# zero-savvy/vimz

Measured on AMD Instinct MI355X. Metric: nova_folding_steps_per_sec, higher is better.
Workload: dtype u32 limbs (256-bit Montgomery integers over BN254 Fr/Fq)

## Files before the change

### include/vimz_hip.h

```cpp
#ifndef VIMZ_HIP_H
#define VIMZ_HIP_H

#include <stddef.h>
#include <stdint.h>

#ifdef __cplusplus
extern "C" {
#endif

#define VIMZ_OK 0
#define VIMZ_ERR_INVALID (-1)
#define VIMZ_ERR_HIP (-2)
#define VIMZ_ERR_NO_DEVICE (-3)
#define VIMZ_ERR_UNSAT (-4)

#define VIMZ_FORM_CANONICAL 0
#define VIMZ_FORM_MONTGOMERY 1

#define VIMZ_CURVE_BN254_G1 0
#define VIMZ_CURVE_GRUMPKIN 1
#define VIMZ_CURVE_PALLAS 2
#define VIMZ_CURVE_VESTA 3

#define VIMZ_FIELD_BN254_FR 0
#define VIMZ_FIELD_BN254_FQ 1
#define VIMZ_FIELD_PALLAS_FP 2
#define VIMZ_FIELD_VESTA_FQ 3

typedef struct vimz_ctx vimz_ctx;
typedef struct vimz_bases vimz_bases;
typedef struct vimz_vec vimz_vec;

int vimz_ctx_create(int device, vimz_ctx** out);
void vimz_ctx_destroy(vimz_ctx* ctx);
const char* vimz_last_error(const vimz_ctx* ctx);
const char* vimz_version(void);
int vimz_device_info(vimz_ctx* ctx, char* name, size_t name_len, int* cus, uint64_t* hbm_bytes);
int vimz_sync(vimz_ctx* ctx);

int vimz_trace_marker(vimz_ctx* ctx, int id);
long vimz_set_head_rows(long rows);
long vimz_set_rows_group(long rows);
int vimz_host_fingerprint(vimz_ctx* ctx, double out[4]);
int vimz_timer_start(vimz_ctx* ctx);
int vimz_timer_stop(vimz_ctx* ctx, float* ms_out);
int vimz_set_profiling(vimz_ctx* ctx, int enabled);
int vimz_msm_last_profile(vimz_ctx* ctx, float ms[6], uint32_t info[4]);
int vimz_msm_profile_totals(vimz_ctx* ctx, double ms[6], uint64_t counts[3], int reset);

int vimz_bases_upload(vimz_ctx* ctx, int curve, const uint64_t* xy, size_t n, int form, vimz_bases** out);
int vimz_bases_generate(vimz_ctx* ctx, int curve, const char* label, size_t label_len, size_t n, vimz_bases** out);
int vimz_bases_download(vimz_ctx* ctx, const vimz_bases* b, size_t offset, uint64_t* xy, size_t n, int form);
int vimz_bases_precompute(vimz_ctx* ctx, vimz_bases* b, int window_bits);
size_t vimz_bases_len(const vimz_bases* b);
void vimz_bases_free(vimz_ctx* ctx, vimz_bases* b);

size_t vimz_pack_count(size_t height, size_t width, int block);
int vimz_pack_pixels(vimz_ctx* ctx, const uint8_t* pixels, size_t height, size_t width, int channels, int block, uint64_t* out);

typedef struct {
  const uint8_t* pixels;
  size_t height, width;
  int channels;
  const uint64_t* units;
  size_t n_units, unit_len;
  int block;
  size_t max_units;
  const uint8_t* drop;
} vimz_image_desc;
int vimz_image_hash(vimz_ctx* ctx, const vimz_image_desc* imgs, size_t n, uint64_t* out);
int vimz_image_hash_last_profile(vimz_ctx* ctx, double ms[2]);

#define VIMZ_EDIT_HASH 0
#define VIMZ_EDIT_GRAYSCALE 1
#define VIMZ_EDIT_BRIGHTNESS 2
#define VIMZ_EDIT_CONTRAST 3
#define VIMZ_EDIT_BLUR 4
#define VIMZ_EDIT_SHARPNESS 5
#define VIMZ_EDIT_RESIZE 6
#define VIMZ_EDIT_CROP 7
#define VIMZ_EDIT_REDACT 8
typedef struct {
  int op;
  const uint8_t* pixels;
  size_t height, width;
  int channels;
  int64_t source;
  double factor;
  size_t x, y;
  size_t new_width, new_height;
  const uint8_t* redact;
  size_t n_redact;
  uint8_t* out_pixels;
  uint64_t* out_source;
  uint64_t* out_target;
} vimz_edit_desc;
typedef struct {
  size_t height, width;
  int channels;
  size_t source_units, source_unit_len;
  size_t target_units, target_unit_len;
} vimz_edit_shape;
#define VIMZ_EDIT_MAX_DESCS 4096
int vimz_image_edit_shapes(vimz_ctx* ctx, const vimz_edit_desc* descs, size_t n, vimz_edit_shape* out);
int vimz_image_edit(vimz_ctx* ctx, const vimz_edit_desc* descs, size_t n);
int vimz_image_edit_last_profile(vimz_ctx* ctx, double ms[3]);

int vimz_vec_alloc(vimz_ctx* ctx, int field, size_t n, vimz_vec** out);
int vimz_vec_upload(vimz_ctx* ctx, vimz_vec* v, size_t offset, const uint64_t* host, size_t n, int form);
int vimz_vec_download(vimz_ctx* ctx, const vimz_vec* v, size_t offset, uint64_t* host, size_t n, int form);
size_t vimz_vec_len(const vimz_vec* v);
void vimz_vec_free(vimz_ctx* ctx, vimz_vec* v);

int vimz_msm(vimz_ctx* ctx, const vimz_bases* bases, const uint64_t* scalars, size_t n, int form,
             int window_bits, uint64_t out_xy[8], int out_form);
int vimz_msm_vec(vimz_ctx* ctx, const vimz_bases* bases, size_t base_offset, const vimz_vec* v, size_t offset,
                 size_t n, int window_bits, uint64_t out_xy[8], int out_form);

#define VIMZ_MSM_SPLIT_ONES 1
int vimz_msm_vec_ex(vimz_ctx* ctx, const vimz_bases* bases, size_t base_offset, const vimz_vec* v, size_t offset,
                    size_t n, int window_bits, int flags, uint64_t out_xy[8], int out_form);

typedef struct vimz_r1cs vimz_r1cs;
typedef struct { const uint32_t* row; const uint32_t* col; const uint64_t* val ; size_t nnz; } vimz_coo;
int vimz_r1cs_upload(vimz_ctx* ctx, int field, size_t nrows, size_t ncols, const vimz_coo* A, const vimz_coo* B, const vimz_coo* C, int form,
// ... 201 lines not shown
```

### include/vimz_hip_testing.h

```cpp
#ifndef VIMZ_HIP_TESTING_H
#define VIMZ_HIP_TESTING_H
#include "vimz_hip.h"

#ifdef __cplusplus
extern "C" {
#endif

int vimz_cf_poke(vimz_cf* v, int which, size_t index, const uint64_t value[4]);
int vimz_cf_selfcheck(int steps, uint32_t* result, uint64_t counts[8]);
int64_t vimz_cf_selfcheck_last_step(int steps, void* buf, size_t cap);
int64_t vimz_cf_selfcheck_merge(int segs_run0, int segs_run1, void* buf, size_t cap);
int64_t vimz_worker_selftest(int jobs);
int vimz_strict_bits_selfcheck(int field, int values, uint64_t out[8]);
void vimz_test_forge_public_slot(int on);
int vimz_decider_selfcheck(int steps, int full, uint32_t* result, uint64_t counts[4]);
int vimz_testing_kzg_setup_seeded(vimz_ctx* ctx, const uint8_t* seed, size_t seed_len, size_t n, vimz_bases** srs_out, uint64_t vk_g2_out[16]);
int vimz_testing_decider_setup_seeded(vimz_cf* prover, const uint64_t kzg_vk_g2[16], int light, const uint8_t* seed, size_t seed_len, vimz_decider** out, double seconds[4]);

int vimz_test_fp29_probe(vimz_ctx* ctx, int field, int op, const uint32_t* a, const uint32_t* b, const uint32_t* c, const uint32_t* d, uint32_t* out, size_t n);
int vimz_test_spmv_cross16(vimz_ctx* ctx, const vimz_r1cs* S, size_t row0, size_t nrows, const vimz_vec* z, vimz_vec* az, vimz_vec* bz, vimz_vec* cz,
                           const vimz_vec* az1, const vimz_vec* bz1, const vimz_vec* cz1, const uint64_t u1[4], const uint64_t u2[4], int form, vimz_vec* T);
int vimz_test_cross_term_masked(vimz_ctx* ctx, size_t n, const vimz_vec* az1, const vimz_vec* bz1, const vimz_vec* cz1, const uint64_t u1[4], const vimz_vec* az2,
                                const vimz_vec* bz2, const vimz_vec* cz2, const uint64_t u2[4], int form, vimz_vec* T, vimz_vec* Tm, size_t nb);
int vimz_test_msm_rows(vimz_ctx* ctx, const vimz_bases* bases, const uint64_t* scalars, size_t n, size_t row_stride, size_t G, int form, int use_tables,
                       size_t n_ones, int calls, uint64_t* out_xy, uint64_t* s1_xy, uint64_t* s1_ref_xy);

#ifdef __cplusplus
}
#endif
#endif
```

### vimz_amd/csrc/ivc.hip

```cpp
#include "ivc_internal.hpp"

namespace {

int scalar_bits(const uint32_t* k) {
  for (int i = 7; i >= 0; i--) if (k[i]) return 32 * i + 32 - __builtin_clz(k[i]);
  return 0;
}

int finish_secondary(vimz_ivc* v) {
  if (!v->pending_sec) return VIMZ_OK;
  vimz_ctx* ctx = v->ctx;
  double t0 = now_s();
  P_TRY(vz_wait_stream(v->s2));
  v->u2.W = msm_finish<Grumpkin>(v->plan_W2, v->pin + 2 * v->pin_res);
  P_TRY(vz_wait_stream(ctx->stream));
  v->ph_s[IP_WAIT_SEC] += now_s() - t0; v->ph_n[IP_WAIT_SEC]++;
  if (ctx->profiling) { float ms = 0; if (hipEventElapsedTime(&ms, v->ev_b0, v->ev_b1) == hipSuccess) { v->ph_s[IP_RESERVED] += ms * 1e-3; v->ph_n[IP_RESERVED]++; } }
  if (v->sec_T_valid) v->T2 = msm_finish<Grumpkin>(v->plan_T2, v->pin + 3 * v->pin_res);
  else { v->T2.x = Fe::zero(); v->T2.y = Fe::zero(); }
  static const bool dbg = getenv("VIMZ_DEBUG_CHECK_MSM") != nullptr;
  if (dbg) {
    G2Aff r; MsmStats st;
    P_TRY(msm_run<Grumpkin>(ctx->stream, ctx->msm_ws, v->ck2->d, v->sec.z2 + 8, v->sec.n_w - 3, 1, 0, &r, &st, nullptr, 0, nullptr));
    if (!r.x.eq(v->u2.W.x) || !r.y.eq(v->u2.W.y)) fprintf(stderr, "[dbg] step %llu: MSM(W2) on stream 2 differs from the recomputation\n", (unsigned long long)v->i);
    if (v->sec_T_valid) {
      P_TRY(msm_run<Grumpkin>(ctx->stream, ctx->msm_ws, v->ck2->d, v->sec.T, v->sec.n_c, 1, 0, &r, &st, nullptr, 0, nullptr));
      if (!r.x.eq(v->T2.x) || !r.y.eq(v->T2.y)) fprintf(stderr, "[dbg] step %llu: MSM(T2) differs from the recomputation\n", (unsigned long long)v->i);
    }
  }
  v->pending_sec = false;
  return VIMZ_OK;
}

int ivc_fold_core(vimz_ivc* v, const uint64_t* step_inputs, const uint64_t* witnesses, size_t nsteps) {
  if (!nsteps) return VIMZ_OK;
  vimz_ctx* ctx = v->ctx;
  if (v->broken) return vz_fail(ctx, VIMZ_ERR_INVALID, "this IVC failed in the middle of a step and cannot be folded any further");
  vimz_prover* p = v->pri;
  std::lock_guard<std::mutex> g(ctx->mu);
  P_TRY(hipSetDevice(ctx->device));
  hipStream_t s = ctx->stream;
  const size_t nw = p->n_wires, nc = p->n_c, sw = p->step_wires, sc = p->step_c;
  const size_t aw1 = v->c1->aug_wires();
  SecDev& S = v->sec;
  int rc;
  const double t_all = now_s();
  FoldJob job; job.step_inputs = step_inputs; job.witnesses = witnesses; job.nsteps = nsteps;
  dbg_stamp(p, "ivc fold: lock taken");
  if ((rc = fold_prepare(p, job, true))) return rc;
  struct BrokenGuard { vimz_ivc* v; bool armed = true; ~BrokenGuard() { if (armed) v->broken = true; } } guard{v};
  auto settle = [&](size_t rows_done) {
    hipStreamSynchronize(p->sB);
    if (p->sD) hipStreamSynchronize(p->sD);
    hipStreamSynchronize(v->s3); v->t1[0].step = v->t1[1].step = -1;
    const int rc2 = finish_secondary(v);
    for (uint32_t q = 0; q < p->len_z; q++) p->z_cur[q] = job.zs[rows_done * p->len_z + q];
    if (!rc2) guard.armed = false;
  };
  static const bool dbg_timing = getenv("VIMZ_DEBUG_TIMING") != nullptr;
  const double t_prep = now_s() - t_all;
  double t_first = 0, t_wait0 = 0, t_hook = 0, t_hk[5] = {0, 0, 0, 0, 0}, t_wp[5] = {0, 0, 0, 0, 0};
  const std::vector<Fe>& zs = job.zs;
  const size_t pin_stride = FoldJob::pin_stride;
  char* pin_aug1 = v->pin + 5 * v->pin_res;
  char* pin_w2 = pin_aug1 + 32 * aw1;
  const Fq zero_q = Fq::zero();

  typedef vimz_prover::BatchBuf BufRef;
  const bool trick = v->bool_rows && v->helpers.empty() && !witnesses;
  if (trick && v->i > 0 && !v->ca_valid) {
    G1Aff r; MsmStats st;
    P_TRY(hipStreamSynchronize(v->s3));
    P_TRY(msm_run<BnG1>(s, ctx->msm_ws, p->ck->d, p->AZ, p->n_bool, 1, 0, &r, &st, nullptr, 0, p->ck->tables ? &job.tbl : nullptr));
    v->CA = from_affine(r);
  }
  v->ca_valid = false;
  G1Aff S1_row; S1_row.x = S1_row.y = Fq::zero();
  bool pend_ca = false; uint32_t pend_rho[4] = {0, 0, 0, 0}; G1Aff pend_S1 = S1_row; int pend_slot[2] = {-1, -1};
  auto apply_pending_ca = [&]() {
    if (!pend_ca) return;
    if (!aff_is_identity(pend_S1)) { const uint32_t k[5] = {pend_rho[0], pend_rho[1], pend_rho[2], pend_rho[3], 1u}; G1 t = scalar_mul(pend_S1, k, 129); add_full(v->CA, t); }
    for (int q : pend_slot) if (q >= 0) v->t1[q].ca_at = v->CA;
    pend_ca = false;
  };
  auto queue_msm = [&](int par) -> int {
    auto& S = v->t1[par];
    const size_t parts = v->helpers.size() + 1, share = (sc + parts - 1) / parts;
    v->t1_main_n = std::min(share, sc);
    if (!v->helpers.empty()) {
      P_TRY(hipEventRecord(v->ev_T, v->s3));
      size_t off = v->t1_main_n;
      for (auto& h : v->helpers) {
        h.off = off; h.n = off < sc ? std::min(share, sc - off) : 0; off += h.n;
        if (!h.n) continue;
        P_TRY(hipSetDevice(h.ctx->device));
        P_TRY(hipStreamWaitEvent(h.s, v->ev_T, 0));
        P_TRY(hipMemcpyAsync(h.T, S.buf + 8 * h.off, 32 * h.n, hipMemcpyDefault, h.s));
        P_TRY(msm_launch<BnG1>(h.s, h.ws, h.ck->d + (size_t)AFFINE_WORDS * h.off, h.T, h.n, 1, 0, h.pin, &h.plan, nullptr, 0, nullptr));
      }
      P_TRY(hipSetDevice(ctx->device));
    }
    double tq = now_s();
    P_TRY(msm_launch<BnG1>(v->s3, v->ws3, p->ck->d, S.tricked ? S.bufm : S.buf, v->t1_main_n, 1, 0, S.pin, &S.plan, ctx->profiling ? S.ev : nullptr, 0,
                           p->ck->tables && v->helpers.empty() ? &job.tbl : nullptr));
    t_hk[2] += now_s() - tq; tq = now_s();
    if (ctx->profiling) P_TRY(hipMemcpyAsync(S.pin + v->pin_res, v->ws3.totals, 8, hipMemcpyDeviceToHost, v->s3));
    P_TRY(hipEventRecord(S.done, v->s3));
    t_hk[1] += now_s() - tq;
    return VIMZ_OK;
  };
  auto launch_direct = [&](BufRef& b2, size_t row, uint64_t step) -> int {
    auto& S = v->t1[step & 1];
    P_TRY(hipEventRecord(v->ev_fold, s));
    P_TRY(hipStreamWaitEvent(v->s3, v->ev_fold, 0));
    P_TRY(wait_row_flag(b2, row, b2.ev[row]));
    hipLaunchKernelGGL(k_cross_term<Fr>, dim3(stream_grid(sc)), dim3(256), 0, v->s3, sc, p->AZ, p->BZ, p->CZ, v->u1_run,
                       b2.az + 8 * row * nc, b2.bz + 8 * row * nc, b2.cz + 8 * row * nc, Fe::one(), S.buf, trick ? S.bufm : (uint32_t*)nullptr, p->n_bool);
    P_TRY(hipGetLastError());
    S.step = (int64_t)step; S.hasB = false;
    S.tricked = trick; S.u_at = v->u1_run; S.ca_at = v->CA;
    return queue_msm((int)(step & 1));
  };
  struct RowAt { BufRef* b; size_t row; };
  struct FoldArgs { uint64_t i; BufRef* cur; size_t r; Fe rho; bool need1; RowAt next1; bool look; RowAt next2; };
  auto launch_fold_and_cross = [&](const FoldArgs& a) -> int {
    const int par = (int)(a.i & 1);
    auto& Scur = v->t1[par]; auto& Soth = v->t1[par ^ 1];
    const bool fold_E = a.i > 0, hasB = fold_E && Scur.hasB;
    const uint32_t *az = a.cur->az + 8 * a.r * nc, *bz = a.cur->bz + 8 * a.r * nc, *cz = a.cur->cz + 8 * a.r * nc;
    if (hasB) P_TRY(wait_row_flag(*a.cur, a.cur->flag_rows + a.r, a.cur->ev_d[a.r]));
    const RowAt* t = a.need1 ? &a.next1 : a.look ? &a.next2 : nullptr;
    uint32_t* out = a.need1 ? Soth.buf : a.look ? Scur.buf : nullptr;
    uint32_t* outm = !trick ? nullptr : a.need1 ? Soth.bufm : a.look ? Scur.bufm : nullptr;
    double tq = now_s();
    if (t) P_TRY(wait_row_flag(*t->b, t->row, t->b->ev[t->row]));
    t_hk[4] += now_s() - tq; tq = now_s();
    hipLaunchKernelGGL(k_fold_cross<Fr>, dim3(stream_grid(sc)), dim3(256), 0, v->s3, sc, p->AZ, p->BZ, p->CZ, p->E, (const uint32_t*)Scur.buf, fold_E ? 1 : 0, a.rho,
                       hasB ? 1 : 0, v->rho_prev, hasB ? (const uint32_t*)(a.cur->d + 8 * a.r * sc) : (const uint32_t*)nullptr, v->u1_run, az, bz, cz,
                       out, t ? t->b->az + 8 * t->row * nc : nullptr, t ? t->b->bz + 8 * t->row * nc : nullptr, t ? t->b->cz + 8 * t->row * nc : nullptr, Fe::one(),
                       outm, p->n_bool);
    P_TRY(hipGetLastError());
    if (a.need1 && a.look) {
      P_TRY(wait_row_flag(*a.next2.b, a.next2.row, a.next2.b->ev[a.next2.row]));
      hipLaunchKernelGGL(k_cross_term<Fr>, dim3(stream_grid(sc)), dim3(256), 0, v->s3, sc, p->AZ, p->BZ, p->CZ, v->u1_run,
                         a.next2.b->az + 8 * a.next2.row * nc, a.next2.b->bz + 8 * a.next2.row * nc, a.next2.b->cz + 8 * a.next2.row * nc, Fe::one(), Scur.buf,
                         trick ? Scur.bufm : (uint32_t*)nullptr, p->n_bool);
      P_TRY(hipGetLastError());
    }
    t_hk[0] += now_s() - tq; tq = now_s();
    P_TRY(hipEventRecord(v->ev_fused, v->s3)); v->fused_recorded = true;
    t_hk[1] += now_s() - tq;
    if (a.need1) { Soth.step = (int64_t)a.i + 1; Soth.hasB = false; Soth.tricked = trick; Soth.u_at = v->u1_run; int rc2 = queue_msm(par ^ 1); if (rc2) return rc2; }
    if (a.look) { Scur.step = (int64_t)a.i + 2; Scur.hasB = true; Scur.tricked = trick; Scur.u_at = v->u1_run; int rc2 = queue_msm(par); if (rc2) return rc2; }
    return VIMZ_OK;
  };
  std::atomic<size_t> allowed{0}, issued{job.next_issue};
  std::atomic<int> issuer_rc{VIMZ_OK};
  std::atomic<bool> issuer_stop{false};
  std::thread issuer([&, b0 = job.next_issue] {
    if (hipSetDevice(ctx->device) != hipSuccess) { issuer_rc = VIMZ_ERR_HIP; return; }
    for (size_t b = b0; b < job.nbatches; b++) {
      const size_t need = job.first(b) + job.rows(b);
      while (allowed.load(std::memory_order_acquire) <= b || job.states_upto.load(std::memory_order_acquire) < need) {
        if (issuer_stop.load()) return;
        if (job.helper_done.load() && job.states_upto.load() < need) { issuer_rc = job.helper_rc ? job.helper_rc : VIMZ_ERR_HIP; return; }
        std::this_thread::sleep_for(std::chrono::microseconds(100));
      }
      const double _ti = now_s();
      const int rc2 = fold_issue(p, job, b);
      if (dbg_timing) fprintf(stderr, "[timing] producer: batch %zu (%zu rows): ready at %.1f ms, issue took %.1f ms\n", b, job.rows(b), 1e3 * (_ti - t_all), 1e3 * (now_s() - _ti));
      if (rc2) { issuer_rc = rc2; return; }
      issued.store(b + 1, std::memory_order_release);
    }
  });
  struct IssuerJoin { std::thread& t; std::atomic<bool>& stop; ~IssuerJoin() { stop = true; if (t.joinable()) t.join(); } } issuer_join{issuer, issuer_stop};
  auto wait_issued = [&](size_t b) -> int {
    const double t_wait = now_s(); uint64_t spins = 0;
    while (issued.load(std::memory_order_acquire) <= b) {
      const int irc = issuer_rc.load();
      if (irc) { if (ctx->err.empty()) ctx->err = job.helper_err.empty() ? std::string("fold: the batch producer stopped early") : job.helper_err; return irc; }
      std::this_thread::yield();
      if ((++spins & 0xfffff) == 0 && now_s() - t_wait > 120.0) return vz_fail(ctx, VIMZ_ERR_HIP, "fold: batch not issued within 120 s");
    }
    return VIMZ_OK;
  };
  for (size_t k = 0; k < job.nbatches; k++) {
    auto& bb = p->buf[k & 1];
    const size_t first = job.first(k), rows = job.rows(k);
    double t0 = now_s();
    allowed.store(k + 2, std::memory_order_release);
    if ((rc = wait_issued(k))) return rc;
    if (k == 0) dbg_stamp(p, "ivc fold: first batch issued");
    P_TRY(vz_wait_event(bb.wit_done));
    v->ph_s[IP_PRODUCER] += now_s() - t0;
    if (k == 0) { t_wait0 = now_s() - t0; t_first = now_s() - t_all; dbg_stamp(p, "ivc fold: first batch's witnesses ready"); }
    for (size_t r = 0; r < rows; r++) if (bb.status_host[r]) {
      char msg[128]; snprintf(msg, sizeof(msg), "step %llu: the step relation is not satisfiable for these rows", (unsigned long long)(v->i + r));
      settle(first);
      return vz_fail(ctx, VIMZ_ERR_UNSAT, msg);
    }
    for (size_t r = 0; r < rows; r++) {
      const uint64_t i = v->i;
      uint32_t* Zi = bb.Z + 8 * r * nw;
      uint32_t *az = bb.az + 8 * r * nc, *bz = bb.bz + 8 * r * nc, *cz = bb.cz + 8 * r * nc;
      v->c1->precompute_statement(i + 1, v->z0, zs.data() + (first + r + 1) * p->len_z);
      G1 boolCorr = G1::identity();
      if (trick) {
        apply_pending_ca();
        P_TRY(wait_row_flag(bb, r, bb.ev[r]));
        S1_row = to_affine(ones_finish<BnG1>((const char*)bb.pin + r * pin_stride + vimz_prover::S1_SLOT));
        auto& sl = v->t1[i & 1];
        if (i > 0 && sl.step == (int64_t)i && sl.tricked) {
          if (!aff_is_identity(S1_row)) { const Fe uc = Fe::from_mont(sl.u_at); boolCorr = scalar_mul(S1_row, uc.v, scalar_bits(uc.v)); }
          G1 nca = sl.ca_at; if (!nca.is_identity()) nca.Y = Fq::neg(nca.Y);
          add_full(boolCorr, nca);
        }
      }
      if ((rc = finish_secondary(v))) return rc;
      t0 = now_s();
      AugIn<BnFr> in1; in1.digest = v->c1->digest; in1.z0 = v->z0; in1.i = i; in1.U = v->U2; in1.u = v->u2; in1.T = v->T2;
      std::vector<Fe> aug1; bool bad = false;
      AugOut<BnFr> o1 = v->c1->witness(in1, zs.data() + (first + r) * p->len_z, zs.data() + (first + r + 1) * p->len_z, aug1, &bad);
      if (bad) { settle(first + r); return vz_fail(ctx, VIMZ_ERR_UNSAT, "primary verifier circuit: inconsistent incoming instance"); }
      v->ph_s[IP_SYNTH1] += now_s() - t0; v->ph_n[IP_SYNTH1]++;
      t0 = now_s();
      v->U2 = o1.U_new;
      memcpy(pin_aug1, aug1.data(), 32 * aw1);
      P_TRY(wait_row_flag(bb, r, bb.ev[r]));
      P_TRY(upload_pinned(s, Zi + 8 * sw, pin_aug1, 32 * aw1));
      P_TRY(hipEventRecord(v->ev_fork, s));
      P_TRY(hipStreamWaitEvent(v->s2, v->ev_fork, 0));
      P_TRY(msm_launch<BnG1>(v->s2, v->ws2, p->ck->d + (size_t)AFFINE_WORDS * (sw - 1), Zi + 8 * sw, aw1 - 2, 1, 0, v->pin, &v->plan_aug, nullptr, 0, v->tb_aug.d ? &v->tb_aug : nullptr));
      P_TRY(hipStreamWaitEvent(s, v->ev_fold, 0));
      hipLaunchKernelGGL(k_spmv_cross16<Fr>, dim3((unsigned)((16 * (nc - sc) + 255) / 256)), dim3(256), 0, s, p->A, p->B, p->C, p->dict, (uint32_t)sc, (uint32_t)(nc - sc),
                         Zi, az, bz, cz, i > 0 ? p->AZ : nullptr, p->BZ, p->CZ, v->u1_run, Fe::one(), p->T);
// ... 764 lines not shown
```

### vimz_amd/csrc/msm.hpp

```cpp
#pragma once
#include <cstdlib>
#include <cstring>
#include <mutex>
#include "msm_api.hpp"
#include "ec_mem.hpp"

namespace vz {

struct MsmTuning { int sort_blocks = 0, combine_lane_bits = -1, small_lean = 0, witness_sub = 0, ones_dense = 1, reduce_planes = 0, accum_lds_kb = 0, dense_sub = 0, signed_scalars = 1; };
inline const MsmTuning& msm_tuning() {
  static const MsmTuning t = [] {
    MsmTuning r;
    if (const char* e = getenv("VIMZ_TUNE")) {
      if (const char* q = strstr(e, "sort_blocks=")) r.sort_blocks = atoi(q + 12);
      if (const char* q = strstr(e, "combine_lane_bits=")) r.combine_lane_bits = atoi(q + 18);
      if (const char* q = strstr(e, "small_lean=")) r.small_lean = atoi(q + 11);
      if (const char* q = strstr(e, "witness_sub=")) { const int v = atoi(q + 12); if (v >= 2 && v <= MSM_SUB) r.witness_sub = v; }
      if (const char* q = strstr(e, "dense_sub=")) { const int v = atoi(q + 10); if (v >= 2 && v <= MSM_SUB) r.dense_sub = v; }
      if (const char* q = strstr(e, "ones_dense=")) r.ones_dense = atoi(q + 11);
      if (const char* q = strstr(e, "reduce_planes=")) r.reduce_planes = atoi(q + 14);
      if (const char* q = strstr(e, "signed_scalars=")) r.signed_scalars = atoi(q + 15) != 0;
      if (const char* q = strstr(e, "accum_lds_kb=")) { const int v = atoi(q + 13); if (v >= 0 && v <= 160) r.accum_lds_kb = v; }
    }
    return r;
  }();
  return t;
}


__device__ __forceinline__ uint32_t window_bits(const uint32_t* s, int lo, int c) {
  int limb = lo >> 5, off = lo & 31;
  if (limb >= 8) return 0;
  uint64_t v = s[limb];
  if (limb + 1 < 8) v |= (uint64_t)s[limb + 1] << 32;
  return (uint32_t)(v >> off) & ((1u << c) - 1);
}

template <class S>
__device__ __forceinline__ bool load_scalar(const uint32_t* __restrict__ scalars, size_t i, int mont, int skip_ones, int sgn, uint32_t* s, uint32_t& flip) {
  const uint4* p = reinterpret_cast<const uint4*>(scalars + 8 * i);
  uint4 a = p[0], b = p[1];
  S x;
  x.v[0] = a.x; x.v[1] = a.y; x.v[2] = a.z; x.v[3] = a.w; x.v[4] = b.x; x.v[5] = b.y; x.v[6] = b.z; x.v[7] = b.w;
  if (x.is_zero()) return false;
  if (skip_ones) {
    bool one;
    if (mont) one = x.eq(S::one());
    else { uint32_t o = x.v[0] ^ 1u; for (int k = 1; k < 8; k++) o |= x.v[k]; one = o == 0; }
    if (one) return false;
  }
  if (mont) x = S::from_mont(x);
  flip = 0;
  if (sgn) {
    uint32_t t[8]; uint64_t br = 0, lt = 0;
#pragma unroll
    for (int k = 0; k < 8; k++) { const uint64_t d = (uint64_t)S::Params::MOD.w[k] - x.v[k] - br; t[k] = (uint32_t)d; br = (d >> 32) & 1; }
#pragma unroll
    for (int k = 0; k < 8; k++) { const uint64_t d = (uint64_t)t[k] - x.v[k] - lt; lt = (d >> 32) & 1; }
    if (!br && lt) {
      flip = 1;
#pragma unroll
      for (int k = 0; k < 8; k++) x.v[k] = t[k];
    }
  }
#pragma unroll
  for (int k = 0; k < 8; k++) s[k] = x.v[k];
  return true;
}

template <class Fn>
__device__ __forceinline__ void for_each_digit(const uint32_t* s, int c, int K, uint32_t flip, Fn f) {
  uint32_t carry = 0;
  const uint32_t half = 1u << (c - 1);
  for (int w = 0; w < K; w++) {
    uint32_t d = window_bits(s, w * c, c) + carry;
    uint32_t neg = d > half;
    uint32_t mag = neg ? (1u << c) - d : d;
    carry = neg;
    if (mag) f(w, mag - 1, neg ^ flip);
  }
}

__device__ __forceinline__ uint32_t agg_atomic_inc(uint32_t* __restrict__ ctr, uint32_t g) {
  const uint32_t lane = __lane_id();
  bool done = false;
  uint32_t pos = 0;
  for (int round = 0; round < 4; round++) {
    const uint64_t pending = __ballot(!done);
    if (pending == 0) break;
    const int leader = __ffsll((unsigned long long)pending) - 1;
    const uint32_t lg = __shfl(g, leader);
    const bool mine = !done && g == lg;
    const uint64_t same = __ballot(mine);
    uint32_t base = 0;
    if (mine && lane == (uint32_t)leader) base = atomicAdd(&ctr[g], (uint32_t)__popcll(same));
    base = __shfl(base, leader);
    if (mine) { pos = base + (uint32_t)__popcll(same & ((1ull << lane) - 1ull)); done = true; }
    if (__popcll(same) < 4) break;
  }
  if (!done) pos = atomicAdd(&ctr[g], 1u);
  return pos;
}

template <class S>
__global__ void k_hist(const uint32_t* __restrict__ scalars, size_t n, int mont, int skip_ones, int sgn, int c, int K, uint32_t nbw ,
                       uint32_t* __restrict__ counts) {
  for (size_t i = blockIdx.x * (size_t)blockDim.x + threadIdx.x; i < n; i += (size_t)gridDim.x * blockDim.x) {
    uint32_t s[8], flip;
    if (!load_scalar<S>(scalars, i, mont, skip_ones, sgn, s, flip)) continue;
    for_each_digit(s, c, K, flip, [&](int w, uint32_t b, uint32_t) { agg_atomic_inc(counts, (uint32_t)w * nbw + b); });
  }
}

__device__ __forceinline__ void scan_body(const uint32_t* __restrict__ counts, uint32_t nb,
                                               uint32_t* __restrict__ bucket_off, uint32_t* __restrict__ sub_off,
                                               uint32_t* __restrict__ totals, uint32_t sub,
                                               uint32_t* __restrict__ heavy ,
                                               uint32_t heavy_min, uint32_t heavy_cap) {
  __shared__ uint32_t wv_e[2][16], wv_s[2][16];
  const uint32_t t = threadIdx.x, lane = t & 63u, wv = t >> 6;
  uint32_t carry_e = 0, carry_s = 0;
  for (uint32_t base = 0, it = 0; base < nb; base += 1024, it++) {
    const uint32_t b = base + t;
    const uint32_t cnt = b < nb ? counts[b] : 0u, m = (cnt + sub - 1) / sub;
    uint32_t ie = cnt, is = m;
#pragma unroll
    for (uint32_t d = 1; d < 64; d <<= 1) {
      const uint32_t ve = __shfl_up(ie, d), vs = __shfl_up(is, d);
      if (lane >= d) { ie += ve; is += vs; }
    }
    if (lane == 63) { wv_e[it & 1][wv] = ie; wv_s[it & 1][wv] = is; }
    __syncthreads();
    uint32_t oe = 0, os = 0, te = 0, ts = 0;
    for (uint32_t q = 0; q < 16; q++) { const uint32_t xe = wv_e[it & 1][q], xs = wv_s[it & 1][q]; if (q < wv) { oe += xe; os += xs; } te += xe; ts += xs; }
    if (b < nb) {
      bucket_off[b] = carry_e + oe + ie - cnt; sub_off[b] = carry_s + os + is - m;
      if (m > heavy_min) { const uint32_t slot = atomicAdd(&heavy[0], 1u); if (slot < heavy_cap) heavy[1 + slot] = b; }
    }
    carry_e += te; carry_s += ts;
  }
  if (t == 0) { bucket_off[nb] = carry_e; sub_off[nb] = carry_s; totals[0] = carry_s; totals[1] = carry_e; }
}
template <int SUB>
__global__ void __launch_bounds__(1024) k_scan(const uint32_t* __restrict__ counts, uint32_t nb, uint32_t* __restrict__ bucket_off, uint32_t* __restrict__ sub_off,
                                               uint32_t* __restrict__ totals, uint32_t sub, uint32_t* __restrict__ heavy, uint32_t heavy_min, uint32_t heavy_cap) {
  scan_body(counts, nb, bucket_off, sub_off, totals, sub, heavy, heavy_min, heavy_cap);
}

template <class S>
__global__ void k_scatter(const uint32_t* __restrict__ scalars, size_t n, int mont, int skip_ones, int sgn, int c, int K, uint32_t nbw,
                          uint32_t pt_stride ,
                          const uint32_t* __restrict__ bucket_off, uint32_t* __restrict__ cursor,
                          uint32_t* __restrict__ sorted) {
  for (size_t i = blockIdx.x * (size_t)blockDim.x + threadIdx.x; i < n; i += (size_t)gridDim.x * blockDim.x) {
    uint32_t s[8], flip;
    if (!load_scalar<S>(scalars, i, mont, skip_ones, sgn, s, flip)) continue;
    for_each_digit(s, c, K, flip, [&](int w, uint32_t b, uint32_t neg) {
      uint32_t g = (uint32_t)w * nbw + b;
      uint32_t pos = bucket_off[g] + agg_atomic_inc(cursor, g);
      sorted[pos] = ((uint32_t)i + (uint32_t)w * pt_stride) | (neg << 31);
    });
  }
}

constexpr uint32_t SORT_BLOCKS = 256;
constexpr uint32_t SORT_THREADS = 1024;

template <class S>
__global__ void __launch_bounds__(SORT_THREADS) k_hist_lds(const uint32_t* __restrict__ scalars, size_t n, int mont, int skip_ones, int sgn, int c, int K,
                                                           uint32_t nbw, uint32_t nb, uint32_t* __restrict__ block_hist , MsmRowStrides rs) {
  extern __shared__ uint32_t lds_cnt[];
  scalars += blockIdx.y * rs.scalars; block_hist += blockIdx.y * rs.block_hist;
  for (uint32_t g = threadIdx.x; g < nb; g += SORT_THREADS) lds_cnt[g] = 0;
  __syncthreads();
  const size_t chunk = (n + gridDim.x - 1) / gridDim.x;
  const size_t lo = blockIdx.x * chunk, hi = lo + chunk < n ? lo + chunk : n;
  for (size_t i = lo + threadIdx.x; i < hi; i += SORT_THREADS) {
    uint32_t s[8], flip;
    if (!load_scalar<S>(scalars, i, mont, skip_ones, sgn, s, flip)) continue;
    for_each_digit(s, c, K, flip, [&](int w, uint32_t b, uint32_t) { atomicAdd(&lds_cnt[(uint32_t)w * nbw + b], 1u); });
  }
  __syncthreads();
  uint32_t* out = block_hist + (size_t)blockIdx.x * nb;
  for (uint32_t g = threadIdx.x; g < nb; g += SORT_THREADS) out[g] = lds_cnt[g];
}

template <int DUMMY>
__global__ void __launch_bounds__(1024) k_prefix_scan(uint32_t* __restrict__ block_hist, uint32_t nb, uint32_t* __restrict__ counts, uint32_t nblocks,
                                                      uint32_t* __restrict__ heavy, uint32_t* __restrict__ bucket_off, uint32_t* __restrict__ sub_off,
                                                      uint32_t* __restrict__ totals, uint32_t sub, uint32_t heavy_min, uint32_t heavy_cap, MsmRowStrides rs) {
  __shared__ uint32_t s_last;
  {
    const size_t row = blockIdx.y;
    block_hist += row * rs.block_hist; counts += row * rs.counts; heavy += row * rs.heavy; bucket_off += row * rs.offs; sub_off += row * rs.offs; totals += row * rs.totals;
  }
  const uint32_t g = blockIdx.x * blockDim.x + threadIdx.x;
  if (g < nb) {
    uint32_t run = 0;
    for (uint32_t blk = 0; blk < nblocks; blk++) {
      const size_t idx = (size_t)blk * nb + g;
      const uint32_t v = block_hist[idx];
      block_hist[idx] = run;
      run += v;
    }
    counts[g] = run;
  }
  __threadfence();
  __syncthreads();
  if (threadIdx.x == 0) s_last = atomicAdd(&totals[2], 1u) == gridDim.x - 1 ? 1u : 0u;
  __syncthreads();
  if (!s_last) return;
  __threadfence();
  if (threadIdx.x == 0) { __hip_atomic_store(&totals[2], 0u, __ATOMIC_RELAXED, __HIP_MEMORY_SCOPE_AGENT); heavy[0] = 0; }
  __syncthreads();
  scan_body(counts, nb, bucket_off, sub_off, totals, sub, heavy, heavy_min, heavy_cap);
}

template <class S>
__global__ void __launch_bounds__(SORT_THREADS) k_scatter_lds(const uint32_t* __restrict__ scalars, size_t n, int mont, int skip_ones, int sgn, int c, int K,
                                                              uint32_t nbw, uint32_t nb, uint32_t pt_stride, const uint32_t* __restrict__ bucket_off,
                                                              const uint32_t* __restrict__ block_hist, uint32_t* __restrict__ sorted, MsmRowStrides rs) {
  extern __shared__ uint32_t lds_pos[];
  { const size_t row = blockIdx.y; scalars += row * rs.scalars; bucket_off += row * rs.offs; block_hist += row * rs.block_hist; sorted += row * rs.sorted; }
  const uint32_t* mine = block_hist + (size_t)blockIdx.x * nb;
  for (uint32_t g = threadIdx.x; g < nb; g += SORT_THREADS) lds_pos[g] = bucket_off[g] + mine[g];
  __syncthreads();
  const size_t chunk = (n + gridDim.x - 1) / gridDim.x;
  const size_t lo = blockIdx.x * chunk, hi = lo + chunk < n ? lo + chunk : n;
  for (size_t i = lo + threadIdx.x; i < hi; i += SORT_THREADS) {
    uint32_t s[8], flip;
    if (!load_scalar<S>(scalars, i, mont, skip_ones, sgn, s, flip)) continue;
    for_each_digit(s, c, K, flip, [&](int w, uint32_t b, uint32_t neg) {
      const uint32_t pos = atomicAdd(&lds_pos[(uint32_t)w * nbw + b], 1u);
      sorted[pos] = ((uint32_t)i + (uint32_t)w * pt_stride) | (neg << 31);
    });
  }
}

template <class F>
__global__ void __launch_bounds__(256, 3) k_accum(const uint32_t* __restrict__ bases, const uint32_t* __restrict__ sorted,
                                               const uint32_t* __restrict__ bucket_off, const uint32_t* __restrict__ sub_off,
                                               uint32_t nb, const uint32_t* __restrict__ totals,
                                               uint32_t* __restrict__ partial, uint32_t sub, MsmRowStrides rs) {
  { const size_t row = blockIdx.y; sorted += row * rs.sorted; bucket_off += row * rs.offs; sub_off += row * rs.offs; totals += row * rs.totals; partial += row * rs.partial; }
  const uint32_t total = totals[0];
  uint32_t s = blockIdx.x * blockDim.x + threadIdx.x;
  if (s >= total) return;
  uint32_t lo = 0, hi = nb;
  while (hi - lo > 1) {
    uint32_t mid = (lo + hi) >> 1;
    if (sub_off[mid] <= s) lo = mid; else hi = mid;
  }
  const uint32_t b = lo, k = s - sub_off[b];
  const uint32_t beg = bucket_off[b] + k * sub;
  const uint32_t end = min(bucket_off[b + 1], beg + sub);
  XYZZ<F> acc = XYZZ<F>::identity();
  uint32_t ent = beg < end ? sorted[beg] : 0u;
  RawAffine raw = load_affine_raw(bases, ent & 0x7fffffffu);
  for (uint32_t e = beg; e < end; e++) {
    const uint32_t ent_n = e + 1 < end ? sorted[e + 1] : ent;
    const RawAffine raw_n = load_affine_raw(bases, ent_n & 0x7fffffffu);
    Affine<F> q = affine_of_raw<F>(raw);
    if ((ent >> 31) && !aff_is_identity(q)) q.y = F::neg(q.y);
    add_mixed(acc, q);
    ent = ent_n; raw = raw_n;
  }
  store_xyzz(partial, s, acc);
}

constexpr uint32_t ONES_THREADS = 16384;
template <class S>
__device__ __forceinline__ bool scalar_is_one(const uint32_t* __restrict__ scalars, size_t i, int mont) {
  const uint4* p = reinterpret_cast<const uint4*>(scalars + 8 * i);
  const uint4 a = p[0], b = p[1];
  if (mont) return a.x == S::Params::R1.w[0] && a.y == S::Params::R1.w[1] && a.z == S::Params::R1.w[2] && a.w == S::Params::R1.w[3] &&
                   b.x == S::Params::R1.w[4] && b.y == S::Params::R1.w[5] && b.z == S::Params::R1.w[6] && b.w == S::Params::R1.w[7];
  return a.x == 1u && (a.y | a.z | a.w | b.x | b.y | b.z | b.w) == 0u;
}
template <class S, class F>
__global__ void __launch_bounds__(256) k_ones_partial(const uint32_t* __restrict__ scalars, const uint32_t* __restrict__ bases, size_t n, int mont,
                                                      uint32_t* __restrict__ out ) {
  const uint32_t t = blockIdx.x * blockDim.x + threadIdx.x;
  XYZZ<F> acc = XYZZ<F>::identity();
  for (size_t i = t; i < n; i += ONES_THREADS)
    if (scalar_is_one<S>(scalars, i, mont)) { Affine<F> q = load_affine<F>(bases, (uint32_t)i); add_mixed(acc, q); }
  store_xyzz(out, t, acc);
}
template <class S, class F>
__device__ __forceinline__ XYZZ<F> ones_dense_sum(const uint32_t* __restrict__ scalars, const uint32_t* __restrict__ bases, size_t n, int mont, uint32_t (*queue)[128]) {
  const uint32_t t = blockIdx.x * blockDim.x + threadIdx.x, lane = threadIdx.x & 63u, wv = threadIdx.x >> 6;
  const size_t wave = t >> 6, nwaves = ONES_THREADS / 64;
  volatile uint32_t* q = queue[wv];
  XYZZ<F> acc = XYZZ<F>::identity();
  uint32_t cnt = 0;
  for (size_t base = wave * 64; base < n; base += nwaves * 64) {
    const size_t i = base + lane;
    const bool one = i < n && scalar_is_one<S>(scalars, i, mont);
    const uint64_t m = __ballot(one);
    if (one) q[cnt + (uint32_t)__popcll(m & ((1ull << lane) - 1ull))] = (uint32_t)i;
    cnt += (uint32_t)__popcll(m);
    __builtin_amdgcn_wave_barrier();
    if (cnt >= 64) {
      cnt -= 64;
      const uint32_t idx = q[cnt + lane];
      __builtin_amdgcn_wave_barrier();
      Affine<F> pt = load_affine<F>(bases, idx);
      add_mixed(acc, pt);
    }
  }
  if (lane < cnt) { Affine<F> pt = load_affine<F>(bases, q[lane]); add_mixed(acc, pt); }
  return acc;
}
// ... 428 lines not shown
    have[k] = false; neg[k] = false;
    if (i < n) {
      uint32_t sc[8], flip;
      if (load_scalar<S>(scalars, i, mont, 0, sgn, sc, flip)) {
        const int d = flip ? -signed_digit<SMALL_C>(sc, (int)w) : signed_digit<SMALL_C>(sc, (int)w);
        if (d) {
          have[k] = true; neg[k] = d < 0;
          const uint32_t m = (uint32_t)(d < 0 ? -d : d) - 1u;
          const uint32_t* src = mult + (size_t)AFFINE_WORDS * (((size_t)w * tstride + i) * NM + m);
          pt[k] = load_affine_at<F>(src);
        }
      }
    }
  }
  XYZZ<F> acc = XYZZ<F>::identity();
#pragma unroll
  for (int k = 0; k < (int)FIXED_PER_THREAD; k++) {
    if (have[k]) {
      if (neg[k] && !aff_is_identity(pt[k])) pt[k].y = F::neg(pt[k].y);
      add_mixed(acc, pt[k]);
    }
  }
  sh[t] = acc;
  __syncthreads();
  quad_level<F>(sh, 64, [](uint32_t e) { return e; }, [](uint32_t e) { return e + 128; });
  quad_level<F>(sh, 64, [](uint32_t e) { return e + 64; }, [](uint32_t e) { return e + 192; });
  for (uint32_t d = 64; d > 0; d >>= 1) quad_level<F>(sh, d, [](uint32_t e) { return e; }, [d](uint32_t e) { return e + d; });
  if (Q == 1) { if (t == 0) store_xyzz(window_sums, w, sh[0]); return; }
  if (t < 64) {
    if (t == 0) store_xyzz(partial, (size_t)w * Q + q, sh[0]);
    __threadfence();
    if (t == 0) s_ticket = atomicAdd(&done[w], 1u);
  }
  __syncthreads();
  if (s_ticket != Q - 1) return;
  __threadfence();
  if (t < FIXED_MAXQ) {
    XYZZ<F> v = XYZZ<F>::identity();
    if (t < Q) {
      v = load_xyzz<F>(partial, (size_t)w * Q + t);
    }
    sh[t] = v;
  }
  __syncthreads();
  uint32_t top = 1; while (top < Q) top <<= 1;
  for (uint32_t d = top >> 1; d > 0; d >>= 1) quad_level<F>(sh, d, [](uint32_t e) { return e; }, [d](uint32_t e) { return e + d; });
  if (t == 0) { store_xyzz(window_sums, w, sh[0]); __hip_atomic_store(&done[w], 0u, __ATOMIC_RELAXED, __HIP_MEMORY_SCOPE_AGENT); }
}



template <class F>
__device__ __forceinline__ XYZZ<F> small_mul(const XYZZ<F>& p, uint32_t k) {
  XYZZ<F> acc = XYZZ<F>::identity();
  if (!k) return acc;
  for (int bit = 31 - __clz(k); bit >= 0; bit--) { acc = dbl(acc); if ((k >> bit) & 1) add_full(acc, p); }
  return acc;
}
template <class F>
__global__ void __launch_bounds__(256) k_build_tables(const uint32_t* __restrict__ bases, size_t n, int c, int K, uint32_t* __restrict__ tables) {
  const size_t i = blockIdx.x * (size_t)blockDim.x + threadIdx.x;
  if (i >= n) return;
  Affine<F> p = load_affine<F>(bases, (uint32_t)i);
  store_affine<F>(tables, i, p);
  for (int j = 1; j < K; j++) {
    XYZZ<F> acc = from_affine(p);
    for (int k = 0; k < c; k++) acc = dbl(acc);
    p = to_affine(acc);
    store_affine<F>(tables, (size_t)j * n + i, p);
  }
}
template <class C>
hipError_t build_tables(hipStream_t stream, const uint32_t* d_bases, size_t n, int c, int K, uint32_t* d_tables) {
  typedef typename C::Coord F;
  if (!n) return hipSuccess;
  hipLaunchKernelGGL(k_build_tables<F>, dim3((unsigned)((n + 255) / 256)), dim3(256), 0, stream, d_bases, n, c, K, d_tables);
  return hipGetLastError();
}

struct MsmRowGroup { uint32_t G; size_t scalar_row_stride , pinned_row_stride ; const OnesDesc* extra; uint32_t n_extra; uint32_t max_rows; size_t* row_bytes_out ; };
template <class C>
static hipError_t msm_launch_impl(hipStream_t stream, MsmWorkspace& ws, const uint32_t* d_bases, const uint32_t* d_scalars, size_t n,
                                  int scalars_mont, int c_override, void* pinned_dst, MsmPlan* plan_out, hipEvent_t* ev, int split_ones,
                                  const BaseTables* tb, const MsmRowGroup* rg) {
  typedef typename C::Coord F;
  typedef typename C::Scalar S;
  if (n == 0 || n >= (1u << 31)) return hipErrorInvalidValue;
  const uint32_t G = rg ? rg->G : 1u;
  if (rg && !rg->row_bytes_out && (G == 0 || G > MSM_ROWS_MAX || rg->n_extra > MSM_ROWS_MAX || (split_ones == 0 && rg->n_extra))) return hipErrorInvalidValue;
  const int sgn = msm_tuning().signed_scalars;
  constexpr bool direct = true;
  static const bool no_small = getenv("VIMZ_DEBUG_NO_SMALL_MSM") != nullptr;
  const bool small_fmt = tb && tb->d && tb->c == SMALL_C;
  const bool small_tb = small_fmt && !no_small && c_override <= 0;
  bool tabled = tb && tb->d && !small_fmt && c_override <= 0;
  if (tabled && tb->own && tb->c != msm_plan(n, S::Params::BITS, 0).c) tabled = false;
  const bool own = tabled && tb->own;
  if (small_tb && (n > MSM_SMALL_MAX || tb->K != (S::Params::BITS + SMALL_C) / SMALL_C)) return hipErrorInvalidValue;
  if (!no_small && !tabled && c_override <= 0 && n <= MSM_SMALL_MAX) {
    if (rg) return hipErrorNotSupported;
    MsmPlan ps; ps.c = SMALL_C; ps.K = (S::Params::BITS + SMALL_C) / SMALL_C; ps.nbw = SMALL_NBW; ps.nb = SMALL_NBW * (uint32_t)ps.K; ps.split_ones = 0; ps.tabled = small_tb ? 2 : 0;
    *plan_out = ps;
    VZ_HIP_CHECK(ws.reserve_small());
    const uint32_t Q = (uint32_t)((n + SMALL_CHUNK - 1) / SMALL_CHUNK), chunk = (uint32_t)((n + Q - 1) / Q);
    uint32_t* done = reinterpret_cast<uint32_t*>(ws.small_buf);
    uint32_t* chunk_out = done + 128;
    if (small_tb && tb->mult) {
      const uint32_t Qf = (uint32_t)((n + FIXED_CHUNK - 1) / FIXED_CHUNK);
      if (ev) for (int i = 0; i < 4; i++) VZ_HIP_CHECK(hipEventRecord(ev[i], stream));
      hipLaunchKernelGGL((k_msm_fixed<S, F>), dim3(Qf, ps.K), dim3(256), 0, stream, tb->mult + (size_t)AFFINE_WORDS * SMALL_NBW * tb->offset, (uint32_t)tb->n_total, d_scalars, (uint32_t)n,
                         scalars_mont, sgn, Qf, chunk_out, done, direct ? reinterpret_cast<uint32_t*>(pinned_dst) : reinterpret_cast<uint32_t*>(ws.window_sums));
      if (ev) for (int i = 4; i < 7; i++) VZ_HIP_CHECK(hipEventRecord(ev[i], stream));
      VZ_HIP_CHECK(hipGetLastError());
      if (!direct) VZ_HIP_CHECK(hipMemcpyAsync(pinned_dst, ws.window_sums, 4 * (size_t)XYZZ_WORDS * ps.K, hipMemcpyDeviceToHost, stream));
      return hipSuccess;
    }
    if (ev) for (int i = 0; i < 4; i++) VZ_HIP_CHECK(hipEventRecord(ev[i], stream));
    static const bool sum_kernel = getenv("VIMZ_DEBUG_SMALL_SUM_KERNEL") != nullptr;
#define VZ_SMALL(LEAN) hipLaunchKernelGGL((k_msm_small<S, F, LEAN>), dim3(ps.K, Q), dim3(SMALL_THREADS), 0, stream, d_bases, d_scalars, (uint32_t)n, scalars_mont, sgn, Q, chunk, chunk_out, \
                       sum_kernel ? (uint32_t*)nullptr : done, direct ? reinterpret_cast<uint32_t*>(pinned_dst) : reinterpret_cast<uint32_t*>(ws.window_sums), \
                       small_tb ? tb->d + (size_t)AFFINE_WORDS * tb->offset : (const uint32_t*)nullptr, small_tb ? (uint32_t)tb->n_total : 0u)
    switch (msm_tuning().small_lean) { case 0: VZ_SMALL(0); break; case 1: VZ_SMALL(1); break; default: VZ_SMALL(2); break; }
#undef VZ_SMALL
    if (Q > 1 && sum_kernel) hipLaunchKernelGGL(k_msm_small_sum<F>, dim3(ps.K), dim3(64), 0, stream, chunk_out, Q, direct ? reinterpret_cast<uint32_t*>(pinned_dst) : reinterpret_cast<uint32_t*>(ws.window_sums));
    if (ev) for (int i = 4; i < 7; i++) VZ_HIP_CHECK(hipEventRecord(ev[i], stream));
    VZ_HIP_CHECK(hipGetLastError());
    if (!direct) VZ_HIP_CHECK(hipMemcpyAsync(pinned_dst, ws.window_sums, 4 * (size_t)XYZZ_WORDS * ps.K, hipMemcpyDeviceToHost, stream));
    return hipSuccess;
  }
  MsmPlan pl = msm_plan(n, S::Params::BITS, tabled ? tb->c : c_override);
  if (tabled) {
    if (tb->K != pl.K || pl.nbw < 256 || (size_t)tb->K * tb->n_total >= (1u << 31)) return hipErrorInvalidValue;
    if (!own && 2 * (pl.nbw / std::min<uint32_t>(pl.nbw, MSM_VWIN)) + 1 > (uint32_t)MSM_MAX_WINDOWS) return hipErrorInvalidValue;
    if (own) pl.tabled = 3; else { pl.nb = pl.nbw; pl.tabled = 1; }
    d_bases = tb->d + (size_t)AFFINE_WORDS * tb->offset;
  }
  if (pl.K + 1 > MSM_MAX_WINDOWS || pl.c > 16 || pl.c < 2) return hipErrorInvalidValue;
  pl.split_ones = split_ones;
  const bool no_planes = !msm_tuning().reduce_planes;
  uint32_t Pl = 0; while ((1u << Pl) < pl.nbw) Pl++;
  uint32_t Gp = std::min<uint32_t>(16u, pl.nbw / 1024u);
  while (Gp > 1 && (Pl + 2) * Gp > 256) Gp >>= 1;
  const bool planes = tabled && !own && !no_planes && pl.nbw >= 1024 && (1u << Pl) == pl.nbw && (Pl + 2) * Gp <= 256 && (int)Pl + 2 + 1 <= MSM_MAX_WINDOWS;
  if (planes) pl.tabled = 4;
  const bool lds_sort = (size_t)pl.nb * 4 <= 144 * 1024;
  if (rg && (planes || own || !lds_sort)) return hipErrorNotSupported;
  *plan_out = pl;
  const size_t entries = (size_t)pl.K * n;
  const int wsub = msm_tuning().witness_sub;
  const int dsub = tb && tb->sub_hint > 0 ? tb->sub_hint : msm_tuning().dense_sub;
  const uint32_t sub = n < (1u << 15) ? 8u : split_ones ? (uint32_t)(wsub > 0 ? wsub : n < (1u << 19) ? 8 : MSM_SUB) : (uint32_t)(dsub >= 2 && dsub <= (int)MSM_SUB ? dsub : MSM_SUB);
  const size_t max_subs = entries / sub + pl.nb + 1;
  if (rg && rg->row_bytes_out) { *rg->row_bytes_out = MsmWorkspace::row_bytes(pl.nb, entries, max_subs, (size_t)SORT_BLOCKS * pl.nb); return hipSuccess; }
  VZ_HIP_CHECK(ws.reserve(pl.nb, entries, max_subs, rg ? std::max<size_t>(G, rg->max_rows) : 1));
  MsmRowStrides rs;
  if (G > 1) {
    rs.scalars = 8 * rg->scalar_row_stride; rs.block_hist = (size_t)SORT_BLOCKS * pl.nb; rs.sorted = entries; rs.partial = (size_t)XYZZ_WORDS * max_subs;
    rs.heavy_scratch = MsmWorkspace::HEAVY_SCRATCH_WORDS; rs.out = rg->pinned_row_stride / 4;
    rs.counts = pl.nb; rs.offs = pl.nb + 1; rs.totals = MsmWorkspace::TOTALS_WORDS; rs.heavy = MsmWorkspace::HEAVY_CAP + 1; rs.heavy_done = MsmWorkspace::HEAVY_DONE_WORDS;
  }
  const int TB = 256;
#define VZ_EV(i) do { if (ev) VZ_HIP_CHECK(hipEventRecord(ev[i], stream)); } while (0)
  VZ_EV(0);
  const unsigned gs = (unsigned)std::min<size_t>((n + TB - 1) / TB, 256 * 16);
  if (!lds_sort) {
    VZ_HIP_CHECK(hipMemsetAsync(ws.counts, 0, 4 * (size_t)pl.nb, stream));
    VZ_HIP_CHECK(hipMemsetAsync(ws.cursor, 0, 4 * (size_t)pl.nb, stream));
    VZ_HIP_CHECK(hipMemsetAsync(ws.heavy, 0, 4, stream));
  }
  const int sort_blocks_env = msm_tuning().sort_blocks;
  const uint32_t sort_blocks = sort_blocks_env > 0 && sort_blocks_env <= (int)SORT_BLOCKS ? (uint32_t)sort_blocks_env
                                                                                           : (uint32_t)std::min<size_t>(SORT_BLOCKS, std::max<size_t>(32, n / 4096));
  const uint32_t bstride = tabled && !own ? 0u : pl.nbw, pstride = tabled ? (uint32_t)tb->n_total : 0u;
  if (lds_sort) {
    VZ_HIP_CHECK(ws.reserve_block_hist((size_t)SORT_BLOCKS * pl.nb));
    {
      static std::mutex attr_mu;
      static uint64_t attr_devices = 0;
      int dev = 0;
      VZ_HIP_CHECK(hipGetDevice(&dev));
      std::lock_guard<std::mutex> g(attr_mu);
      if (!((attr_devices >> (dev & 63)) & 1ull)) {
        VZ_HIP_CHECK(hipFuncSetAttribute(reinterpret_cast<const void*>(&k_hist_lds<S>), hipFuncAttributeMaxDynamicSharedMemorySize, 160 * 1024));
        VZ_HIP_CHECK(hipFuncSetAttribute(reinterpret_cast<const void*>(&k_scatter_lds<S>), hipFuncAttributeMaxDynamicSharedMemorySize, 160 * 1024));
        attr_devices |= 1ull << (dev & 63);
      }
    }
    hipLaunchKernelGGL(k_hist_lds<S>, dim3(sort_blocks, G), dim3(SORT_THREADS), pl.nb * 4, stream, d_scalars, n, scalars_mont, split_ones, sgn, pl.c, pl.K, bstride, pl.nb, ws.block_hist, rs);
  } else {
    hipLaunchKernelGGL(k_hist<S>, dim3(gs), dim3(TB), 0, stream, d_scalars, n, scalars_mont, split_ones, sgn, pl.c, pl.K, bstride, ws.counts);
  }
  VZ_EV(1);
  const size_t mean_parts = (split_ones ? entries / 8 : entries) / sub / pl.nb + 1;
  const int lane_bits_env = msm_tuning().combine_lane_bits;
  const uint32_t lane_bits = lane_bits_env >= 0 ? (uint32_t)lane_bits_env : mean_parts > 96 ? 4u : mean_parts > 48 ? 3u : mean_parts > 24 ? 2u : 1u;
  const uint32_t heavy_min = 16u << lane_bits;
  if (lds_sort)
    hipLaunchKernelGGL(k_prefix_scan<0>, dim3((pl.nb + 1023) / 1024, G), dim3(1024), 0, stream, ws.block_hist, pl.nb, ws.counts, sort_blocks, ws.heavy, ws.bucket_off, ws.sub_off,
                       ws.totals, sub, heavy_min, MsmWorkspace::HEAVY_CAP, rs);
  else
    hipLaunchKernelGGL(k_scan<MSM_SUB>, dim3(1), dim3(1024), 0, stream, ws.counts, pl.nb, ws.bucket_off, ws.sub_off, ws.totals, sub, ws.heavy, heavy_min, MsmWorkspace::HEAVY_CAP);
  VZ_EV(2);
  if (lds_sort)
    hipLaunchKernelGGL(k_scatter_lds<S>, dim3(sort_blocks, G), dim3(SORT_THREADS), pl.nb * 4, stream, d_scalars, n, scalars_mont, split_ones, sgn, pl.c, pl.K, bstride, pl.nb,
                       pstride, ws.bucket_off, ws.block_hist, ws.sorted, rs);
  else
    hipLaunchKernelGGL(k_scatter<S>, dim3(gs), dim3(TB), 0, stream, d_scalars, n, scalars_mont, split_ones, sgn, pl.c, pl.K, bstride, pstride,
                       ws.bucket_off, ws.cursor, ws.sorted);
  VZ_EV(3);
  uint32_t* partial = reinterpret_cast<uint32_t*>(ws.partial);
  const unsigned ga = (unsigned)((max_subs + TB - 1) / TB);
  const size_t accum_lds = (size_t)msm_tuning().accum_lds_kb * 1024;
  if (accum_lds > 65536) { static const hipError_t once = hipFuncSetAttribute((const void*)k_accum<F>, hipFuncAttributeMaxDynamicSharedMemorySize, 160 * 1024); (void)once; }
  hipLaunchKernelGGL(k_accum<F>, dim3(ga, G), dim3(TB), accum_lds, stream, d_bases, ws.sorted, ws.bucket_off, ws.sub_off, pl.nb,
                     ws.totals, partial, sub, rs);
  VZ_EV(4);
  const unsigned per_wg = 256u >> lane_bits, nbn = (pl.nb + per_wg - 1) / per_wg;
  hipLaunchKernelGGL(k_combine<F>, dim3(nbn + COMBINE_HEAVY_BLOCKS + COMBINE_SPLIT_BLOCKS, G), dim3(256), 0, stream, partial, ws.sub_off, pl.nb, nbn,
                     (const uint32_t*)ws.heavy, MsmWorkspace::HEAVY_CAP, ws.heavy_scratch, lane_bits, heavy_min, ws.heavy_done, rs);
  VZ_EV(5);
  const unsigned T = pl.nbw < 256 ? pl.nbw : 256;
  uint32_t* wsum = direct ? reinterpret_cast<uint32_t*>(pinned_dst) : reinterpret_cast<uint32_t*>(ws.window_sums);
  const uint32_t vw = std::min<uint32_t>(pl.nbw, MSM_VWIN);
  const int V = (int)(pl.nbw / vw);
  const int kout = planes ? (int)Pl + 2 : tabled && !own ? 2 * V : pl.K;
  if (planes) {
    hipLaunchKernelGGL(k_reduce_planes<F>, dim3((Pl + 2) * Gp), dim3(256), 0, stream, (const uint32_t*)partial, (const uint32_t*)ws.counts, (const uint32_t*)ws.sub_off, pl.nbw, Pl, Gp,
                       pl.nbw / (512u * Gp), ws.plane_scratch, ws.totals + 3, wsum);
  } else if (tabled && !own) {
    hipLaunchKernelGGL(k_reduce<F>, dim3(V, G), dim3(vw < 256 ? vw : 256), 0, stream, (const uint32_t*)partial, (const uint32_t*)ws.counts, (const uint32_t*)ws.sub_off, vw, wsum, wsum + (size_t)XYZZ_WORDS * V, rs);
  } else
    hipLaunchKernelGGL(k_reduce<F>, dim3(pl.K, G), dim3(T), 0, stream, (const uint32_t*)partial, (const uint32_t*)ws.counts, (const uint32_t*)ws.sub_off, pl.nbw, wsum, (uint32_t*)nullptr, rs);
  VZ_EV(6);
#undef VZ_EV
  if (split_ones && rg) {
    OnesDesc ds[2 * MSM_ROWS_MAX];
    for (uint32_t r = 0; r < G; r++) ds[r] = OnesDesc{d_scalars + 8 * r * rg->scalar_row_stride, d_bases, wsum + r * (rg->pinned_row_stride / 4) + (size_t)XYZZ_WORDS * kout, n};
    for (uint32_t e = 0; e < rg->n_extra; e++) ds[G + e] = rg->extra[e];
    VZ_HIP_CHECK(ones_launch_rows<C>(stream, ws, ds, G + rg->n_extra, scalars_mont));
  } else if (split_ones) {
    uint32_t* lvl0 = reinterpret_cast<uint32_t*>(ws.ones_partial);
    if (msm_tuning().ones_dense) hipLaunchKernelGGL((k_ones_dense<S, F>), dim3(ONES_THREADS / 256), dim3(256), 0, stream, d_scalars, d_bases, n, scalars_mont, lvl0);
    else hipLaunchKernelGGL((k_ones_partial<S, F>), dim3(ONES_THREADS / 256), dim3(256), 0, stream, d_scalars, d_bases, n, scalars_mont, lvl0);
    uint32_t* lvl1 = lvl0 + (size_t)XYZZ_WORDS * ONES_THREADS;
    hipLaunchKernelGGL(k_tree256<F>, dim3(ONES_THREADS / 256), dim3(256), 0, stream, lvl0, ONES_THREADS, lvl1);
    hipLaunchKernelGGL(k_tree256<F>, dim3(1), dim3(256), 0, stream, lvl1, ONES_THREADS / 256, wsum + (size_t)XYZZ_WORDS * kout);
  }
  VZ_HIP_CHECK(hipGetLastError());
  if (!direct) VZ_HIP_CHECK(hipMemcpyAsync(pinned_dst, wsum, 4 * (size_t)XYZZ_WORDS * (kout + (split_ones ? 1 : 0)), hipMemcpyDeviceToHost, stream));
  return hipSuccess;
}

template <class C>
hipError_t msm_launch(hipStream_t stream, MsmWorkspace& ws, const uint32_t* d_bases, const uint32_t* d_scalars, size_t n,
                      int scalars_mont, int c_override, void* pinned_dst, MsmPlan* plan_out, hipEvent_t* ev, int split_ones,
                      const BaseTables* tb) {
  return msm_launch_impl<C>(stream, ws, d_bases, d_scalars, n, scalars_mont, c_override, pinned_dst, plan_out, ev, split_ones, tb, nullptr);
}
template <class C>
hipError_t msm_launch_rows(hipStream_t stream, MsmWorkspace& ws, const uint32_t* d_bases, const uint32_t* d_scalars, size_t n, size_t scalar_row_stride, uint32_t G,
                           int scalars_mont, void* pinned_dst, size_t pinned_row_stride, MsmPlan* plan_out, int split_ones, const BaseTables* tb,
                           const OnesDesc* extra, uint32_t n_extra, uint32_t max_rows) {
  if (G > 1 && (scalar_row_stride < n || (pinned_row_stride & 15))) return hipErrorInvalidValue;
  const MsmRowGroup rg{G, scalar_row_stride, pinned_row_stride, extra, n_extra, max_rows, nullptr};
  const hipError_t e = msm_launch_impl<C>(stream, ws, d_bases, d_scalars, n, scalars_mont, 0, pinned_dst, plan_out, nullptr, split_ones, tb, &rg);
  if (e != hipErrorNotSupported) return e;
  for (uint32_t r = 0; r < G; r++)
    VZ_HIP_CHECK(msm_launch<C>(stream, ws, d_bases, d_scalars + 8 * r * scalar_row_stride, n, scalars_mont, 0, (char*)pinned_dst + r * pinned_row_stride, plan_out, nullptr, split_ones, tb));
  if (n_extra) VZ_HIP_CHECK(ones_launch_rows<C>(stream, ws, extra, n_extra, scalars_mont));
  return hipSuccess;
}
template <class C>
size_t msm_rows_row_bytes(size_t n, int split_ones, const BaseTables* tb) {
  size_t bytes = 0;
  MsmWorkspace none; MsmPlan pl;
  const MsmRowGroup rg{1, n, 0, nullptr, 0, 0, &bytes};
  return msm_launch_impl<C>(nullptr, none, tb ? tb->d : nullptr, nullptr, n, 1, 0, nullptr, &pl, nullptr, split_ones, tb, &rg) == hipSuccess ? bytes : 0;
}

template <class C>
Affine<typename C::Base> msm_finish(const MsmPlan& pl, const void* pinned) {
  typedef typename C::Coord F;
  typedef typename C::Base FS;
  const uint32_t* hw = reinterpret_cast<const uint32_t*>(pinned);
  auto host_point = [&](int w) {
    XYZZ<FS> p; const uint32_t* d = hw + (size_t)XYZZ_WORDS * w;
    FS* f[4] = {&p.X, &p.Y, &p.ZZ, &p.ZZZ};
    for (int k = 0; k < 4; k++) { F t; for (int i = 0; i < 9; i++) t.v[i] = d[COORD_WORDS * k + i]; *f[k] = t.to_std(); }
    return p;
  };
  XYZZ<FS> acc = XYZZ<FS>::identity();
  if (pl.tabled == 4) {
    int P = 0; while ((1u << P) < pl.nbw) P++;
    for (int q = P - 1; q >= 0; q--) { acc = dbl(acc); add_full(acc, host_point(q)); }
    add_full(acc, host_point(P)); add_full(acc, host_point(P + 1));
    if (pl.split_ones) add_full(acc, host_point(P + 2));
    return to_affine(acc);
  }
  if (pl.tabled == 1) {
    const uint32_t vw = pl.nbw < MSM_VWIN ? pl.nbw : MSM_VWIN;
    const int V = (int)(pl.nbw / vw);
    XYZZ<FS> run = XYZZ<FS>::identity();
    for (int v = V - 1; v >= 1; v--) { add_full(run, host_point(V + v)); add_full(acc, run); }
    for (uint32_t k = 1; k < vw; k <<= 1) acc = dbl(acc);
    for (int v = 0; v < V; v++) add_full(acc, host_point(v));
    if (pl.split_ones) add_full(acc, host_point(2 * V));
    return to_affine(acc);
  }
  const int kout = pl.K;
  for (int w = kout - 1; w >= 0; w--) {
    if (!pl.tabled) for (int k = 0; k < pl.c; k++) acc = dbl(acc);
    add_full(acc, host_point(w));
  }
  if (pl.split_ones) add_full(acc, host_point(kout));
  return to_affine(acc);
}

template <class C>
hipError_t ones_launch(hipStream_t stream, MsmWorkspace& ws, const uint32_t* d_bases, const uint32_t* d_scalars, size_t n, int scalars_mont, void* pinned_dst) {
  typedef typename C::Coord F;
  typedef typename C::Scalar S;
  if (!ws.ones_partial) VZ_HIP_CHECK(hipMalloc(&ws.ones_partial, 4 * (size_t)XYZZ_WORDS * (16384 + 64 + 512)));
  uint32_t* lvl0 = reinterpret_cast<uint32_t*>(ws.ones_partial);
  uint32_t* lvl1 = lvl0 + (size_t)XYZZ_WORDS * ONES_THREADS;
  uint32_t* top = lvl1 + (size_t)XYZZ_WORDS * (ONES_THREADS / 256);
  hipLaunchKernelGGL((k_ones_dense<S, F>), dim3(ONES_THREADS / 256), dim3(256), 0, stream, d_scalars, d_bases, n, scalars_mont, lvl0);
  hipLaunchKernelGGL(k_tree256<F>, dim3(ONES_THREADS / 256), dim3(256), 0, stream, lvl0, ONES_THREADS, lvl1);
  hipLaunchKernelGGL(k_tree256<F>, dim3(1), dim3(256), 0, stream, lvl1, ONES_THREADS / 256, top);
  VZ_HIP_CHECK(hipGetLastError());
  return hipMemcpyAsync(pinned_dst, top, 4 * (size_t)XYZZ_WORDS, hipMemcpyDeviceToHost, stream);
}
template <class C>
hipError_t ones_launch_rows(hipStream_t stream, MsmWorkspace& ws, const OnesDesc* descs, uint32_t count, int scalars_mont) {
  typedef typename C::Coord F;
  typedef typename C::Scalar S;
  if (!count) return hipSuccess;
  if (count > 2 * MSM_ROWS_MAX) return hipErrorInvalidValue;
  if (!ws.ones_partial) VZ_HIP_CHECK(hipMalloc(&ws.ones_partial, 4 * (size_t)XYZZ_WORDS * (16384 + 64 + 512)));
  static_assert(2 * MSM_ROWS_MAX * (ONES_THREADS / 256) <= 16384, "the groups' partial sums fit ones_partial");
  OnesDescs ds;
  for (uint32_t i = 0; i < count; i++) ds.d[i] = descs[i];
  for (uint32_t i = count; i < 2 * MSM_ROWS_MAX; i++) ds.d[i] = OnesDesc{nullptr, nullptr, nullptr, 0};
  uint32_t* lvl = reinterpret_cast<uint32_t*>(ws.ones_partial);
  hipLaunchKernelGGL((k_ones_dense_rows<S, F>), dim3(ONES_THREADS / 256, count), dim3(256), 0, stream, ds, scalars_mont, lvl);
  hipLaunchKernelGGL(k_tree_rows<F>, dim3(count), dim3(256), 0, stream, (const uint32_t*)lvl, ONES_THREADS / 256, ds);
  return hipGetLastError();
}
template <class C>
XYZZ<typename C::Base> ones_finish(const void* pinned) {
  typedef typename C::Coord F;
  typedef typename C::Base FS;
  const uint32_t* d = reinterpret_cast<const uint32_t*>(pinned);
  XYZZ<FS> p; FS* f[4] = {&p.X, &p.Y, &p.ZZ, &p.ZZZ};
// ... 24 lines not shown
```

### vimz_amd/csrc/msm_api.hpp

```cpp
#pragma once
#include <hip/hip_runtime.h>
#include <vector>
#include <algorithm>
#include "ec.hpp"

namespace vz {

#define VZ_HIP_CHECK(x) do { hipError_t _e = (x); if (_e != hipSuccess) return _e; } while (0)

constexpr int MSM_SUB = 16;
constexpr int MSM_MAX_WINDOWS = 96;
constexpr uint32_t MSM_VWIN = 1024;

struct MsmPlan {
  int c;
  int K;
  uint32_t nbw;
  uint32_t nb;
  int split_ones;
  int tabled;
};

constexpr int SMALL_C = 7;
constexpr uint32_t SMALL_CHUNK = 1536, SMALL_MAXQ = 32;
constexpr size_t MSM_SMALL_MAX = (size_t)SMALL_CHUNK * 20;
static_assert(MSM_SMALL_MAX <= (size_t)SMALL_CHUNK * SMALL_MAXQ, "chunk results of a window fit the workspace");

struct BaseTables {
  const uint32_t* d; size_t n_total; size_t offset; int c, K; int own = 0;
  const uint32_t* mult = nullptr;
  int sub_hint = 0;
};

static inline MsmPlan msm_plan(size_t n, int scalar_bits, int c_override) {
  MsmPlan p;
  p.split_ones = 0; p.tabled = 0;
  int c = c_override;
  if (c <= 0) {
    c = n >= (1u << 15) ? 11 : n >= (1u << 12) ? 9 : n >= 256 ? 7 : 5;
  }
  p.c = c;
  p.K = (scalar_bits + 1 + c - 1) / c;
  p.nbw = 1u << (c - 1);
  p.nb = p.nbw * (uint32_t)p.K;
  return p;
}

struct MsmRowStrides {
  size_t scalars = 0, block_hist = 0, sorted = 0, partial = 0, heavy_scratch = 0, out = 0;
  uint32_t counts = 0, offs = 0 , totals = 0, heavy = 0, heavy_done = 0;
};
constexpr uint32_t MSM_ROWS_MAX = 16;
struct OnesDesc { const uint32_t* scalars; const uint32_t* bases; uint32_t* out; size_t n; };
struct OnesDescs { OnesDesc d[2 * MSM_ROWS_MAX]; };

struct MsmWorkspace {
  uint32_t* counts = nullptr;
  uint32_t* cursor = nullptr;
  uint32_t* bucket_off = nullptr;
  uint32_t* sub_off = nullptr;
  uint32_t* sorted = nullptr;
  void* partial = nullptr;
  void* window_sums = nullptr;
  uint32_t* totals = nullptr;
  uint32_t* block_hist = nullptr;
  size_t cap_block_hist = 0;
  void* ones_partial = nullptr;
  uint32_t* heavy = nullptr;
  uint32_t* heavy_scratch = nullptr;
  uint32_t* heavy_done = nullptr;
  uint32_t* plane_scratch = nullptr;
  static constexpr uint32_t HEAVY_CAP = 65536;
  size_t cap_nb = 0, cap_entries = 0, cap_subs = 0;
  size_t cap_rows = 1;
  void* host_pinned = nullptr;
  static constexpr uint32_t TOTALS_WORDS = 16, HEAVY_DONE_WORDS = 1024;
  static constexpr size_t HEAVY_SCRATCH_WORDS = (size_t)XYZZ_WORDS * 1024 * 32;

  static size_t row_bytes(uint32_t nb, size_t entries, size_t subs, size_t block_hist_words) {
    return 4 * (4 * (size_t)nb + 2 + entries + (size_t)XYZZ_WORDS * subs + block_hist_words + TOTALS_WORDS + HEAVY_CAP + 1 + HEAVY_SCRATCH_WORDS + HEAVY_DONE_WORDS);
  }
  hipError_t reserve(uint32_t nb, size_t entries, size_t subs, size_t rows = 1) {
    if (rows > cap_rows) {
      hipFree(counts); hipFree(cursor); hipFree(bucket_off); hipFree(sub_off); hipFree(sorted); hipFree(partial); hipFree(totals); hipFree(heavy); hipFree(heavy_scratch);
      hipFree(heavy_done); hipFree(block_hist);
      counts = cursor = bucket_off = sub_off = sorted = totals = heavy = heavy_scratch = heavy_done = block_hist = nullptr; partial = nullptr;
      cap_nb = cap_entries = cap_subs = cap_block_hist = 0;
      cap_rows = rows;
    }
    const size_t R = cap_rows;
    if (nb > cap_nb) {
      hipFree(counts); hipFree(cursor); hipFree(bucket_off); hipFree(sub_off);
      VZ_HIP_CHECK(hipMalloc(&counts, 4 * R * (size_t)nb)); VZ_HIP_CHECK(hipMalloc(&cursor, 4 * R * (size_t)nb));
      VZ_HIP_CHECK(hipMalloc(&bucket_off, 4 * R * ((size_t)nb + 1))); VZ_HIP_CHECK(hipMalloc(&sub_off, 4 * R * ((size_t)nb + 1)));
      cap_nb = nb;
    }
    if (entries > cap_entries) {
      hipFree(sorted); VZ_HIP_CHECK(hipMalloc(&sorted, 4 * R * entries)); cap_entries = entries;
    }
    if (subs > cap_subs) {
      hipFree(partial);
      VZ_HIP_CHECK(hipMalloc(&partial, 4 * XYZZ_WORDS * R * subs)); cap_subs = subs;
    }
    if (!window_sums) VZ_HIP_CHECK(hipMalloc(&window_sums, 4 * XYZZ_WORDS * MSM_MAX_WINDOWS));
    if (!totals) { VZ_HIP_CHECK(hipMalloc(&totals, 4 * R * TOTALS_WORDS)); VZ_HIP_CHECK(hipMemset(totals, 0, 4 * R * TOTALS_WORDS)); VZ_HIP_CHECK(hipStreamSynchronize(nullptr)); }
    if (!heavy) VZ_HIP_CHECK(hipMalloc(&heavy, 4 * R * (HEAVY_CAP + 1)));
    if (!heavy_scratch) VZ_HIP_CHECK(hipMalloc(&heavy_scratch, 4 * R * HEAVY_SCRATCH_WORDS));
    if (!heavy_done) { VZ_HIP_CHECK(hipMalloc(&heavy_done, 4 * R * HEAVY_DONE_WORDS)); VZ_HIP_CHECK(hipMemset(heavy_done, 0, 4 * R * HEAVY_DONE_WORDS)); VZ_HIP_CHECK(hipStreamSynchronize(nullptr)); }
    if (!plane_scratch) VZ_HIP_CHECK(hipMalloc(&plane_scratch, 4 * (size_t)XYZZ_WORDS * 256));
    if (!ones_partial) VZ_HIP_CHECK(hipMalloc(&ones_partial, 4 * (size_t)XYZZ_WORDS * (16384 + 64 + 512)));
    if (!host_pinned) VZ_HIP_CHECK(hipHostMalloc(&host_pinned, 4 * XYZZ_WORDS * MSM_MAX_WINDOWS));
    return hipSuccess;
  }
  void* small_buf = nullptr;
  hipError_t reserve_small() {
    if (!window_sums) VZ_HIP_CHECK(hipMalloc(&window_sums, 4 * XYZZ_WORDS * MSM_MAX_WINDOWS));
    if (!host_pinned) VZ_HIP_CHECK(hipHostMalloc(&host_pinned, 4 * XYZZ_WORDS * MSM_MAX_WINDOWS));
    if (!totals) { VZ_HIP_CHECK(hipMalloc(&totals, 4 * cap_rows * TOTALS_WORDS)); VZ_HIP_CHECK(hipMemset(totals, 0, 4 * cap_rows * TOTALS_WORDS)); VZ_HIP_CHECK(hipStreamSynchronize(nullptr)); }
    if (small_buf) return hipSuccess;
    const size_t bytes = 512 + 4 * (size_t)XYZZ_WORDS * MSM_MAX_WINDOWS * SMALL_MAXQ * (1u << (SMALL_C - 1));
    VZ_HIP_CHECK(hipMalloc(&small_buf, bytes));
    VZ_HIP_CHECK(hipMemset(small_buf, 0, 512));
    return hipStreamSynchronize(nullptr);
  }
  hipError_t reserve_block_hist(size_t words ) {
    if (words <= cap_block_hist) return hipSuccess;
    hipFree(block_hist); block_hist = nullptr; cap_block_hist = 0;
    VZ_HIP_CHECK(hipMalloc(&block_hist, 4 * cap_rows * words));
    cap_block_hist = words;
    return hipSuccess;
  }
  void release() {
    hipFree(counts); hipFree(cursor); hipFree(bucket_off); hipFree(sub_off); hipFree(sorted);
    hipFree(partial); hipFree(window_sums); hipFree(totals); hipFree(heavy); hipFree(heavy_scratch); hipFree(heavy_done); hipFree(plane_scratch); hipFree(small_buf); hipFree(ones_partial); hipFree(block_hist);
    if (host_pinned) hipHostFree(host_pinned);
    *this = MsmWorkspace();
  }
};

struct MsmStats { int c, K; uint32_t subs, entries; float ms[6]; };

template <class C>
hipError_t msm_launch(hipStream_t stream, MsmWorkspace& ws, const uint32_t* d_bases, const uint32_t* d_scalars, size_t n,
                      int scalars_mont, int c_override, void* pinned_dst, MsmPlan* plan_out, hipEvent_t* ev, int split_ones,
                      const BaseTables* tb = nullptr);
template <class C>
hipError_t msm_launch_rows(hipStream_t stream, MsmWorkspace& ws, const uint32_t* d_bases, const uint32_t* d_scalars, size_t n, size_t scalar_row_stride, uint32_t G,
                           int scalars_mont, void* pinned_dst, size_t pinned_row_stride, MsmPlan* plan_out, int split_ones, const BaseTables* tb,
                           const OnesDesc* extra = nullptr, uint32_t n_extra = 0, uint32_t max_rows = 0);
template <class C>
size_t msm_rows_row_bytes(size_t n, int split_ones, const BaseTables* tb);
template <class C>
hipError_t ones_launch_rows(hipStream_t stream, MsmWorkspace& ws, const OnesDesc* descs, uint32_t count, int scalars_mont);
template <class C>
hipError_t build_tables(hipStream_t stream, const uint32_t* d_bases, size_t n, int c, int K, uint32_t* d_tables);
template <class C>
hipError_t build_multiples(hipStream_t stream, const uint32_t* d_tables, size_t n, int c, int K, uint32_t* d_mult);
template <class C>
Affine<typename C::Base> msm_finish(const MsmPlan& pl, const void* pinned);
template <class C>
hipError_t msm_run(hipStream_t stream, MsmWorkspace& ws, const uint32_t* d_bases, const uint32_t* d_scalars, size_t n,
                   int scalars_mont, int c_override, Affine<typename C::Base>* out_affine_mont, MsmStats* stats,
                   hipEvent_t* ev , int split_ones, const BaseTables* tb = nullptr);
template <class C>
hipError_t ones_launch(hipStream_t stream, MsmWorkspace& ws, const uint32_t* d_bases, const uint32_t* d_scalars, size_t n, int scalars_mont, void* pinned_dst);
template <class C>
XYZZ<typename C::Base> ones_finish(const void* pinned);

}
```

### vimz_amd/csrc/msm_inst_bn254_g1.hip

```cpp
#include "msm.hpp"
namespace vz {
template hipError_t msm_run<BnG1>(hipStream_t, MsmWorkspace&, const uint32_t*, const uint32_t*, size_t, int, int,
                                  Affine<BnG1::Base>*, MsmStats*, hipEvent_t*, int, const BaseTables*);
template hipError_t msm_launch<BnG1>(hipStream_t, MsmWorkspace&, const uint32_t*, const uint32_t*, size_t, int, int, void*, MsmPlan*, hipEvent_t*, int, const BaseTables*);
template hipError_t build_tables<BnG1>(hipStream_t, const uint32_t*, size_t, int, int, uint32_t*);
template hipError_t build_multiples<BnG1>(hipStream_t, const uint32_t*, size_t, int, int, uint32_t*);
template Affine<BnG1::Base> msm_finish<BnG1>(const MsmPlan&, const void*);
template hipError_t ones_launch<BnG1>(hipStream_t, MsmWorkspace&, const uint32_t*, const uint32_t*, size_t, int, void*);
template XYZZ<BnG1::Base> ones_finish<BnG1>(const void*);
template hipError_t msm_launch_rows<BnG1>(hipStream_t, MsmWorkspace&, const uint32_t*, const uint32_t*, size_t, size_t, uint32_t, int, void*, size_t, MsmPlan*, int, const BaseTables*,
                                          const OnesDesc*, uint32_t, uint32_t);
template size_t msm_rows_row_bytes<BnG1>(size_t, int, const BaseTables*);
template hipError_t ones_launch_rows<BnG1>(hipStream_t, MsmWorkspace&, const OnesDesc*, uint32_t, int);
}
```

### vimz_amd/csrc/prover.hip

```cpp
#include "prover_internal.hpp"

HostPool& vz_shared_pool() {
  static HostPool* pool = [] { const unsigned hw = usable_cpus(); return new HostPool(hw > 2 ? std::min(15u, hw - 2) : 0u); }();
  return *pool;
}

std::atomic<long>& vz_head_rows_override() { static std::atomic<long> v{-1}; return v; }
std::atomic<long>& vz_rows_group_override() { static std::atomic<long> v{-1}; return v; }

extern "C" {

void vimz_prover_free(vimz_prover* p) {
  if (!p) return;
  if (p->ctx) {
    std::lock_guard<std::mutex> g(p->ctx->mu);
    hipSetDevice(p->ctx->device);
    hipStreamSynchronize(p->ctx->stream);
    { int lo = 0, hi = 0; hipDeviceGetStreamPriorityRange(&lo, &hi); vz_stream_release(p->ctx, lo, p->sB); vz_stream_release(p->ctx, lo, p->sH); }
    if (p->ev_head) hipEventDestroy(p->ev_head);
    if (p->ev_hash) hipEventDestroy(p->ev_hash);
    p->wsH.release();
    if (p->stage_host) hipHostFree(p->stage_host);
    if (p->jobvals_host) hipHostFree(p->jobvals_host);
    if (p->zs_host) hipHostFree(p->zs_host);
    hipFree(p->stage_d); hipFree(p->jobvals_d);
    for (auto& bb : p->buf) {
      for (auto e : bb.ev) hipEventDestroy(e);
      if (bb.wit_done) hipEventDestroy(bb.wit_done);
      for (auto e : bb.ev_p) hipEventDestroy(e);
      for (auto e : bb.ev_d) hipEventDestroy(e);
      if (bb.pin_d) hipHostFree(bb.pin_d);
      if (bb.pin) hipHostFree(bb.pin);
      if (bb.status_host) hipHostFree(bb.status_host);
      if (bb.row_flag) hipHostFree(bb.row_flag);
    }
    p->wsB.release();
    hipFree(p->priv_all_d); hipFree(p->zs_all_d); hipFree(p->job_all_d);
    for (void* d : p->retired) hipFree(d);
    for (void* d : p->owned) hipFree(d);
  }
  delete p;
}

int vimz_prover_create(vimz_ctx* ctx, const vimz_circuit* circuit, const vimz_bases* ck, size_t max_batch, vimz_prover** out) {
  return vz_prover_create_layout(ctx, circuit, ck, max_batch, 0, 0, 0, out);
}
}

int vz_prover_create_layout(vimz_ctx* ctx, const vimz_circuit* circuit, const vimz_bases* ck, size_t max_batch, int ivc, uint32_t step_wires, uint32_t step_c, vimz_prover** out) {
  if (!ctx || !circuit || !ck || !out || max_batch == 0) return vz_fail(ctx, VIMZ_ERR_INVALID, "vimz_prover_create: bad argument");
  if (ck->curve != VIMZ_CURVE_BN254_G1) return vz_fail(ctx, VIMZ_ERR_INVALID, "vimz_prover_create: the step circuits are over BN254 Fr; the key must be on BN254 G1");
  const cb::Builder& b = circuit->build->b;
  const uint32_t c0 = ivc ? 1u : 1 + 2 * b.len_z;
  const uint32_t n_aux = ivc ? b.n_wires - 3 : b.n_wires - 1 - 2 * b.len_z;
  if (ck->n < n_aux || ck->n < b.n_constraints()) return vz_fail(ctx, VIMZ_ERR_INVALID, "vimz_prover_create: commitment key shorter than max(witness, constraints)");
  for (auto& J : b.jobs) if (J.t != 3 && J.t != 9) return vz_fail(ctx, VIMZ_ERR_INVALID, "vimz_prover_create: the GPU Poseidon kernel supports widths 3 and 9 only (row widths must be multiples of 8... of the window fold)");
  std::lock_guard<std::mutex> g(ctx->mu);
  P_TRY(hipSetDevice(ctx->device));
  auto* p = new vimz_prover();
  p->ctx = ctx; p->circuit = circuit; p->ck = ck; p->max_batch = max_batch;
  static const bool dbg_create = getenv("VIMZ_DEBUG_TIMING") != nullptr;
  double t_c = now_s();
  auto lap = [&](const char* what) { if (dbg_create) { const double t = now_s(); fprintf(stderr, "[timing] prover_create(%p): %s %.1f ms\n", (void*)ctx, what, 1e3 * (t - t_c)); t_c = t; } };
  p->n_wires = b.n_wires; p->n_c = b.n_constraints(); p->len_z = b.len_z; p->n_priv = b.n_priv; p->n_aux = n_aux;
  p->n_jobs = (uint32_t)b.jobs.size(); p->n_fops = (uint32_t)b.fops.size();
  p->ivc = ivc != 0; p->c0 = c0; p->step_wires = ivc ? step_wires : b.n_wires; p->step_c = ivc ? step_c : b.n_constraints();
  p->n_bool = std::min<uint32_t>(b.n_bool, p->step_c);
  auto fail_free = [&](const char* what, hipError_t e) { for (void* d : p->owned) hipFree(d); delete p; return vz_fail(ctx, VIMZ_ERR_HIP, what, e); };
  hipError_t e;
#define UP(vec, dst) do { e = upload(vec, &dst); if (dst) p->owned.push_back((void*)dst); if (e != hipSuccess) return fail_free("upload " #vec, e); } while (0)
  UP(b.A.row_ptr, p->A.row_ptr); UP(b.A.col, p->A.col); UP(b.A.coef, p->A.coef);
  UP(b.B.row_ptr, p->B.row_ptr); UP(b.B.col, p->B.col); UP(b.B.coef, p->B.coef);
  UP(b.C.row_ptr, p->C.row_ptr); UP(b.C.col, p->C.col); UP(b.C.coef, p->C.coef);
  { const Fe* d = nullptr; const std::vector<Fe> dd = dict_for_device(b.dict); UP(dd, d); p->dict = (const uint32_t*)d; }
  {
    std::vector<uint32_t> items, items_aug;
    const cb::Csr* Ms[3] = {&b.A, &b.B, &b.C};
    for (uint32_t m = 0; m < 3; m++)
      for (uint32_t r = 0; r + 1 < Ms[m]->row_ptr.size(); r++)
        if (Ms[m]->row_ptr[r + 1] - Ms[m]->row_ptr[r] > SPMV_LONG) (r < p->step_c ? items : items_aug).push_back((m << 30) | r);
    auto terms = [&](uint32_t it) { const cb::Csr* M = Ms[it >> 30]; const uint32_t r = it & 0x3fffffffu; return M->row_ptr[r + 1] - M->row_ptr[r]; };
    p->n_med = spmv_sort_items(items, terms); p->n_med_aug = spmv_sort_items(items_aug, terms);
    p->n_long = (uint32_t)items.size(); p->n_long_aug = (uint32_t)items_aug.size();
    UP(items, p->long_items); UP(items_aug, p->long_items_aug);
  }
  lap("CSR + dictionary uploads");
  WitnessDev& W = p->wd;
  UP(b.decomp, W.decomp); UP(b.lane_groups, W.groups); UP(b.lane_instr, W.instr); UP(b.lane_rows, W.rows);
  UP(b.jobs, W.jobs); UP(b.chains, W.chains); UP(b.fops, W.fops); UP(b.lc_terms, W.lc_terms);
  W.dict = p->dict;
  W.n_decomp = (uint32_t)b.decomp.size(); W.n_groups = (uint32_t)b.lane_groups.size(); W.n_jobs = p->n_jobs;
// ... 23 lines not shown
      const uint32_t* w;
      const std::vector<uint32_t> c29 = to29(t == 3 ? t3.C : t9.C), m29 = to29(t == 3 ? t3.M : t9.M), s29 = to29(packed), f29 = to29(S.Pfin);
      UP(c29, w); (t == 3 ? W.pc3_29 : W.pc9_29) = w;
      UP(m29, w); (t == 3 ? W.pm3_29 : W.pm9_29) = w;
      UP(s29, w); (t == 3 ? W.ps3_29 : W.ps9_29) = w;
      UP(f29, w); (t == 3 ? W.pf3_29 : W.pf9_29) = w;
    }
    W.poseidon29 = getenv("VIMZ_DEBUG_POSEIDON_STD") ? 0u : 1u;
  }
#undef UP
  lap("witness program + Poseidon tables");
  auto dalloc = [&](uint32_t** dst, size_t bytes) { e = hipMalloc((void**)dst, bytes ? bytes : 32); if (e == hipSuccess) { p->owned.push_back(*dst); e = hipMemset(*dst, 0, bytes ? bytes : 32); } return e; };
  const size_t B = max_batch;
  if (dalloc(&p->priv_d, 32 * B * p->n_priv) != hipSuccess || dalloc(&p->zs_d, 32 * (B + 1) * p->len_z) != hipSuccess ||
      dalloc(&p->Z_d, 32 * B * (size_t)p->n_wires) != hipSuccess || dalloc(&p->job_out_d, 32 * B * (size_t)(p->n_jobs + p->n_fops)) != hipSuccess ||
      dalloc(&p->status_d, 4 * B) != hipSuccess || dalloc(&p->Zrun, 32 * (size_t)p->n_wires) != hipSuccess ||
      dalloc(&p->E, 32 * (size_t)p->n_c) != hipSuccess || dalloc(&p->AZ, 32 * (size_t)p->n_c) != hipSuccess ||
      dalloc(&p->BZ, 32 * (size_t)p->n_c) != hipSuccess || dalloc(&p->CZ, 32 * (size_t)p->n_c) != hipSuccess ||
      dalloc(&p->T, 32 * (size_t)p->n_c) != hipSuccess || dalloc(&p->az2, 32 * (size_t)p->n_c) != hipSuccess ||
      dalloc(&p->bz2, 32 * (size_t)p->n_c) != hipSuccess || dalloc(&p->cz2, 32 * (size_t)p->n_c) != hipSuccess ||
      dalloc(&p->bad_d, 64) != hipSuccess)
    return fail_free("device allocation", e);
  lap("device buffers (running instance, batch 0)");
  { int lo = 0, hi = 0; hipDeviceGetStreamPriorityRange(&lo, &hi);
    if ((e = vz_stream_acquire(ctx, lo, &p->sB)) != hipSuccess) return fail_free("stream", e); }
  for (int k = 0; k < 2; k++) {
    auto& bb = p->buf[k];
    if (k == 0) { bb.Z = p->Z_d; bb.job_out = p->job_out_d; bb.status = p->status_d; }
    else if (dalloc(&bb.Z, 32 * B * (size_t)p->n_wires) != hipSuccess || dalloc(&bb.job_out, 32 * B * (size_t)(p->n_jobs + p->n_fops)) != hipSuccess ||
             dalloc(&bb.status, 4 * B) != hipSuccess) return fail_free("device allocation", e);
    if (dalloc(&bb.az, 32 * B * (size_t)p->n_c) != hipSuccess || dalloc(&bb.bz, 32 * B * (size_t)p->n_c) != hipSuccess ||
        dalloc(&bb.cz, 32 * B * (size_t)p->n_c) != hipSuccess) return fail_free("device allocation", e);
    bb.ev.resize(B);
    for (size_t i = 0; i < B; i++) if ((e = hipEventCreateWithFlags(&bb.ev[i], hipEventDisableTiming)) != hipSuccess) return fail_free("event", e);
    if ((e = hipEventCreateWithFlags(&bb.wit_done, hipEventDisableTiming)) != hipSuccess) return fail_free("event", e);
    if ((e = hipHostMalloc(&bb.pin, 4 * (size_t)XYZZ_WORDS * MSM_MAX_WINDOWS * B)) != hipSuccess) return fail_free("pinned", e);
    if ((e = hipHostMalloc((void**)&bb.status_host, 4 * B)) != hipSuccess) return fail_free("pinned", e);
    if ((e = hipHostMalloc((void**)&bb.row_flag, 8 * B)) != hipSuccess) return fail_free("pinned", e);
    memset(bb.row_flag, 0, 8 * B); bb.flag_rows = B;
    bb.has_d.assign(B, 0);
    if (p->ivc) {
      bb.ev_p.resize(B);
      for (size_t i = 0; i < B; i++) if ((e = hipEventCreateWithFlags(&bb.ev_p[i], hipEventDisableTiming)) != hipSuccess) return fail_free("event", e);
    }
    if (p->ivc && ivc_lookahead_enabled()) {
      if (dalloc(&bb.d, 32 * B * (size_t)p->step_c) != hipSuccess) return fail_free("device allocation", e);
      if ((e = hipHostMalloc(&bb.pin_d, 4 * (size_t)XYZZ_WORDS * MSM_MAX_WINDOWS * B)) != hipSuccess) return fail_free("pinned", e);
      bb.ev_d.resize(B);
      for (size_t i = 0; i < B; i++) if ((e = hipEventCreateWithFlags(&bb.ev_d[i], hipEventDisableTiming)) != hipSuccess) return fail_free("event", e);
    }
  }
  lap("batch buffers, events, pinned");
  {
    int lo = 0, hi = 0; hipDeviceGetStreamPriorityRange(&lo, &hi);
    if ((e = vz_stream_acquire(ctx, lo, &p->sH)) != hipSuccess) return fail_free("stream", e);
    p->sD = p->sH;
    if ((e = hipEventCreateWithFlags(&p->ev_head, hipEventDisableTiming)) != hipSuccess || (e = hipEventCreateWithFlags(&p->ev_hash, hipEventDisableTiming)) != hipSuccess)
      return fail_free("event", e);
    const cb::PoseidonTable& t3 = cb::poseidon_table(3); const cb::PoseidonTable& t9 = cb::poseidon_table(9);
    p->job_stage_off.assign(1, 0); p->job_fold_mask.clear();
    for (auto& J : b.jobs) {
      uint32_t mask = 0, nonconst = 0;
      for (uint32_t i = 0; i + 1 < J.t; i++) { if (J.in[i].kind == REF_CONST_ZERO) mask |= 1u << (i + 1); else nonconst++; }
      p->job_fold_mask.push_back(mask);
      p->job_stage_off.push_back(p->job_stage_off.back() + cb::poseidon_job_wire_count((int)J.t, J.t == 3 ? t3.rp : t9.rp, nonconst, J.out_wire != 0));
    }
    e = upload(p->job_stage_off, &p->job_stage_off_d); if (p->job_stage_off_d) p->owned.push_back((void*)p->job_stage_off_d);
    if (e != hipSuccess) return fail_free("upload job layout", e);
    bool ok = !b.jobs.empty() && b.gpu_witness && !b.zout.empty();
    for (auto& c : b.chains) ok = ok && c.phase <= 1;
    for (auto& f : b.fops) ok = ok && !f.early && f.op != FOP_LC;
    p->head_eligible = ok;
  }
  if ((e = hipStreamSynchronize(nullptr)) != hipSuccess) return fail_free("sync", e);
  lap("head-batch layout + sync of the fills");
  p->z_cur.assign(p->len_z, Fe::zero()); p->z0 = p->z_cur;
  *out = p;
  return VIMZ_OK;
}

extern "C" {
long vimz_set_head_rows(long rows) { return vz_head_rows_override().exchange(rows < 0 ? -1 : rows); }
long vimz_set_rows_group(long rows) { return vz_rows_group_override().exchange(rows < 0 ? -1 : rows); }

int vimz_prover_reset(vimz_prover* p, const uint64_t* z0) {
  if (!p || !z0) return VIMZ_ERR_INVALID;
  vimz_ctx* ctx = p->ctx;
  std::lock_guard<std::mutex> g(ctx->mu);
  P_TRY(hipSetDevice(ctx->device));
  for (uint32_t i = 0; i < p->len_z; i++) p->z_cur[i] = fe_from_canon(z0 + 4 * i);
  p->steps = 0; p->u = Fe::zero();
  p->comm_W.x = Fq::zero(); p->comm_W.y = Fq::zero(); p->comm_E = p->comm_W;
  Fe seed[6] = {cb::fe_from_u64(0x56494d7a), cb::fe_from_u64(p->n_c), cb::fe_from_u64(p->n_wires), cb::fe_from_u64(p->len_z),
                cb::fe_from_u64((uint64_t)p->circuit->transformation), cb::fe_from_u64((uint64_t)p->circuit->shape.width)};
  p->ro = cb::poseidon_hash(seed, 6);
  prover_start_state_changed(p);
  memset(p->phase_s, 0, sizeof(p->phase_s)); memset(p->phase_n, 0, sizeof(p->phase_n));
  P_TRY(hipMemsetAsync(p->Zrun, 0, 32 * (size_t)p->n_wires, ctx->stream));
  P_TRY(hipMemsetAsync(p->E, 0, 32 * (size_t)p->n_c, ctx->stream));
  P_TRY(hipMemsetAsync(p->AZ, 0, 32 * (size_t)p->n_c, ctx->stream));
  P_TRY(hipMemsetAsync(p->BZ, 0, 32 * (size_t)p->n_c, ctx->stream));
  P_TRY(hipMemsetAsync(p->CZ, 0, 32 * (size_t)p->n_c, ctx->stream));
  P_TRY(hipStreamSynchronize(ctx->stream));
  return VIMZ_OK;
}

static int witness_batch_locked(vimz_prover* p, const uint64_t* inputs, size_t rows, std::vector<Fe>& zs) {
  vimz_ctx* ctx = p->ctx;
  hipStream_t s = ctx->stream;
  FoldJob job; job.step_inputs = inputs; job.nsteps = rows;
  int rc = fold_prepare(p, job);
  if (rc) return rc;
  zs = job.zs;
  double t0 = now_s();
  P_TRY(hipMemsetAsync(p->status_d, 0, 4 * rows, s));
  if ((rc = launch_witness(p, s, p->Z_d, p->job_out_d, p->status_d, p->priv_all_d, 0, rows, job, false))) return rc;
  p->last_status.assign(rows, 0);
  P_TRY(hipMemcpyAsync(p->last_status.data(), p->status_d, 4 * rows, hipMemcpyDeviceToHost, s));
  P_TRY(hipStreamSynchronize(s));
  p->phase_s[PH_WITNESS] += now_s() - t0;
  return VIMZ_OK;
}

int vimz_prover_witness(vimz_prover* p, const uint64_t* inputs, size_t rows, uint64_t* z_wires_out, uint64_t* zs_out, uint32_t* status_out) {
  if (!p || !inputs || rows == 0 || rows > p->max_batch) return vz_fail(p ? p->ctx : nullptr, VIMZ_ERR_INVALID, "vimz_prover_witness: bad argument");
  if (!p->circuit->build->b.gpu_witness || p->circuit->build->b.zout.empty()) return vz_fail(p->ctx, VIMZ_ERR_INVALID, "vimz_prover_witness: this circuit has no GPU witness program");
  vimz_ctx* ctx = p->ctx;
  std::lock_guard<std::mutex> g(ctx->mu);
  P_TRY(hipSetDevice(ctx->device));
  std::vector<Fe> zs;
  int rc = witness_batch_locked(p, inputs, rows, zs);
  if (rc) return rc;
  if (zs_out) for (size_t i = 0; i < zs.size(); i++) fe_to_canon(zs[i], zs_out + 4 * i);
  if (status_out) memcpy(status_out, p->last_status.data(), 4 * rows);
  if (z_wires_out) {
    const size_t n = rows * (size_t)p->n_wires;
    rc = vz_ensure_scratch(ctx, 32 * n); if (rc) return rc;
    launch_from_mont<Fr>(ctx->stream, p->Z_d, (uint32_t*)ctx->scratch, n);
    P_TRY(hipMemcpyAsync(z_wires_out, ctx->scratch, 32 * n, hipMemcpyDeviceToHost, ctx->stream));
    P_TRY(hipStreamSynchronize(ctx->stream));
  }
  return VIMZ_OK;
}

int vimz_prover_spmv(vimz_prover* p, const uint64_t* z, uint64_t* az, uint64_t* bz, uint64_t* cz) {
  if (!p || !z || !az || !bz || !cz) return VIMZ_ERR_INVALID;
  vimz_ctx* ctx = p->ctx;
  std::lock_guard<std::mutex> g(ctx->mu);
  P_TRY(hipSetDevice(ctx->device));
  hipStream_t s = ctx->stream;
  int rc = vz_ensure_scratch(ctx, 32 * (size_t)p->n_wires); if (rc) return rc;
  uint32_t* zd = (uint32_t*)ctx->scratch;
  P_TRY(hipMemcpyAsync(zd, z, 32 * (size_t)p->n_wires, hipMemcpyHostToDevice, s));
  launch_to_mont<Fr>(s, zd, p->n_wires);
  launch_spmv(p, s, zd, p->az2, p->bz2, p->cz2);
  uint32_t* src[3] = {p->az2, p->bz2, p->cz2}; uint64_t* dst[3] = {az, bz, cz};
  for (int m = 0; m < 3; m++) {
    launch_from_mont<Fr>(s, src[m], p->T, p->n_c);
    P_TRY(hipMemcpyAsync(dst[m], p->T, 32 * (size_t)p->n_c, hipMemcpyDeviceToHost, s));
    P_TRY(hipStreamSynchronize(s));
  }
  return VIMZ_OK;
}

static void ro_absorb_point(const G1Aff& pt, Fe* out2) {
  Fq xc = Fq::from_mont(pt.x), yc = Fq::from_mont(pt.y);
// ... 452 lines not shown
```

### vimz_amd/csrc/prover_internal.hpp

```cpp
#pragma once
#include <hip/hip_runtime.h>
#include <atomic>
#include <chrono>
#include <condition_variable>
#include <cstdio>
#include <cstring>
#include <functional>
#include <memory>
#include <string>
#include <thread>
#include <vector>
#include <algorithm>

#include "internal.hpp"
#include "circuit_handle.hpp"
#include "r1cs_ops.hpp"
#include "witness.hpp"
#include "aug/cs.hpp"

using namespace vz;
typedef cb::Fe Fe;
typedef Fp<BnFq> Fq;
typedef Affine<Fq> G1Aff;
typedef XYZZ<Fq> G1;
// ... 326 lines not shown

struct FoldJob {
  int started_batch = -1;
  const uint64_t* step_inputs = nullptr;
  const uint64_t* witnesses = nullptr;
  size_t nsteps = 0;
  std::vector<Fe> zs;
  size_t nbatches = 0;
  std::vector<size_t> bfirst, brows;
  size_t first(size_t k) const { return bfirst[k]; }
  size_t rows(size_t k) const { return brows[k]; }
  uint32_t nA = 0, nB = 0, nE = 0;
  bool early_fops = false;
  size_t pre_rows = 0;
  BaseTables tbl{};
  bool head = false;
  size_t next_issue = 0;
  std::thread helper; std::atomic<size_t> states_upto{0};
  std::atomic<int> helper_done{1}; int helper_rc = VIMZ_OK; std::string helper_err;
  std::vector<Fe> jobA_rest;
  ~FoldJob() { if (helper.joinable()) helper.join(); }
  static constexpr size_t pin_stride = 4 * (size_t)XYZZ_WORDS * MSM_MAX_WINDOWS;
};

static int launch_witness(vimz_prover* p, hipStream_t st, uint32_t* Z, uint32_t* job_out, uint32_t* status, const uint32_t* priv, size_t first, size_t rows,
                          const FoldJob& J, bool ahead, int part = 0) {
  vimz_ctx* ctx = p->ctx;
  const cb::Builder& b = p->circuit->build->b;
  const WitnessDev& W = p->wd;
  const unsigned R = (unsigned)rows;
  auto chain_wires_std = [&](uint32_t phase) {
    if (W.poseidon29 && p->n_jobs) hipLaunchKernelGGL(k_wit_chain_wires_std, dim3(p->n_jobs, R), dim3(128), 0, st, W, p->job_stage_off_d, phase, Z);
  };
  if (part != 2)
    for (uint32_t gI = 0; gI < W.n_decomp; gI++) {
      const uint32_t total = (b.decomp[gI].nbits - 1) * b.decomp[gI].count;
      hipLaunchKernelGGL(k_wit_decomp, dim3((total + 255) / 256, R), dim3(256), 0, st, W, gI, priv, Z, status);
    }
  hipLaunchKernelGGL(k_wit_inputs, dim3(((1 + 2 * p->len_z + p->n_priv) + 255) / 256, R), dim3(256), 0, st, W, priv, (const uint32_t*)p->zs_all_d, Z, (uint32_t)first);
  if (part == 1) {
    hipLaunchKernelGGL(k_wit_chains, dim3((J.nA + 3) / 4, R), dim3(64), 0, st, W, 0u, Z, job_out, (const uint32_t*)nullptr);
    chain_wires_std(0u);
    P_TRY(hipGetLastError());
    return VIMZ_OK;
  }
  for (uint32_t gI = 0; gI < W.n_groups; gI++)
    hipLaunchKernelGGL(k_wit_lanes, dim3((b.lane_groups[gI].lanes + LANE_TB - 1) / LANE_TB, R), dim3(LANE_TB), 0, st, W, gI, priv, (const uint32_t*)p->zs_all_d, (uint32_t)first, Z, status);
  if (J.nA && !ahead && part != 2) { hipLaunchKernelGGL(k_wit_chains, dim3((J.nA + 3) / 4, R), dim3(64), 0, st, W, 0u, Z, job_out, (const uint32_t*)nullptr); chain_wires_std(0u); }
  if (J.early_fops) {
    hipLaunchKernelGGL(k_wit_fops_lc, dim3(p->n_fops, R), dim3(64), 0, st, W, (const uint32_t*)Z, job_out, 1u);
    hipLaunchKernelGGL(k_wit_fops, dim3((R + 63) / 64), dim3(64), 0, st, W, Z, job_out, (uint32_t)rows, 1u);
  }
  if (J.nE) { hipLaunchKernelGGL(k_wit_chains, dim3((J.nE + 3) / 4, R), dim3(64), 0, st, W, 2u, Z, job_out, (const uint32_t*)nullptr); chain_wires_std(2u); }
  if (!ahead) {
    if (J.nB) { hipLaunchKernelGGL(k_wit_chains, dim3((J.nB + 3) / 4, R), dim3(64), 0, st, W, 1u, Z, job_out, (const uint32_t*)nullptr); chain_wires_std(1u); }
    if (p->n_fops) hipLaunchKernelGGL(k_wit_fops, dim3((R + 63) / 64), dim3(64), 0, st, W, Z, job_out, (uint32_t)rows, 0u);
  }
  P_TRY(hipGetLastError());
  return VIMZ_OK;
}

static void plan_batches(FoldJob& J, size_t first, size_t n, size_t B) {
  if (!n) return;
  const size_t nb = (n + B - 1) / B, per = (n + nb - 1) / nb;
  for (size_t off = 0; off < n; off += per) { J.bfirst.push_back(first + off); J.brows.push_back(std::min(per, n - off)); }
}

template <int DUMMY>
__global__ void k_row_flag(uint32_t* flag, uint32_t v) { __hip_atomic_store(flag, v, __ATOMIC_RELEASE, __HIP_MEMORY_SCOPE_SYSTEM); }
template <int DUMMY>
__global__ void k_row_flags(uint32_t* flag, uint32_t v, uint32_t n) { if (threadIdx.x < n) __hip_atomic_store(flag + threadIdx.x, v, __ATOMIC_RELEASE, __HIP_MEMORY_SCOPE_SYSTEM); }
static inline hipError_t mark_row(hipStream_t st, vimz_prover::BatchBuf& bb, size_t idx) {
  hipLaunchKernelGGL(k_row_flag<0>, dim3(1), dim3(1), 0, st, bb.row_flag + idx, bb.gen);
  return hipGetLastError();
}
std::atomic<long>& vz_rows_group_override();
constexpr size_t ROWS_GROUP_DEFAULT = 4, ROWS_GROUP_BYTES_MAX = (size_t)2 << 30;
static size_t rows_group_wanted() {
  static const long env = [] { const char* e = getenv("VIMZ_TUNE"); const char* q = e ? strstr(e, "rows_group=") : nullptr; return q ? atol(q + 11) : -1L; }();
  const long ov = vz_rows_group_override().load(std::memory_order_relaxed);
  const long v = ov >= 0 ? ov : env >= 0 ? env : (long)ROWS_GROUP_DEFAULT;
  return (size_t)std::min<long>(v, (long)MSM_ROWS_MAX);
}
static inline hipError_t wait_row_flag(const vimz_prover::BatchBuf& bb, size_t idx, hipEvent_t ev) {
  const uint32_t want = bb.gen;
  const uint32_t* f = bb.row_flag + idx;
  double t_start = 0;
  for (uint32_t spins = 1; __atomic_load_n(f, __ATOMIC_ACQUIRE) != want; spins++) {
    if (spins & 31) continue;
    std::this_thread::yield();
    if ((spins & 0x3ffff) == 0) {
      const hipError_t q = hipEventQuery(ev);
      if (q == hipSuccess) break;
      if (q != hipErrorNotReady) return q;
      if (t_start == 0) t_start = now_s(); else if (now_s() - t_start > 120.0) return hipErrorNotReady;
    }
  }
  return hipSuccess;
}
static int fold_issue(vimz_prover* p, const FoldJob& J, size_t k);

static bool getenv_once(const char* name) {
  static std::mutex m; static std::vector<std::pair<std::string, bool>> seen;
  std::lock_guard<std::mutex> g(m);
  for (auto& e : seen) if (e.first == name) return e.second;
  seen.emplace_back(name, getenv(name) != nullptr);
  return seen.back().second;
}
static unsigned usable_cpus() {
  static const unsigned v = [] {
    unsigned n = aug::affinity_cpus();
    if (FILE* f = fopen("/sys/fs/cgroup/cpu.max", "r")) {
      char q[32] = {0}; long per = 0;
      if (fscanf(f, "%31s %ld", q, &per) == 2 && strcmp(q, "max") != 0 && per > 0) { const long k = atol(q) / per; if (k >= 1) n = std::min<unsigned>(n, (unsigned)k); }
      fclose(f);
    } else if (FILE* g = fopen("/sys/fs/cgroup/cpu/cpu.cfs_quota_us", "r")) {
      long quota = -1, per = 100000;
      if (fscanf(g, "%ld", &quota) != 1) quota = -1;
      fclose(g);
      if (FILE* h = fopen("/sys/fs/cgroup/cpu/cpu.cfs_period_us", "r")) { if (fscanf(h, "%ld", &per) != 1) per = 100000; fclose(h); }
      if (quota > 0 && per > 0 && quota / per >= 1) n = std::min<unsigned>(n, (unsigned)(quota / per));
    }
    const bool bound = aug::affinity_cpus() < std::max(1u, std::thread::hardware_concurrency());
    if (const char* lw = getenv("LOCAL_WORLD_SIZE")) { const long k = atol(lw); if (k > 1 && !bound) n = std::max(1u, n / (unsigned)k); }
    return n;
  }();
  return v;
}

static inline hipError_t vz_wait_stream(hipStream_t s) { return hipStreamSynchronize(s); }
static inline hipError_t vz_wait_event(hipEvent_t e) { return hipEventSynchronize(e); }

std::atomic<long>& vz_head_rows_override();
constexpr size_t HEAD_CALL_MAX = 24;
constexpr size_t HEAD_JOB_MAX = 28;
static size_t head_rows_wanted(size_t nsteps = 0) {
  static const long env = getenv("VIMZ_HEAD_ROWS") ? atol(getenv("VIMZ_HEAD_ROWS")) : -1;
  const long ov = vz_head_rows_override().load(std::memory_order_relaxed);
  if (ov >= 0) return (size_t)ov;
  if (env >= 0) return (size_t)env;
  static const bool few_cores = usable_cpus() < 6;
  if (few_cores) return 0;
  return nsteps == 0 || nsteps <= HEAD_CALL_MAX ? 24 : 0;
}

static bool ivc_lookahead_enabled() { static const bool v = getenv("VIMZ_IVC_LOOKAHEAD") && atoi(getenv("VIMZ_IVC_LOOKAHEAD")) != 0; return v; }

static int fold_issue_d(vimz_prover* p, const FoldJob& J, size_t k, size_t r, hipStream_t sp, MsmWorkspace& ws) {
  vimz_ctx* ctx = p->ctx;
  auto& bb = p->buf[k & 1];
  bb.has_d[r] = 0;
  if (!p->want_d) return VIMZ_OK;
  const size_t nc = p->n_c, sc = p->step_c;
  const uint32_t *az0, *bz0, *cz0; hipEvent_t prev;
  if (r > 0) { az0 = bb.az + 8 * (r - 1) * nc; bz0 = bb.bz + 8 * (r - 1) * nc; cz0 = bb.cz + 8 * (r - 1) * nc; prev = bb.ev_p[r - 1]; }
  else if (k > 0) { auto& ob = p->buf[(k - 1) & 1]; const size_t lr = J.rows(k - 1) - 1; az0 = ob.az + 8 * lr * nc; bz0 = ob.bz + 8 * lr * nc; cz0 = ob.cz + 8 * lr * nc; prev = ob.ev_p[lr]; }
  else return VIMZ_OK;
  P_TRY(hipStreamWaitEvent(sp, prev, 0));
  uint32_t* d = bb.d + 8 * r * sc;
  hipLaunchKernelGGL(k_fresh_cross_neg<Fr>, dim3(stream_grid(sc)), dim3(256), 0, sp, sc, az0, bz0, cz0, bb.az + 8 * r * nc, bb.bz + 8 * r * nc, bb.cz + 8 * r * nc, d);
  P_TRY(hipGetLastError());
  P_TRY(msm_launch<BnG1>(sp, ws, p->ck->d, d, sc, 1, 0, (char*)bb.pin_d + r * FoldJob::pin_stride, &p->planD, nullptr, 1, nullptr));
  P_TRY(mark_row(sp, bb, bb.flag_rows + r));
  P_TRY(hipEventRecord(bb.ev_d[r], sp));
  bb.has_d[r] = 1;
  return VIMZ_OK;
// ... 401 lines not shown
```

### vimz_amd/csrc/r1cs_capi.hip

```cpp
#include <hip/hip_runtime.h>
#include <array>
#include <cstring>
#include <memory>
#include <new>
#include <unordered_map>
#include <vector>

#include "internal.hpp"
#include "r1cs_ops.hpp"

using namespace vz;

struct vimz_r1cs {
  int field = 0;
  size_t nrows = 0, ncols = 0, nnz[3] = {0, 0, 0};
  CsrDev M[3] = {};
  uint32_t* dict = nullptr; size_t ndict = 0;
  uint32_t* long_items = nullptr; uint32_t n_long = 0, n_med = 0;
  uint32_t* scratch = nullptr;
  std::vector<void*> owned;
};

#define R_TRY(x) do { hipError_t _e = (x); if (_e != hipSuccess) return vz_fail(ctx, VIMZ_ERR_HIP, #x, _e); } while (0)

namespace {

struct KeyHash {
  size_t operator()(const std::array<uint64_t, 4>& k) const { return (size_t)(k[0] * 0x9e3779b97f4a7c15ull ^ (k[1] + 0x7f4a7c15ull) * 0xff51afd7ed558ccdull ^ k[2] * 0xc4ceb9fe1a85ec53ull ^ k[3]); }
};

template <class F>
int upload_shape(vimz_ctx* ctx, vimz_r1cs* S, const uint32_t* const rows[3], const uint32_t* const cols[3], const uint64_t* const vals[3], const size_t nnz[3], int form) {
  const size_t nr = S->nrows;
  std::unordered_map<std::array<uint64_t, 4>, uint32_t, KeyHash> index;
  std::vector<F> dict;
  std::vector<uint32_t> items;
  for (int m = 0; m < 3; m++) {
    std::vector<uint32_t> row_ptr(nr + 1, 0), col(nnz[m]), coef(nnz[m]);
    for (size_t k = 0; k < nnz[m]; k++) {
      if (rows[m][k] >= nr || cols[m][k] >= S->ncols) return vz_fail(ctx, VIMZ_ERR_INVALID, "vimz_r1cs_upload: triplet outside the shape");
      row_ptr[rows[m][k] + 1]++;
    }
    for (size_t r = 0; r < nr; r++) row_ptr[r + 1] += row_ptr[r];
    std::vector<uint32_t> cur(row_ptr.begin(), row_ptr.end() - 1);
    for (size_t k = 0; k < nnz[m]; k++) {
      std::array<uint64_t, 4> key; memcpy(key.data(), vals[m] + 4 * k, 32);
      auto it = index.find(key);
      uint32_t id;
      if (it == index.end()) {
        F v; memcpy(v.v, key.data(), 32);
        if (!v.is_reduced()) return vz_fail(ctx, VIMZ_ERR_INVALID, "vimz_r1cs_upload: coefficient not below the modulus");
        id = (uint32_t)dict.size();
        dict.push_back(form == VIMZ_FORM_CANONICAL ? F::to_mont(v) : v);
        index.emplace(key, id);
      } else id = it->second;
      const uint32_t pos = cur[rows[m][k]]++;
      col[pos] = cols[m][k]; coef[pos] = id;
    }
    for (size_t r = 0; r < nr; r++) if (row_ptr[r + 1] - row_ptr[r] > SPMV_LONG) items.push_back(((uint32_t)m << 30) | (uint32_t)r);
    auto up = [&](const std::vector<uint32_t>& v, const uint32_t** dst) -> hipError_t {
      uint32_t* d = nullptr;
      hipError_t e = hipMalloc((void**)&d, 4 * std::max<size_t>(v.size(), 1));
      if (e != hipSuccess) return e;
      S->owned.push_back(d);
      *dst = d;
      return v.empty() ? hipSuccess : hipMemcpy(d, v.data(), 4 * v.size(), hipMemcpyHostToDevice);
    };
    R_TRY(up(row_ptr, &S->M[m].row_ptr)); R_TRY(up(col, &S->M[m].col)); R_TRY(up(coef, &S->M[m].coef));
    S->nnz[m] = nnz[m];
  }
  {
    std::vector<std::vector<uint32_t>> cnt(3, std::vector<uint32_t>(nr, 0));
    for (int m = 0; m < 3; m++) for (size_t k = 0; k < nnz[m]; k++) cnt[m][rows[m][k]]++;
    S->n_med = spmv_sort_items(items, [&](uint32_t it) { return cnt[it >> 30][it & 0x3fffffffu]; });
  }
  S->n_long = (uint32_t)items.size();
  if (!items.empty()) {
    R_TRY(hipMalloc((void**)&S->long_items, 4 * items.size())); S->owned.push_back(S->long_items);
    R_TRY(hipMemcpy(S->long_items, items.data(), 4 * items.size(), hipMemcpyHostToDevice));
  }
  S->ndict = dict.size();
  const std::vector<F> dd = dict_for_device(dict);
  R_TRY(hipMalloc((void**)&S->dict, 32 * std::max<size_t>(dd.size(), 1))); S->owned.push_back(S->dict);
  if (!dd.empty()) R_TRY(hipMemcpy(S->dict, dd.data(), 32 * dd.size(), hipMemcpyHostToDevice));
  R_TRY(hipMalloc((void**)&S->scratch, 32 * 6 * std::max<size_t>(nr, 1))); S->owned.push_back(S->scratch);
  return VIMZ_OK;
}

template <class F>
void spmv3(const vimz_r1cs* S, hipStream_t s, const uint32_t* z, uint32_t* az, uint32_t* bz, uint32_t* cz) {
  hipLaunchKernelGGL(k_spmv3<F>, dim3(stream_grid(3 * S->nrows)), dim3(256), 0, s, S->M[0], S->M[1], S->M[2], (const uint32_t*)S->dict, S->nrows, z, az, bz, cz);
  if (S->n_long)
// ... 186 lines not shown

int vimz_test_fp29_probe(vimz_ctx* ctx, int field, int op, const uint32_t* a, const uint32_t* b, const uint32_t* c, const uint32_t* d, uint32_t* out, size_t n) {
  if (!ctx || !a || !b || !c || !d || !out || field < 0 || field > 3) return vz_fail(ctx, VIMZ_ERR_INVALID, "vimz_test_fp29_probe: bad argument");
  {
    uint32_t zero[FP29_PROBE_WORDS] = {}, r[FP29_PROBE_WORDS];
    if (fp29_probe<BnFr>(op, zero, zero, zero, zero, r)) return vz_fail(ctx, VIMZ_ERR_INVALID, "vimz_test_fp29_probe: unknown operation");
  }
  if (!n) return VIMZ_OK;
  std::lock_guard<std::mutex> g(ctx->mu);
  R_TRY(hipSetDevice(ctx->device));
  const size_t bytes = 4 * (size_t)FP29_PROBE_WORDS * n;
  uint32_t* buf = nullptr;
  R_TRY(hipMalloc((void**)&buf, 5 * bytes));
  const uint32_t* src[4] = {a, b, c, d};
  hipError_t e = hipSuccess;
  for (int k = 0; k < 4 && e == hipSuccess; k++) e = hipMemcpyAsync((char*)buf + k * bytes, src[k], bytes, hipMemcpyHostToDevice, ctx->stream);
  if (e == hipSuccess) {
    uint32_t* p = buf; const size_t w = (size_t)FP29_PROBE_WORDS * n;
    fp29_probe_field(field, [&](auto pp) {
      typedef decltype(pp) P;
      hipLaunchKernelGGL(k_fp29_probe<P>, dim3(stream_grid(n)), dim3(256), 0, ctx->stream, op, (const uint32_t*)p, (const uint32_t*)(p + w), (const uint32_t*)(p + 2 * w), (const uint32_t*)(p + 3 * w), p + 4 * w, n);
      return 0;
    });
    e = hipGetLastError();
  }
  if (e == hipSuccess) e = hipMemcpyAsync(out, (char*)buf + 4 * bytes, bytes, hipMemcpyDeviceToHost, ctx->stream);
  const hipError_t e2 = hipStreamSynchronize(ctx->stream);
  hipFree(buf);
  if (e != hipSuccess) return vz_fail(ctx, VIMZ_ERR_HIP, "vimz_test_fp29_probe", e);
  if (e2 != hipSuccess) return vz_fail(ctx, VIMZ_ERR_HIP, "vimz_test_fp29_probe: synchronize", e2);
  return VIMZ_OK;
}

int vimz_test_spmv_cross16(vimz_ctx* ctx, const vimz_r1cs* S, size_t row0, size_t nrows, const vimz_vec* z, vimz_vec* az, vimz_vec* bz, vimz_vec* cz,
                           const vimz_vec* az1, const vimz_vec* bz1, const vimz_vec* cz1, const uint64_t u1[4], const uint64_t u2[4], int form, vimz_vec* T) {
  if (!ctx || !S || !z || !az || !bz || !cz || !u1 || !u2) return vz_fail(ctx, VIMZ_ERR_INVALID, "vimz_test_spmv_cross16: bad argument");
  if (az1 && (!bz1 || !cz1 || !T)) return vz_fail(ctx, VIMZ_ERR_INVALID, "vimz_test_spmv_cross16: a running instance needs all of az1, bz1, cz1 and T");
  if (row0 > S->nrows || nrows > S->nrows - row0) return vz_fail(ctx, VIMZ_ERR_INVALID, "vimz_test_spmv_cross16: rows outside the shape");
  const vimz_vec* vs[7] = {az, bz, cz, az1, bz1, cz1, T};
  for (const vimz_vec* v : vs) if (v && (v->field != S->field || v->n < S->nrows)) return vz_fail(ctx, VIMZ_ERR_INVALID, "vimz_test_spmv_cross16: field or length of a vector does not fit the shape");
  if (z->field != S->field || z->n < S->ncols) return vz_fail(ctx, VIMZ_ERR_INVALID, "vimz_test_spmv_cross16: z does not fit the shape");
  if (!nrows) return VIMZ_OK;
  std::lock_guard<std::mutex> g(ctx->mu);
  R_TRY(hipSetDevice(ctx->device));
  int rc = field_dispatch(S->field, [&](auto f) {
    typedef decltype(f) F;
    F a, b; int r;
    if ((r = scalar_arg(ctx, u1, form, &a, "vimz_test_spmv_cross16: u1 not below the modulus")) || (r = scalar_arg(ctx, u2, form, &b, "vimz_test_spmv_cross16: u2 not below the modulus"))) return r;
    hipLaunchKernelGGL(k_spmv_cross16<F>, dim3((unsigned)((16 * nrows + 255) / 256)), dim3(256), 0, ctx->stream, S->M[0], S->M[1], S->M[2], (const uint32_t*)S->dict, (uint32_t)row0, (uint32_t)nrows,
                       (const uint32_t*)z->d, az->d, bz->d, cz->d, az1 ? (const uint32_t*)az1->d : (const uint32_t*)nullptr, bz1 ? (const uint32_t*)bz1->d : (const uint32_t*)nullptr,
                       cz1 ? (const uint32_t*)cz1->d : (const uint32_t*)nullptr, a, b, T ? T->d : (uint32_t*)nullptr);
    return VIMZ_OK;
  });
  if (rc) return rc;
  R_TRY(hipGetLastError());
  R_TRY(hipStreamSynchronize(ctx->stream));
  return VIMZ_OK;
}

int vimz_test_cross_term_masked(vimz_ctx* ctx, size_t n, const vimz_vec* az1, const vimz_vec* bz1, const vimz_vec* cz1, const uint64_t u1[4], const vimz_vec* az2, const vimz_vec* bz2,
                                const vimz_vec* cz2, const uint64_t u2[4], int form, vimz_vec* T, vimz_vec* Tm, size_t nb) {
  if (!ctx || !az1 || !bz1 || !cz1 || !az2 || !bz2 || !cz2 || !u1 || !u2 || !T) return vz_fail(ctx, VIMZ_ERR_INVALID, "vimz_test_cross_term_masked: bad argument");
  const vimz_vec* vs[8] = {az1, bz1, cz1, az2, bz2, cz2, T, Tm};
  for (const vimz_vec* v : vs) if (v && (v->field != T->field || v->n < n)) return vz_fail(ctx, VIMZ_ERR_INVALID, "vimz_test_cross_term_masked: field or length of a vector");
  if (nb > n || n >= (1ull << 32)) return vz_fail(ctx, VIMZ_ERR_INVALID, "vimz_test_cross_term_masked: nb beyond n");
  if (T == Tm) return vz_fail(ctx, VIMZ_ERR_INVALID, "vimz_test_cross_term_masked: T and Tm must differ");
  if (!n) return VIMZ_OK;
  std::lock_guard<std::mutex> g(ctx->mu);
  R_TRY(hipSetDevice(ctx->device));
  int rc = field_dispatch(T->field, [&](auto f) {
    typedef decltype(f) F;
    F a, b; int r;
    if ((r = scalar_arg(ctx, u1, form, &a, "vimz_test_cross_term_masked: u1 not below the modulus")) || (r = scalar_arg(ctx, u2, form, &b, "vimz_test_cross_term_masked: u2 not below the modulus"))) return r;
    hipLaunchKernelGGL(k_cross_term<F>, dim3(stream_grid(n)), dim3(256), 0, ctx->stream, n, (const uint32_t*)az1->d, (const uint32_t*)bz1->d, (const uint32_t*)cz1->d, a,
                       (const uint32_t*)az2->d, (const uint32_t*)bz2->d, (const uint32_t*)cz2->d, b, T->d, Tm ? Tm->d : (uint32_t*)nullptr, (uint32_t)nb);
    return VIMZ_OK;
  });
  if (rc) return rc;
  R_TRY(hipGetLastError());
  R_TRY(hipStreamSynchronize(ctx->stream));
  return VIMZ_OK;
}

}
#endif
```

### vimz_amd/csrc/r1cs_ops.hpp

```cpp
#pragma once
#include <hip/hip_runtime.h>
#include <algorithm>
#include <vector>
#include "vecops.hpp"
#include "fp29.hpp"

namespace vz {

struct CsrDev { const uint32_t* row_ptr; const uint32_t* col; const uint32_t* coef; };

template <class F>
inline std::vector<F> dict_for_device(const std::vector<F>& dict) {
  std::vector<F> out(2 * dict.size());
  for (size_t i = 0; i < dict.size(); i++) { F t = dict[i]; out[2 * i] = t; for (int k = 0; k < 5; k++) t = F::dbl(t); out[2 * i + 1] = t; }
  return out;
}

constexpr uint32_t SPMV_LONG = 6;

template <class F>
__device__ __forceinline__ void spmv_term(R29<F>& acc, const uint32_t* __restrict__ dict, uint32_t coef, const uint32_t* __restrict__ z, uint32_t col) {
  const F v = load_fe<F>(z, col);
  const bool zr = v.is_zero(), on = v.eq(F::one());
  if (__ballot(!zr) == 0ull) return;
// ... 94 lines not shown
                                                      const uint32_t* __restrict__ az1, const uint32_t* __restrict__ bz1, const uint32_t* __restrict__ cz1, F u1, F u2,
                                                      uint32_t* __restrict__ T) {
  VZ_SET_CRIT_PRIO();
  const uint32_t g = (blockIdx.x * blockDim.x + threadIdx.x) >> 4, l = threadIdx.x & 15u;
  const bool live = g < nrows;
  const uint32_t r = row0 + (live ? g : 0u);
  R29<F> acc[3];
#pragma unroll
  for (int m = 0; m < 3; m++) {
    const CsrDev M = m == 0 ? A : (m == 1 ? B : C);
    acc[m] = R29<F>::zero();
    if (live) {
      const uint32_t lo = M.row_ptr[r], hi = M.row_ptr[r + 1];
      for (uint32_t k0 = lo + l; k0 < hi; k0 += 64) {
        uint32_t col[4], cf[4];
#pragma unroll
        for (int j = 0; j < 4; j++) { const uint32_t kk = k0 + 16u * j; const bool on = kk < hi; col[j] = on ? M.col[kk] : 0xffffffffu; cf[j] = on ? M.coef[kk] : 0u; }
        F v[4], c[4];
#pragma unroll
        for (int j = 0; j < 4; j++) { v[j] = col[j] != 0xffffffffu ? load_fe<F>(z, col[j]) : F::zero(); c[j] = load_fe<F>(dict, 2 * (size_t)cf[j]); }
#pragma unroll
        for (int j = 0; j < 4; j++) {
          const bool zr = v[j].is_zero(), on = v[j].eq(F::one());
          if (__ballot(!zr) == 0ull) continue;
          F t = c[j];
          const bool cp = t.eq(F::one()), cm = t.eq(F::neg(F::one()));
          if (!on && cp) t = v[j];
          if (!on && cm) t = F::neg(v[j]);
          R29<F> term = R29<F>::pack(t.v);
          if (__ballot(!(zr || on || cp || cm)) != 0ull) {
            const R29<F> mm = R29<F>::mul(R29<F>::pack(load_fe<F>(dict, 2 * (size_t)cf[j] + 1).v), R29<F>::pack(v[j].v));
            if (!(on || cp || cm)) term = mm;
          }
          if (!zr) acc[m] = R29<F>::add(acc[m], term);
        }
        acc[m] = acc[m].weak_reduce();
      }
    }
  }
#pragma unroll
  for (int m = 0; m < 3; m++) {
#pragma unroll
    for (int off = 8; off >= 1; off >>= 1) spmv_exchange_add<F>(acc[m], off);
    acc[m] = acc[m].weak_reduce().canon();
  }
  if (!live || l != 0) return;
  F a2, b2, c2;
  acc[0].unpack(a2.v); acc[1].unpack(b2.v); acc[2].unpack(c2.v);
  store_fe(az, r, a2); store_fe(bz, r, b2); store_fe(cz, r, c2);
  if (!az1) return;
  typedef R29<F> G;
  const G t1 = G::mul_add2(r29_of<F>(load_fe<F>(az1, r)), acc[1], acc[0], r29_of<F>(load_fe<F>(bz1, r)));
  const F c1 = load_fe<F>(cz1, r);
  G t2;
  if (u2.eq(F::one())) t2 = G::add(G::mul(r29_of<F>(u1), acc[2]), G::pack(c1.v));
  else t2 = G::mul_add2(r29_of<F>(u1), acc[2], r29_of<F>(u2), G::pack(c1.v));
  store_fe(T, r, fe_of29<F>(G::template sub<3>(t1, t2)));
}

template <class F>
__device__ __forceinline__ F bool_row_masked(const F& t, const F& a, const F& az_fresh) {
  const bool z = az_fresh.is_zero(), o = az_fresh.eq(F::one());
  F r = F::zero();
  if (o) r = F::dbl(t);
  if (!z && !o) r = F::add(t, a);
  return r;
}
template <class F>
__global__ void __launch_bounds__(256) k_cross_term(size_t n, const uint32_t* __restrict__ az1, const uint32_t* __restrict__ bz1, const uint32_t* __restrict__ cz1, F u1,
                                                    const uint32_t* __restrict__ az2, const uint32_t* __restrict__ bz2, const uint32_t* __restrict__ cz2, F u2,
                                                    uint32_t* __restrict__ T, uint32_t* __restrict__ Tm = nullptr, uint32_t nb = 0) {
  VZ_GRID_STRIDE(i, n) {
    const F a1 = load_fe<F>(az1, i), a2 = load_fe<F>(az2, i);
    F t = mul_fresh(a1, load_fe<F>(bz2, i));
    t = F::add(t, mul_fresh(load_fe<F>(bz1, i), a2));
    t = F::sub(t, mul_fresh(u1, load_fe<F>(cz2, i)));
    t = F::sub(t, mul_fresh(load_fe<F>(cz1, i), u2));
    store_fe(T, i, t);
    if (Tm) store_fe(Tm, i, i < nb ? bool_row_masked(t, a1, a2) : t);
  }
}

template <class F>
__global__ void __launch_bounds__(256) k_fold_cross(size_t n, uint32_t* __restrict__ AZ, uint32_t* __restrict__ BZ, uint32_t* __restrict__ CZ, uint32_t* __restrict__ E,
                                                    const uint32_t* Tin, int fold_E, F r, int hasB, F r_prev, const uint32_t* __restrict__ negB, F u1_new,
                                                    const uint32_t* __restrict__ az, const uint32_t* __restrict__ bz, const uint32_t* __restrict__ cz,
                                                    uint32_t* out, const uint32_t* __restrict__ azn, const uint32_t* __restrict__ bzn, const uint32_t* __restrict__ czn, F u2,
                                                    uint32_t* __restrict__ outm = nullptr, uint32_t nb = 0) {
  VZ_GRID_STRIDE(i, n) {
    const F a = F::add(load_fe<F>(AZ, i), mul_fresh(r, load_fe<F>(az, i)));
    const F b = F::add(load_fe<F>(BZ, i), mul_fresh(r, load_fe<F>(bz, i)));
    const F c = F::add(load_fe<F>(CZ, i), mul_fresh(r, load_fe<F>(cz, i)));
    store_fe(AZ, i, a); store_fe(BZ, i, b); store_fe(CZ, i, c);
    if (fold_E) {
      F t = load_fe<F>(Tin, i);
      if (hasB) t = F::sub(t, mul_fresh(r_prev, load_fe<F>(negB, i)));
      if (__ballot(!t.is_zero()) != 0ull) { const F e = F::add(load_fe<F>(E, i), F::mul(r, t)); if (!t.is_zero()) store_fe(E, i, e); }
    }
    if (out) {
      const F an = load_fe<F>(azn, i);
      F t = mul_fresh(a, load_fe<F>(bzn, i));
      t = F::add(t, mul_fresh(b, an));
      t = F::sub(t, mul_fresh(u1_new, load_fe<F>(czn, i)));
      t = F::sub(t, mul_fresh(c, u2));
      store_fe(out, i, t);
      if (outm) store_fe(outm, i, i < nb ? bool_row_masked(t, a, an) : t);
    }
  }
}

template <class F>
__global__ void __launch_bounds__(256) k_fresh_cross_neg(size_t n, const uint32_t* __restrict__ az0, const uint32_t* __restrict__ bz0, const uint32_t* __restrict__ cz0,
                                                         const uint32_t* __restrict__ az1, const uint32_t* __restrict__ bz1, const uint32_t* __restrict__ cz1,
                                                         uint32_t* __restrict__ out) {
  VZ_GRID_STRIDE(i, n) {
    F t = F::add(load_fe<F>(cz0, i), load_fe<F>(cz1, i));
    t = F::sub(t, F::mul(load_fe<F>(az0, i), load_fe<F>(bz1, i)));
    t = F::sub(t, F::mul(load_fe<F>(az1, i), load_fe<F>(bz0, i)));
    store_fe(out, i, t);
  }
}

template <class F>
__global__ void __launch_bounds__(256) k_axpy_inplace(size_t n, uint32_t* __restrict__ x1, F r, const uint32_t* __restrict__ x2) {
  VZ_GRID_STRIDE(i, n) store_fe(x1, i, F::add(load_fe<F>(x1, i), F::mul(r, load_fe<F>(x2, i))));
}

static __global__ void __launch_bounds__(256) k_copy16(uint4* __restrict__ dst, const uint4* __restrict__ src, size_t n16) {
  VZ_GRID_STRIDE(i, n16) dst[i] = src[i];
}
static __global__ void __launch_bounds__(256) k_copy4(uint32_t* __restrict__ dst, const uint32_t* __restrict__ src, size_t n4) {
  VZ_GRID_STRIDE(i, n4) dst[i] = src[i];
}
static inline hipError_t copy_pinned(hipStream_t s, void* dst, const void* src, size_t bytes) {
  if (!bytes) return hipSuccess;
  if ((bytes & 15) || (((uintptr_t)dst | (uintptr_t)src) & 15)) {
    if (bytes & 3) return hipErrorInvalidValue;
    hipLaunchKernelGGL(k_copy4, dim3((unsigned)std::min<size_t>(1024, (bytes / 4 + 255) / 256)), dim3(256), 0, s, (uint32_t*)dst, (const uint32_t*)src, bytes / 4);
    return hipGetLastError();
  }
  const size_t n16 = bytes / 16;
  hipLaunchKernelGGL(k_copy16, dim3((unsigned)std::min<size_t>(1024, (n16 + 255) / 256)), dim3(256), 0, s, (uint4*)dst, (const uint4*)src, n16);
  return hipGetLastError();
}
static inline hipError_t upload_pinned(hipStream_t s, void* dst, const void* src_pinned, size_t bytes) { return copy_pinned(s, dst, src_pinned, bytes); }

struct Fold5 { uint32_t* x1[5]; const uint32_t* x2[5]; size_t n[5]; };
template <class F>
__global__ void __launch_bounds__(256) k_fold5(Fold5 a, F r) {
#pragma unroll 1
  for (int v = 0; v < 5; v++) {
    uint32_t* x1 = a.x1[v]; const uint32_t* x2 = a.x2[v];
    if (!x1) continue;
    VZ_GRID_STRIDE(i, a.n[v]) {
      const F y = load_fe<F>(x2, i);
      if (!y.is_zero()) store_fe(x1, i, F::add(load_fe<F>(x1, i), mul_fresh(r, y)));
    }
  }
}

template <class F>
__global__ void __launch_bounds__(256) k_check_relaxed(size_t n, const uint32_t* __restrict__ az, const uint32_t* __restrict__ bz, const uint32_t* __restrict__ cz,
                                                       F u, const uint32_t* __restrict__ E, uint32_t* __restrict__ bad ) {
  VZ_GRID_STRIDE(i, n) {
    F lhs = F::mul(load_fe<F>(az, i), load_fe<F>(bz, i));
    F rhs = F::mul(u, load_fe<F>(cz, i));
    if (E) rhs = F::add(rhs, load_fe<F>(E, i));
    if (!lhs.eq(rhs)) { atomicAdd(&bad[0], 1u); atomicMin(&bad[1], (uint32_t)i); }
  }
}

static __global__ void __launch_bounds__(256) k_count_diff(size_t n, const uint32_t* __restrict__ a, const uint32_t* __restrict__ b, uint32_t* __restrict__ bad) {
  VZ_GRID_STRIDE(i, n) {
    uint32_t d = 0;
#pragma unroll
    for (int k = 0; k < 8; k++) d |= a[8 * i + k] ^ b[8 * i + k];
    if (d) atomicAdd(&bad[0], 1u);
  }
}

template <class F>
__global__ void __launch_bounds__(256) k_count_unreduced(size_t n, const uint32_t* __restrict__ a, uint32_t* __restrict__ bad) {
  VZ_GRID_STRIDE(i, n) {
    F x = load_fe<F>(a, i);
    if (!x.is_reduced()) atomicAdd(&bad[0], 1u);
  }
}

}
```

### vimz_amd/hip.py

```python
import ctypes as C

import numpy as np

from . import _lib as L


def _ptr(a):
    return a.ctypes.data_as(C.c_void_p) if a is not None else None


def _u64(a):
    return np.ascontiguousarray(a, dtype=np.uint64)


class DeviceVec:
    def __init__(self, ctx, handle, field, n):
        self.ctx, self.h, self.field, self.n = ctx, handle, field, n

    def upload(self, host, offset=0, form=L.FORM_CANONICAL):
        host = _u64(host)
        self.ctx._chk(self.ctx.lib.vimz_vec_upload(self.ctx.h, self.h, offset, _ptr(host), host.size // 4, form))
        return self

    def download(self, offset=0, n=None, form=L.FORM_CANONICAL):
# ... 722 lines not shown
        n = lib.vimz_cf_proof_size(self.h)
        buf = np.zeros(n, dtype=np.uint8)
        self.ctx._chk(lib.vimz_cf_proof_export(self.h, _ptr(buf), n))
        return buf

    def proof_import(self, blob):
        lib = self.ctx.lib
        lib.vimz_cf_proof_import.argtypes = [C.c_void_p, C.c_void_p, C.c_size_t]
        b = np.ascontiguousarray(blob, dtype=np.uint8)
        self.ctx._chk(lib.vimz_cf_proof_import(self.h, _ptr(b), b.size))


def cyclefold_selfcheck_last_step(steps=4):
    from . import _lib
    lib = _lib.testing_lib()
    lib.vimz_cf_selfcheck_last_step.argtypes = [C.c_int, C.c_void_p, C.c_size_t]
    lib.vimz_cf_selfcheck_last_step.restype = C.c_int64
    n = lib.vimz_cf_selfcheck_last_step(int(steps), None, 0)
    if n < 0:
        raise _lib.VimzError(int(n), "vimz_cf_selfcheck_last_step")
    buf = np.zeros(n // 8, dtype=np.uint64)
    assert lib.vimz_cf_selfcheck_last_step(int(steps), _ptr(buf), n) == n
    ints = lambda a: sum(int(a[k]) << (64 * k) for k in range(4))
    return ints(buf[0:4]), ints(buf[4:8]), buf[8:]


def cyclefold_selfcheck_merge(segs_run0=3, segs_run1=2):
    from . import _lib
    lib = _lib.testing_lib()
    lib.vimz_cf_selfcheck_merge.argtypes = [C.c_int, C.c_int, C.c_void_p, C.c_size_t]
    lib.vimz_cf_selfcheck_merge.restype = C.c_int64
    n = lib.vimz_cf_selfcheck_merge(segs_run0, segs_run1, None, 0)
    if n < 0:
        raise _lib.VimzError(int(n), "vimz_cf_selfcheck_merge")
    buf = np.zeros(n // 8, dtype=np.uint64)
    assert lib.vimz_cf_selfcheck_merge(segs_run0, segs_run1, _ptr(buf), n) == n
    w = [int(x) for x in buf]
    el = lambda pos: sum(w[pos + k] << (64 * k) for k in range(4))
    dg, nrec = el(0), w[4]
    rec = buf[5:5 + nrec]
    pos = 5 + nrec
    acc = {"n": w[pos], "zs": [el(pos + 1)], "ze": [el(pos + 5)]}
    pos += 9
    vals = [el(pos + 4 * k) for k in range(7 + 12)]
    acc["P"] = [(vals[0], vals[1]), (vals[2], vals[3]), vals[4], vals[5], vals[6]]
    acc["Q"] = [(vals[7], vals[8]), (vals[9], vals[10]), vals[11], vals[12:19]]
    return dg, rec, acc


def kzg_setup(ctx, n, seed=None):
    vp = C.c_void_p
    h = vp()
    vk = np.zeros((4, 4), dtype=np.uint64)
    if seed is None:
        ctx.lib.vimz_kzg_setup.argtypes = [vp, C.c_size_t, C.POINTER(vp), vp]
        ctx._chk(ctx.lib.vimz_kzg_setup(ctx.h, n, C.byref(h), _ptr(vk)))
    else:
        fn = _seeded(ctx, "vimz_testing_kzg_setup_seeded")
        fn.argtypes = [vp, C.c_char_p, C.c_size_t, C.c_size_t, C.POINTER(vp), vp]
        ctx._chk(fn(ctx.h, bytes(seed), len(seed), n, C.byref(h), _ptr(vk)))
    return Bases(ctx, h, L.CURVE_BN254_G1, n), vk


def _seeded(ctx, name):
    if not hasattr(ctx.lib, name):
        raise RuntimeError(f"{name} exists only in libvimz_hip_testing.so (start the process with VIMZ_HIP_LIBRARY=testing): seeded setups are test hooks")
    return getattr(ctx.lib, name)


def set_head_rows(rows):
    lib = L.lib()
    lib.vimz_set_head_rows.argtypes = [C.c_long]
    lib.vimz_set_head_rows.restype = C.c_long
    return int(lib.vimz_set_head_rows(int(rows)))


def set_rows_group(rows):
    lib = L.lib()
    lib.vimz_set_rows_group.argtypes = [C.c_long]
    lib.vimz_set_rows_group.restype = C.c_long
    return int(lib.vimz_set_rows_group(int(rows)))


class Decider:
    RESULT_BITS = {1: "fewer than two steps", 2: "KZG opening of cmW", 4: "KZG opening of cmE", 8: "Groth16", 16: "a word pair is not a curve point"}

    def __init__(self, prover, kzg_vk=None, seed=None, light=False):
        self.prover, self.ctx = prover, prover.ctx
        self.light = bool(light)
        lib = self.ctx.lib
        vp = C.c_void_p
        lib.vimz_decider_setup.argtypes = [vp, vp, C.c_int, C.POINTER(vp), C.POINTER(C.c_double)]
        lib.vimz_decider_free.argtypes = [vp]
        lib.vimz_decider_free.restype = None
        lib.vimz_decider_info.argtypes = [vp, vp]
        lib.vimz_decider_vk.argtypes = [vp, vp, C.c_size_t]
        lib.vimz_decider_vk.restype = C.c_int64
        lib.vimz_decider_prove.argtypes = [vp, vp, vp, vp, C.POINTER(C.c_double)]
        lib.vimz_decider_verify.argtypes = [vp, C.c_uint64, vp, vp, vp, C.POINTER(C.c_uint32)]
        h = vp()
        sec = (C.c_double * 4)()
        self._kzg_vk = None if kzg_vk is None else np.ascontiguousarray(kzg_vk, dtype=np.uint64)
        kp = None if self._kzg_vk is None else _ptr(self._kzg_vk)
        if seed is None:
            self.ctx._chk(lib.vimz_decider_setup(prover.h, kp, int(self.light), C.byref(h), sec))
        else:
            fn = _seeded(self.ctx, "vimz_testing_decider_setup_seeded")
            fn.argtypes = [vp, vp, C.c_int, C.c_char_p, C.c_size_t, C.POINTER(vp), C.POINTER(C.c_double)]
            self.ctx._chk(fn(prover.h, kp, int(self.light), bytes(seed), len(seed), C.byref(h), sec))
        self.h = h
        self.setup_seconds = {"circuit_synthesis": sec[0], "qap_at_trapdoor_host": sec[1], "key_points_gpu": sec[2], "total": sec[3]}

    def close(self):
        if self.h:
            self.ctx.lib.vimz_decider_free(self.h)
            self.h = None

    def save_key(self):
        lib = self.ctx.lib
        lib.vimz_decider_key_save.argtypes = [C.c_void_p, C.c_void_p, C.c_size_t]
        lib.vimz_decider_key_save.restype = C.c_int64
        n = lib.vimz_decider_key_save(self.h, None, 0)
        if n < 0:
            self.ctx._chk(int(n))
        buf = np.zeros(n, dtype=np.uint8)
        got = lib.vimz_decider_key_save(self.h, _ptr(buf), n)
        if got != n:
            self.ctx._chk(int(got) if got < 0 else L.ERR_INVALID)
        return buf

    @classmethod
    def load_key(cls, prover, blob):
        d = cls.__new__(cls)
        d.prover, d.ctx = prover, prover.ctx
        lib = d.ctx.lib
        vp = C.c_void_p
        lib.vimz_decider_key_load.argtypes = [vp, vp, C.c_size_t, C.POINTER(vp)]
        lib.vimz_decider_free.argtypes = [vp]
        lib.vimz_decider_free.restype = None
        lib.vimz_decider_info.argtypes = [vp, vp]
        lib.vimz_decider_vk.argtypes = [vp, vp, C.c_size_t]
        lib.vimz_decider_vk.restype = C.c_int64
        lib.vimz_decider_prove.argtypes = [vp, vp, vp, vp, C.POINTER(C.c_double)]
        lib.vimz_decider_verify.argtypes = [vp, C.c_uint64, vp, vp, vp, C.POINTER(C.c_uint32)]
        b = np.ascontiguousarray(blob, dtype=np.uint8)
        h = vp()
        d.ctx._chk(lib.vimz_decider_key_load(prover.h, _ptr(b), b.size, C.byref(h)))
        d.h = h
        d._kzg_vk = None
        d.setup_seconds = {"circuit_synthesis": 0.0, "qap_at_trapdoor_host": 0.0, "key_points_gpu": 0.0, "total": 0.0}
        return d

    def info(self):
        a = np.zeros(8, dtype=np.uint64)
        self.ctx._chk(self.ctx.lib.vimz_decider_info(self.h, _ptr(a)))
        return dict(zip(["constraints", "wires", "public_inputs", "domain", "nnz_a", "nnz_b", "nnz_c", "cyclefold_rows"], (int(x) for x in a[:8])))

    def key_words(self):
        return _export(self.ctx.lib.vimz_decider_vk, self.h).view(np.uint64)

    def verifying_key(self):
        return parse_verifying_key(self.key_words())

    def prove(self, ivc=None):
        ivc = self.prover if ivc is None else ivc
        n_pub = self.info()["public_inputs"]
# ... 546 lines not shown
```

Baseline: 1437.

## Fuse MSM digit histogram into the fold/cross-term kernel

Adds a fused kernel that computes the folded R1CS rows and cross term and, in the same pass, builds the MSM bucket histogram (and optionally the scan) in LDS. The following commitment MSM then skips its own histogram pass over the scalars. This saves one full read of the scalar vector and a kernel launch per fold step. In exchange it uses 1024-thread blocks with large dynamic LDS for the fold arithmetic, which may lower occupancy. The path is gated by a fused-sort mode setting and only runs when there are no helper devices.

```diff
diff --git a/include/vimz_hip.h b/include/vimz_hip.h
--- a/include/vimz_hip.h
+++ b/include/vimz_hip.h
@@ -41,6 +41,7 @@
 int vimz_trace_marker(vimz_ctx* ctx, int id);
 long vimz_set_head_rows(long rows);
 long vimz_set_rows_group(long rows);
+long vimz_set_fused_sort(long mode);
 int vimz_host_fingerprint(vimz_ctx* ctx, double out[4]);
 int vimz_timer_start(vimz_ctx* ctx);
 int vimz_timer_stop(vimz_ctx* ctx, float* ms_out);
diff --git a/include/vimz_hip_testing.h b/include/vimz_hip_testing.h
--- a/include/vimz_hip_testing.h
+++ b/include/vimz_hip_testing.h
@@ -24,6 +24,10 @@
                                 const vimz_vec* bz2, const vimz_vec* cz2, const uint64_t u2[4], int form, vimz_vec* T, vimz_vec* Tm, size_t nb);
 int vimz_test_msm_rows(vimz_ctx* ctx, const vimz_bases* bases, const uint64_t* scalars, size_t n, size_t row_stride, size_t G, int form, int use_tables,
                        size_t n_ones, int calls, uint64_t* out_xy, uint64_t* s1_xy, uint64_t* s1_ref_xy);
+int vimz_test_fold_cross_msm(vimz_ctx* ctx, const vimz_bases* bases, int use_tables, size_t n, vimz_vec* AZ, vimz_vec* BZ, vimz_vec* CZ, vimz_vec* E, const vimz_vec* Tin,
+                             const vimz_vec* az, const vimz_vec* bz, const vimz_vec* cz, const vimz_vec* azn, const vimz_vec* bzn, const vimz_vec* czn, const uint64_t r[4],
+                             const uint64_t u[4], int form, size_t nb, int fold_E, int mode, vimz_vec* out, vimz_vec* outm, uint64_t commit_xy[8]);
+int vimz_test_msm_counted_refusal(vimz_ctx* ctx, const vimz_bases* bases, int use_tables, size_t n, size_t G, int* hip_error);
 
 #ifdef __cplusplus
 }
diff --git a/vimz_amd/csrc/fold_hist.hpp b/vimz_amd/csrc/fold_hist.hpp
--- /dev/null
+++ b/vimz_amd/csrc/fold_hist.hpp
@@ -0,0 +1,62 @@
+#pragma once
+#include <mutex>
+#include "msm_api.hpp"
+#include "msm_digits.hpp"
+#include "r1cs_ops.hpp"
+
+namespace vz {
+
+template <class F, class S>
+__global__ void __launch_bounds__(SORT_THREADS) k_fold_cross_hist(size_t n, uint32_t* __restrict__ AZ, uint32_t* __restrict__ BZ, uint32_t* __restrict__ CZ, uint32_t* __restrict__ E,
+                                                                  const uint32_t* Tin, int fold_E, F r, int hasB, F r_prev, const uint32_t* __restrict__ negB, F u1_new,
+                                                                  const uint32_t* __restrict__ az, const uint32_t* __restrict__ bz, const uint32_t* __restrict__ cz,
+                                                                  uint32_t* out, const uint32_t* __restrict__ azn, const uint32_t* __restrict__ bzn, const uint32_t* __restrict__ czn, F u2,
+                                                                  uint32_t* __restrict__ outm, uint32_t nb_bool, MsmPrehist h) {
+  static_assert(sizeof(F) == sizeof(S), "the vector's elements are the MSM's scalars");
+  extern __shared__ uint32_t lds_cnt[];
+  __shared__ uint32_t s_last;
+  for (uint32_t g = threadIdx.x; g < h.nb; g += SORT_THREADS) lds_cnt[g] = 0;
+  __syncthreads();
+  const SortRange rows = sort_range(n, gridDim.x, blockIdx.x);
+  for (size_t i = rows.lo + threadIdx.x; i < rows.hi; i += SORT_THREADS) {
+    const F m = fold_cross_row<F>(i, AZ, BZ, CZ, E, Tin, fold_E, r, hasB, r_prev, negB, u1_new, az, bz, cz, out, azn, bzn, czn, u2, outm, nb_bool);
+    S x;
+#pragma unroll
+    for (int k = 0; k < 8; k++) x.v[k] = m.v[k];
+    uint32_t s[8], flip;
+    if (!scalar_of_word<S>(x, 1, 0, h.sgn, s, flip)) continue;
+    for_each_digit(s, h.c, h.K, flip, [&](int w, uint32_t b, uint32_t) { atomicAdd(&lds_cnt[(uint32_t)w * h.bstride + b], 1u); });
+  }
+  __syncthreads();
+  uint32_t* mine = h.block_hist + (size_t)blockIdx.x * h.nb;
+  for (uint32_t g = threadIdx.x; g < h.nb; g += SORT_THREADS) mine[g] = lds_cnt[g];
+  if (!h.scan) return;
+  __threadfence();
+  __syncthreads();
+  if (threadIdx.x == 0) s_last = atomicAdd(&h.totals[2], 1u) == gridDim.x - 1 ? 1u : 0u;
+  __syncthreads();
+  if (!s_last) return;
+  __threadfence();
+  if (threadIdx.x == 0) { __hip_atomic_store(&h.totals[2], 0u, __ATOMIC_RELAXED, __HIP_MEMORY_SCOPE_AGENT); h.heavy[0] = 0; }
+  for (uint32_t g = threadIdx.x; g < h.nb; g += SORT_THREADS) h.counts[g] = prefix_column<8>(h.block_hist, h.nb, gridDim.x, g);
+  __syncthreads();
+  scan_body(h.counts, h.nb, h.bucket_off, h.sub_off, h.totals, h.sub, h.heavy, h.heavy_min, h.heavy_cap);
+}
+
+template <class F, class S, class... Args>
+hipError_t launch_fold_cross_hist(hipStream_t stream, const MsmPrehist& h, Args... args) {
+  {
+    static uint64_t attr_devices = 0;
+    int dev = 0;
+    VZ_HIP_CHECK(hipGetDevice(&dev));
+    std::lock_guard<std::mutex> g(msm_sort_attr_mutex());
+    if (!((attr_devices >> (dev & 63)) & 1ull)) {
+      VZ_HIP_CHECK(hipFuncSetAttribute(reinterpret_cast<const void*>(&k_fold_cross_hist<F, S>), hipFuncAttributeMaxDynamicSharedMemorySize, 159 * 1024));
+      attr_devices |= 1ull << (dev & 63);
+    }
+  }
+  hipLaunchKernelGGL((k_fold_cross_hist<F, S>), dim3(h.sort_blocks), dim3(SORT_THREADS), (size_t)h.nb * 4, stream, args..., h);
+  return hipGetLastError();
+}
+
+}
diff --git a/vimz_amd/csrc/ivc.hip b/vimz_amd/csrc/ivc.hip
--- a/vimz_amd/csrc/ivc.hip
+++ b/vimz_amd/csrc/ivc.hip
@@ -1,4 +1,5 @@
 #include "ivc_internal.hpp"
+#include "fold_hist.hpp"
 
 namespace {
 
@@ -83,7 +84,7 @@
     for (int q : pend_slot) if (q >= 0) v->t1[q].ca_at = v->CA;
     pend_ca = false;
   };
-  auto queue_msm = [&](int par) -> int {
+  auto queue_msm = [&](int par, const MsmPrehist* counted = nullptr) -> int {
     auto& S = v->t1[par];
     const size_t parts = v->helpers.size() + 1, share = (sc + parts - 1) / parts;
     v->t1_main_n = std::min(share, sc);
@@ -101,8 +102,10 @@
       P_TRY(hipSetDevice(ctx->device));
     }
     double tq = now_s();
-    P_TRY(msm_launch<BnG1>(v->s3, v->ws3, p->ck->d, S.tricked ? S.bufm : S.buf, v->t1_main_n, 1, 0, S.pin, &S.plan, ctx->profiling ? S.ev : nullptr, 0,
-                           p->ck->tables && v->helpers.empty() ? &job.tbl : nullptr));
+    if (counted) P_TRY(msm_launch_counted<BnG1>(v->s3, v->ws3, p->ck->d, S.tricked ? S.bufm : S.buf, v->t1_main_n, S.pin, &S.plan, ctx->profiling ? S.ev : nullptr,
+                                                p->ck->tables ? &job.tbl : nullptr, *counted));
+    else P_TRY(msm_launch<BnG1>(v->s3, v->ws3, p->ck->d, S.tricked ? S.bufm : S.buf, v->t1_main_n, 1, 0, S.pin, &S.plan, ctx->profiling ? S.ev : nullptr, 0,
+                                p->ck->tables && v->helpers.empty() ? &job.tbl : nullptr));
     t_hk[2] += now_s() - tq; tq = now_s();
     if (ctx->profiling) P_TRY(hipMemcpyAsync(S.pin + v->pin_res, v->ws3.totals, 8, hipMemcpyDeviceToHost, v->s3));
     P_TRY(hipEventRecord(S.done, v->s3));
@@ -135,10 +138,22 @@
     double tq = now_s();
     if (t) P_TRY(wait_row_flag(*t->b, t->row, t->b->ev[t->row]));
     t_hk[4] += now_s() - tq; tq = now_s();
-    hipLaunchKernelGGL(k_fold_cross<Fr>, dim3(stream_grid(sc)), dim3(256), 0, v->s3, sc, p->AZ, p->BZ, p->CZ, p->E, (const uint32_t*)Scur.buf, fold_E ? 1 : 0, a.rho,
-                       hasB ? 1 : 0, v->rho_prev, hasB ? (const uint32_t*)(a.cur->d + 8 * a.r * sc) : (const uint32_t*)nullptr, v->u1_run, az, bz, cz,
-                       out, t ? t->b->az + 8 * t->row * nc : nullptr, t ? t->b->bz + 8 * t->row * nc : nullptr, t ? t->b->cz + 8 * t->row * nc : nullptr, Fe::one(),
-                       outm, p->n_bool);
+    const int fs = a.need1 && !a.look && a.i > 0 && v->helpers.empty() ? fused_sort_wanted() : 0;
+    MsmPrehist hist; bool counted = false;
+    if (fs) {
+      const hipError_t e = msm_prehist_plan<BnG1>(v->ws3, sc, p->ck->tables ? &job.tbl : nullptr, fs >= 2, &hist);
+      if (e != hipErrorNotSupported) { P_TRY(e); counted = true; }
+    }
+    const uint32_t* negB = hasB ? (const uint32_t*)(a.cur->d + 8 * a.r * sc) : (const uint32_t*)nullptr;
+    if (counted)
+      P_TRY((launch_fold_cross_hist<Fr, BnG1::Scalar>(v->s3, hist, sc, p->AZ, p->BZ, p->CZ, p->E, (const uint32_t*)Scur.buf, fold_E ? 1 : 0, a.rho, hasB ? 1 : 0, v->rho_prev, negB, v->u1_run,
+                                                      az, bz, cz, out, (const uint32_t*)(t->b->az + 8 * t->row * nc), (const uint32_t*)(t->b->bz + 8 * t->row * nc),
+                                                      (const uint32_t*)(t->b->cz + 8 * t->row * nc), Fe::one(), outm, (uint32_t)p->n_bool)));
+    else
+      hipLaunchKernelGGL(k_fold_cross<Fr>, dim3(stream_grid(sc)), dim3(256), 0, v->s3, sc, p->AZ, p->BZ, p->CZ, p->E, (const uint32_t*)Scur.buf, fold_E ? 1 : 0, a.rho,
+                         hasB ? 1 : 0, v->rho_prev, negB, v->u1_run, az, bz, cz,
+                         out, t ? t->b->az + 8 * t->row * nc : nullptr, t ? t->b->bz + 8 * t->row * nc : nullptr, t ? t->b->cz + 8 * t->row * nc : nullptr, Fe::one(),
+                         outm, p->n_bool);
     P_TRY(hipGetLastError());
     if (a.need1 && a.look) {
       P_TRY(wait_row_flag(*a.next2.b, a.next2.row, a.next2.b->ev[a.next2.row]));
@@ -150,7 +165,7 @@
     t_hk[0] += now_s() - tq; tq = now_s();
     P_TRY(hipEventRecord(v->ev_fused, v->s3)); v->fused_recorded = true;
     t_hk[1] += now_s() - tq;
-    if (a.need1) { Soth.step = (int64_t)a.i + 1; Soth.hasB = false; Soth.tricked = trick; Soth.u_at = v->u1_run; int rc2 = queue_msm(par ^ 1); if (rc2) return rc2; }
+    if (a.need1) { Soth.step = (int64_t)a.i + 1; Soth.hasB = false; Soth.tricked = trick; Soth.u_at = v->u1_run; int rc2 = queue_msm(par ^ 1, counted ? &hist : nullptr); if (rc2) return rc2; }
     if (a.look) { Scur.step = (int64_t)a.i + 2; Scur.hasB = true; Scur.tricked = trick; Scur.u_at = v->u1_run; int rc2 = queue_msm(par); if (rc2) return rc2; }
     return VIMZ_OK;
   };
diff --git a/vimz_amd/csrc/msm.hpp b/vimz_amd/csrc/msm.hpp
--- a/vimz_amd/csrc/msm.hpp
+++ b/vimz_amd/csrc/msm.hpp
@@ -4,15 +4,17 @@
 #include <mutex>
 #include "msm_api.hpp"
 #include "ec_mem.hpp"
+#include "msm_digits.hpp"
 
 namespace vz {
 
-struct MsmTuning { int sort_blocks = 0, combine_lane_bits = -1, small_lean = 0, witness_sub = 0, ones_dense = 1, reduce_planes = 0, accum_lds_kb = 0, dense_sub = 0, signed_scalars = 1; };
+struct MsmTuning { int sort_blocks = 0, combine_lane_bits = -1, small_lean = 0, witness_sub = 0, ones_dense = 1, reduce_planes = 0, accum_lds_kb = 0, dense_sub = 0, signed_scalars = 1, fused_blocks = 0; };
 inline const MsmTuning& msm_tuning() {
   static const MsmTuning t = [] {
     MsmTuning r;
     if (const char* e = getenv("VIMZ_TUNE")) {
       if (const char* q = strstr(e, "sort_blocks=")) r.sort_blocks = atoi(q + 12);
+      if (const char* q = strstr(e, "fused_blocks=")) r.fused_blocks = atoi(q + 13);
       if (const char* q = strstr(e, "combine_lane_bits=")) r.combine_lane_bits = atoi(q + 18);
       if (const char* q = strstr(e, "small_lean=")) r.small_lean = atoi(q + 11);
       if (const char* q = strstr(e, "witness_sub=")) { const int v = atoi(q + 12); if (v >= 2 && v <= MSM_SUB) r.witness_sub = v; }
@@ -28,58 +30,6 @@
 }
 
 
-__device__ __forceinline__ uint32_t window_bits(const uint32_t* s, int lo, int c) {
-  int limb = lo >> 5, off = lo & 31;
-  if (limb >= 8) return 0;
-  uint64_t v = s[limb];
-  if (limb + 1 < 8) v |= (uint64_t)s[limb + 1] << 32;
-  return (uint32_t)(v >> off) & ((1u << c) - 1);
-}
-
-template <class S>
-__device__ __forceinline__ bool load_scalar(const uint32_t* __restrict__ scalars, size_t i, int mont, int skip_ones, int sgn, uint32_t* s, uint32_t& flip) {
-  const uint4* p = reinterpret_cast<const uint4*>(scalars + 8 * i);
-  uint4 a = p[0], b = p[1];
-  S x;
-  x.v[0] = a.x; x.v[1] = a.y; x.v[2] = a.z; x.v[3] = a.w; x.v[4] = b.x; x.v[5] = b.y; x.v[6] = b.z; x.v[7] = b.w;
-  if (x.is_zero()) return false;
-  if (skip_ones) {
-    bool one;
-    if (mont) one = x.eq(S::one());
-    else { uint32_t o = x.v[0] ^ 1u; for (int k = 1; k < 8; k++) o |= x.v[k]; one = o == 0; }
-    if (one) return false;
-  }
-  if (mont) x = S::from_mont(x);
-  flip = 0;
-  if (sgn) {
-    uint32_t t[8]; uint64_t br = 0, lt = 0;
-#pragma unroll
-    for (int k = 0; k < 8; k++) { const uint64_t d = (uint64_t)S::Params::MOD.w[k] - x.v[k] - br; t[k] = (uint32_t)d; br = (d >> 32) & 1; }
-#pragma unroll
-    for (int k = 0; k < 8; k++) { const uint64_t d = (uint64_t)t[k] - x.v[k] - lt; lt = (d >> 32) & 1; }
-    if (!br && lt) {
-      flip = 1;
-#pragma unroll
-      for (int k = 0; k < 8; k++) x.v[k] = t[k];
-    }
-  }
-#pragma unroll
-  for (int k = 0; k < 8; k++) s[k] = x.v[k];
-  return true;
-}
-
-template <class Fn>
-__device__ __forceinline__ void for_each_digit(const uint32_t* s, int c, int K, uint32_t flip, Fn f) {
-  uint32_t carry = 0;
-  const uint32_t half = 1u << (c - 1);
-  for (int w = 0; w < K; w++) {
-    uint32_t d = window_bits(s, w * c, c) + carry;
-    uint32_t neg = d > half;
-    uint32_t mag = neg ? (1u << c) - d : d;
-    carry = neg;
-    if (mag) f(w, mag - 1, neg ^ flip);
-  }
-}
 
 __device__ __forceinline__ uint32_t agg_atomic_inc(uint32_t* __restrict__ ctr, uint32_t g) {
   const uint32_t lane = __lane_id();
@@ -112,35 +62,6 @@
   }
 }
 
-__device__ __forceinline__ void scan_body(const uint32_t* __restrict__ counts, uint32_t nb,
-                                               uint32_t* __restrict__ bucket_off, uint32_t* __restrict__ sub_off,
-                                               uint32_t* __restrict__ totals, uint32_t sub,
-                                               uint32_t* __restrict__ heavy ,
-                                               uint32_t heavy_min, uint32_t heavy_cap) {
-  __shared__ uint32_t wv_e[2][16], wv_s[2][16];
-  const uint32_t t = threadIdx.x, lane = t & 63u, wv = t >> 6;
-  uint32_t carry_e = 0, carry_s = 0;
-  for (uint32_t base = 0, it = 0; base < nb; base += 1024, it++) {
-    const uint32_t b = base + t;
-    const uint32_t cnt = b < nb ? counts[b] : 0u, m = (cnt + sub - 1) / sub;
-    uint32_t ie = cnt, is = m;
-#pragma unroll
-    for (uint32_t d = 1; d < 64; d <<= 1) {
-      const uint32_t ve = __shfl_up(ie, d), vs = __shfl_up(is, d);
-      if (lane >= d) { ie += ve; is += vs; }
-    }
-    if (lane == 63) { wv_e[it & 1][wv] = ie; wv_s[it & 1][wv] = is; }
-    __syncthreads();
-    uint32_t oe = 0, os = 0, te = 0, ts = 0;
-    for (uint32_t q = 0; q < 16; q++) { const uint32_t xe = wv_e[it & 1][q], xs = wv_s[it & 1][q]; if (q < wv) { oe += xe; os += xs; } te += xe; ts += xs; }
-    if (b < nb) {
-      bucket_off[b] = carry_e + oe + ie - cnt; sub_off[b] = carry_s + os + is - m;
-      if (m > heavy_min) { const uint32_t slot = atomicAdd(&heavy[0], 1u); if (slot < heavy_cap) heavy[1 + slot] = b; }
-    }
-    carry_e += te; carry_s += ts;
-  }
-  if (t == 0) { bucket_off[nb] = carry_e; sub_off[nb] = carry_s; totals[0] = carry_s; totals[1] = carry_e; }
-}
 template <int SUB>
 __global__ void __launch_bounds__(1024) k_scan(const uint32_t* __restrict__ counts, uint32_t nb, uint32_t* __restrict__ bucket_off, uint32_t* __restrict__ sub_off,
                                                uint32_t* __restrict__ totals, uint32_t sub, uint32_t* __restrict__ heavy, uint32_t heavy_min, uint32_t heavy_cap) {
@@ -163,8 +84,6 @@
   }
 }
 
-constexpr uint32_t SORT_BLOCKS = 256;
-constexpr uint32_t SORT_THREADS = 1024;
 
 template <class S>
 __global__ void __launch_bounds__(SORT_THREADS) k_hist_lds(const uint32_t* __restrict__ scalars, size_t n, int mont, int skip_ones, int sgn, int c, int K,
@@ -173,9 +92,8 @@
   scalars += blockIdx.y * rs.scalars; block_hist += blockIdx.y * rs.block_hist;
   for (uint32_t g = threadIdx.x; g < nb; g += SORT_THREADS) lds_cnt[g] = 0;
   __syncthreads();
-  const size_t chunk = (n + gridDim.x - 1) / gridDim.x;
-  const size_t lo = blockIdx.x * chunk, hi = lo + chunk < n ? lo + chunk : n;
-  for (size_t i = lo + threadIdx.x; i < hi; i += SORT_THREADS) {
+  const SortRange mine_rows = sort_range(n, gridDim.x, blockIdx.x);
+  for (size_t i = mine_rows.lo + threadIdx.x; i < mine_rows.hi; i += SORT_THREADS) {
     uint32_t s[8], flip;
     if (!load_scalar<S>(scalars, i, mont, skip_ones, sgn, s, flip)) continue;
     for_each_digit(s, c, K, flip, [&](int w, uint32_t b, uint32_t) { atomicAdd(&lds_cnt[(uint32_t)w * nbw + b], 1u); });
@@ -195,16 +113,7 @@
     block_hist += row * rs.block_hist; counts += row * rs.counts; heavy += row * rs.heavy; bucket_off += row * rs.offs; sub_off += row * rs.offs; totals += row * rs.totals;
   }
   const uint32_t g = blockIdx.x * blockDim.x + threadIdx.x;
-  if (g < nb) {
-    uint32_t run = 0;
-    for (uint32_t blk = 0; blk < nblocks; blk++) {
-      const size_t idx = (size_t)blk * nb + g;
-      const uint32_t v = block_hist[idx];
-      block_hist[idx] = run;
-      run += v;
-    }
-    counts[g] = run;
-  }
+  if (g < nb) counts[g] = prefix_column<8>(block_hist, nb, nblocks, g);
   __threadfence();
   __syncthreads();
   if (threadIdx.x == 0) s_last = atomicAdd(&totals[2], 1u) == gridDim.x - 1 ? 1u : 0u;
@@ -225,9 +134,8 @@
   const uint32_t* mine = block_hist + (size_t)blockIdx.x * nb;
   for (uint32_t g = threadIdx.x; g < nb; g += SORT_THREADS) lds_pos[g] = bucket_off[g] + mine[g];
   __syncthreads();
-  const size_t chunk = (n + gridDim.x - 1) / gridDim.x;
-  const size_t lo = blockIdx.x * chunk, hi = lo + chunk < n ? lo + chunk : n;
-  for (size_t i = lo + threadIdx.x; i < hi; i += SORT_THREADS) {
+  const SortRange mine_rows = sort_range(n, gridDim.x, blockIdx.x);
+  for (size_t i = mine_rows.lo + threadIdx.x; i < mine_rows.hi; i += SORT_THREADS) {
     uint32_t s[8], flip;
     if (!load_scalar<S>(scalars, i, mont, skip_ones, sgn, s, flip)) continue;
     for_each_digit(s, c, K, flip, [&](int w, uint32_t b, uint32_t neg) {
@@ -822,11 +730,13 @@
 template <class C>
 static hipError_t msm_launch_impl(hipStream_t stream, MsmWorkspace& ws, const uint32_t* d_bases, const uint32_t* d_scalars, size_t n,
                                   int scalars_mont, int c_override, void* pinned_dst, MsmPlan* plan_out, hipEvent_t* ev, int split_ones,
-                                  const BaseTables* tb, const MsmRowGroup* rg) {
+                                  const BaseTables* tb, const MsmRowGroup* rg, const MsmPrehist* counted = nullptr, MsmPrehist* plan_query = nullptr) {
   typedef typename C::Coord F;
   typedef typename C::Scalar S;
   if (n == 0 || n >= (1u << 31)) return hipErrorInvalidValue;
   const uint32_t G = rg ? rg->G : 1u;
+  const bool pre = counted || plan_query;
+  if (pre && (G > 1 || split_ones || !scalars_mont)) return hipErrorNotSupported;
   if (rg && !rg->row_bytes_out && (G == 0 || G > MSM_ROWS_MAX || rg->n_extra > MSM_ROWS_MAX || (split_ones == 0 && rg->n_extra))) return hipErrorInvalidValue;
   const int sgn = msm_tuning().signed_scalars;
   constexpr bool direct = true;
@@ -838,7 +748,7 @@
   const bool own = tabled && tb->own;
   if (small_tb && (n > MSM_SMALL_MAX || tb->K != (S::Params::BITS + SMALL_C) / SMALL_C)) return hipErrorInvalidValue;
   if (!no_small && !tabled && c_override <= 0 && n <= MSM_SMALL_MAX) {
-    if (rg) return hipErrorNotSupported;
+    if (rg || pre) return hipErrorNotSupported;
     MsmPlan ps; ps.c = SMALL_C; ps.K = (S::Params::BITS + SMALL_C) / SMALL_C; ps.nbw = SMALL_NBW; ps.nb = SMALL_NBW * (uint32_t)ps.K; ps.split_ones = 0; ps.tabled = small_tb ? 2 : 0;
     *plan_out = ps;
     VZ_HIP_CHECK(ws.reserve_small());
@@ -885,6 +795,7 @@
   if (planes) pl.tabled = 4;
   const bool lds_sort = (size_t)pl.nb * 4 <= 144 * 1024;
   if (rg && (planes || own || !lds_sort)) return hipErrorNotSupported;
+  if (pre && (own || !lds_sort)) return hipErrorNotSupported;
   *plan_out = pl;
   const size_t entries = (size_t)pl.K * n;
   const int wsub = msm_tuning().witness_sub;
@@ -909,24 +820,25 @@
     VZ_HIP_CHECK(hipMemsetAsync(ws.heavy, 0, 4, stream));
   }
   const int sort_blocks_env = msm_tuning().sort_blocks;
+  const int fused_blocks_env = pre ? msm_tuning().fused_blocks : 0;
   const uint32_t sort_blocks = sort_blocks_env > 0 && sort_blocks_env <= (int)SORT_BLOCKS ? (uint32_t)sort_blocks_env
+                               : fused_blocks_env > 0 && fused_blocks_env <= (int)SORT_BLOCKS ? (uint32_t)fused_blocks_env
                                                                                            : (uint32_t)std::min<size_t>(SORT_BLOCKS, std::max<size_t>(32, n / 4096));
   const uint32_t bstride = tabled && !own ? 0u : pl.nbw, pstride = tabled ? (uint32_t)tb->n_total : 0u;
   if (lds_sort) {
     VZ_HIP_CHECK(ws.reserve_block_hist((size_t)SORT_BLOCKS * pl.nb));
     {
-      static std::mutex attr_mu;
       static uint64_t attr_devices = 0;
       int dev = 0;
       VZ_HIP_CHECK(hipGetDevice(&dev));
-      std::lock_guard<std::mutex> g(attr_mu);
+      std::lock_guard<std::mutex> g(msm_sort_attr_mutex());
       if (!((attr_devices >> (dev & 63)) & 1ull)) {
         VZ_HIP_CHECK(hipFuncSetAttribute(reinterpret_cast<const void*>(&k_hist_lds<S>), hipFuncAttributeMaxDynamicSharedMemorySize, 160 * 1024));
         VZ_HIP_CHECK(hipFuncSetAttribute(reinterpret_cast<const void*>(&k_scatter_lds<S>), hipFuncAttributeMaxDynamicSharedMemorySize, 160 * 1024));
         attr_devices |= 1ull << (dev & 63);
       }
     }
-    hipLaunchKernelGGL(k_hist_lds<S>, dim3(sort_blocks, G), dim3(SORT_THREADS), pl.nb * 4, stream, d_scalars, n, scalars_mont, split_ones, sgn, pl.c, pl.K, bstride, pl.nb, ws.block_hist, rs);
+    if (!pre) hipLaunchKernelGGL(k_hist_lds<S>, dim3(sort_blocks, G), dim3(SORT_THREADS), pl.nb * 4, stream, d_scalars, n, scalars_mont, split_ones, sgn, pl.c, pl.K, bstride, pl.nb, ws.block_hist, rs);
   } else {
     hipLaunchKernelGGL(k_hist<S>, dim3(gs), dim3(TB), 0, stream, d_scalars, n, scalars_mont, split_ones, sgn, pl.c, pl.K, bstride, ws.counts);
   }
@@ -935,7 +847,18 @@
   const int lane_bits_env = msm_tuning().combine_lane_bits;
   const uint32_t lane_bits = lane_bits_env >= 0 ? (uint32_t)lane_bits_env : mean_parts > 96 ? 4u : mean_parts > 48 ? 3u : mean_parts > 24 ? 2u : 1u;
   const uint32_t heavy_min = 16u << lane_bits;
-  if (lds_sort)
+  if (pre) {
+    const MsmPrehist want{sort_blocks, pl.c, pl.K, bstride, pl.nb, sgn, ws.block_hist, counted ? counted->scan : plan_query->scan, ws.counts, ws.heavy, ws.bucket_off, ws.sub_off, ws.totals,
+                          sub, heavy_min, MsmWorkspace::HEAVY_CAP, n};
+    if (plan_query) { *plan_query = want; return hipSuccess; }
+    const MsmPrehist& h = *counted;
+    if (h.sort_blocks != want.sort_blocks || h.c != want.c || h.K != want.K || h.bstride != want.bstride || h.nb != want.nb || h.sgn != want.sgn || h.block_hist != want.block_hist ||
+        h.counts != want.counts || h.heavy != want.heavy || h.bucket_off != want.bucket_off || h.sub_off != want.sub_off || h.totals != want.totals || h.sub != want.sub ||
+        h.heavy_min != want.heavy_min || h.heavy_cap != want.heavy_cap || h.n != want.n)
+      return hipErrorInvalidValue;
+  }
+  if (counted && counted->scan) {}
+  else if (lds_sort)
     hipLaunchKernelGGL(k_prefix_scan<0>, dim3((pl.nb + 1023) / 1024, G), dim3(1024), 0, stream, ws.block_hist, pl.nb, ws.counts, sort_blocks, ws.heavy, ws.bucket_off, ws.sub_off,
                        ws.totals, sub, heavy_min, MsmWorkspace::HEAVY_CAP, rs);
   else
@@ -1000,15 +923,26 @@
 template <class C>
 hipError_t msm_launch_rows(hipStream_t stream, MsmWorkspace& ws, const uint32_t* d_bases, const uint32_t* d_scalars, size_t n, size_t scalar_row_stride, uint32_t G,
                            int scalars_mont, void* pinned_dst, size_t pinned_row_stride, MsmPlan* plan_out, int split_ones, const BaseTables* tb,
-                           const OnesDesc* extra, uint32_t n_extra, uint32_t max_rows) {
+                           const OnesDesc* extra, uint32_t n_extra, uint32_t max_rows, const MsmPrehist* counted) {
   if (G > 1 && (scalar_row_stride < n || (pinned_row_stride & 15))) return hipErrorInvalidValue;
   const MsmRowGroup rg{G, scalar_row_stride, pinned_row_stride, extra, n_extra, max_rows, nullptr};
-  const hipError_t e = msm_launch_impl<C>(stream, ws, d_bases, d_scalars, n, scalars_mont, 0, pinned_dst, plan_out, nullptr, split_ones, tb, &rg);
-  if (e != hipErrorNotSupported) return e;
+  const hipError_t e = msm_launch_impl<C>(stream, ws, d_bases, d_scalars, n, scalars_mont, 0, pinned_dst, plan_out, nullptr, split_ones, tb, &rg, counted);
+  if (e != hipErrorNotSupported || counted) return e;
   for (uint32_t r = 0; r < G; r++)
     VZ_HIP_CHECK(msm_launch<C>(stream, ws, d_bases, d_scalars + 8 * r * scalar_row_stride, n, scalars_mont, 0, (char*)pinned_dst + r * pinned_row_stride, plan_out, nullptr, split_ones, tb));
   if (n_extra) VZ_HIP_CHECK(ones_launch_rows<C>(stream, ws, extra, n_extra, scalars_mont));
   return hipSuccess;
+}
+template <class C>
+hipError_t msm_prehist_plan(MsmWorkspace& ws, size_t n, const BaseTables* tb, int scan, MsmPrehist* out) {
+  MsmPlan pl;
+  out->scan = scan;
+  return msm_launch_impl<C>(nullptr, ws, tb ? tb->d : nullptr, nullptr, n, 1, 0, nullptr, &pl, nullptr, 0, tb, nullptr, nullptr, out);
+}
+template <class C>
+hipError_t msm_launch_counted(hipStream_t stream, MsmWorkspace& ws, const uint32_t* d_bases, const uint32_t* d_scalars, size_t n, void* pinned_dst, MsmPlan* plan_out,
+                              hipEvent_t* ev, const BaseTables* tb, const MsmPrehist& h) {
+  return msm_launch_impl<C>(stream, ws, d_bases, d_scalars, n, 1, 0, pinned_dst, plan_out, ev, 0, tb, nullptr, &h);
 }
 template <class C>
 size_t msm_rows_row_bytes(size_t n, int split_ones, const BaseTables* tb) {
diff --git a/vimz_amd/csrc/msm_api.hpp b/vimz_amd/csrc/msm_api.hpp
--- a/vimz_amd/csrc/msm_api.hpp
+++ b/vimz_amd/csrc/msm_api.hpp
@@ -2,6 +2,7 @@
 #include <hip/hip_runtime.h>
 #include <vector>
 #include <algorithm>
+#include <mutex>
 #include "ec.hpp"
 
 namespace vz {
@@ -140,6 +141,13 @@
 
 struct MsmStats { int c, K; uint32_t subs, entries; float ms[6]; };
 
+struct MsmPrehist {
+  uint32_t sort_blocks; int c, K; uint32_t bstride, nb; int sgn; uint32_t* block_hist;
+  int scan; uint32_t *counts, *heavy, *bucket_off, *sub_off, *totals; uint32_t sub, heavy_min, heavy_cap;
+  size_t n;
+};
+inline std::mutex& msm_sort_attr_mutex() { static std::mutex mu; return mu; }
+
 template <class C>
 hipError_t msm_launch(hipStream_t stream, MsmWorkspace& ws, const uint32_t* d_bases, const uint32_t* d_scalars, size_t n,
                       int scalars_mont, int c_override, void* pinned_dst, MsmPlan* plan_out, hipEvent_t* ev, int split_ones,
@@ -147,7 +155,12 @@
 template <class C>
 hipError_t msm_launch_rows(hipStream_t stream, MsmWorkspace& ws, const uint32_t* d_bases, const uint32_t* d_scalars, size_t n, size_t scalar_row_stride, uint32_t G,
                            int scalars_mont, void* pinned_dst, size_t pinned_row_stride, MsmPlan* plan_out, int split_ones, const BaseTables* tb,
-                           const OnesDesc* extra = nullptr, uint32_t n_extra = 0, uint32_t max_rows = 0);
+                           const OnesDesc* extra = nullptr, uint32_t n_extra = 0, uint32_t max_rows = 0, const MsmPrehist* counted = nullptr);
+template <class C>
+hipError_t msm_prehist_plan(MsmWorkspace& ws, size_t n, const BaseTables* tb, int scan, MsmPrehist* out);
+template <class C>
+hipError_t msm_launch_counted(hipStream_t stream, MsmWorkspace& ws, const uint32_t* d_bases, const uint32_t* d_scalars, size_t n, void* pinned_dst, MsmPlan* plan_out,
+                              hipEvent_t* ev, const BaseTables* tb, const MsmPrehist& h);
 template <class C>
 size_t msm_rows_row_bytes(size_t n, int split_ones, const BaseTables* tb);
 template <class C>
diff --git a/vimz_amd/csrc/msm_digits.hpp b/vimz_amd/csrc/msm_digits.hpp
--- /dev/null
+++ b/vimz_amd/csrc/msm_digits.hpp
@@ -0,0 +1,126 @@
+#pragma once
+#include <hip/hip_runtime.h>
+#include <cstdint>
+
+namespace vz {
+
+__device__ __forceinline__ uint32_t window_bits(const uint32_t* s, int lo, int c) {
+  int limb = lo >> 5, off = lo & 31;
+  if (limb >= 8) return 0;
+  uint64_t v = s[limb];
+  if (limb + 1 < 8) v |= (uint64_t)s[limb + 1] << 32;
+  return (uint32_t)(v >> off) & ((1u << c) - 1);
+}
+
+template <class S>
+__device__ __forceinline__ S load_scalar_word(const uint32_t* __restrict__ scalars, size_t i) {
+  const uint4* p = reinterpret_cast<const uint4*>(scalars + 8 * i);
+  uint4 a = p[0], b = p[1];
+  S x;
+  x.v[0] = a.x; x.v[1] = a.y; x.v[2] = a.z; x.v[3] = a.w; x.v[4] = b.x; x.v[5] = b.y; x.v[6] = b.z; x.v[7] = b.w;
+  return x;
+}
+template <class S>
+__device__ __forceinline__ bool scalar_of_word(S x, int mont, int skip_ones, int sgn, uint32_t* s, uint32_t& flip) {
+  if (x.is_zero()) return false;
+  if (skip_ones) {
+    bool one;
+    if (mont) one = x.eq(S::one());
+    else { uint32_t o = x.v[0] ^ 1u; for (int k = 1; k < 8; k++) o |= x.v[k]; one = o == 0; }
+    if (one) return false;
+  }
+  if (mont) x = S::from_mont(x);
+  flip = 0;
+  if (sgn) {
+    uint32_t t[8]; uint64_t br = 0, lt = 0;
+#pragma unroll
+    for (int k = 0; k < 8; k++) { const uint64_t d = (uint64_t)S::Params::MOD.w[k] - x.v[k] - br; t[k] = (uint32_t)d; br = (d >> 32) & 1; }
+#pragma unroll
+    for (int k = 0; k < 8; k++) { const uint64_t d = (uint64_t)t[k] - x.v[k] - lt; lt = (d >> 32) & 1; }
+    if (!br && lt) {
+      flip = 1;
+#pragma unroll
+      for (int k = 0; k < 8; k++) x.v[k] = t[k];
+    }
+  }
+#pragma unroll
+  for (int k = 0; k < 8; k++) s[k] = x.v[k];
+  return true;
+}
+template <class S>
+__device__ __forceinline__ bool load_scalar(const uint32_t* __restrict__ scalars, size_t i, int mont, int skip_ones, int sgn, uint32_t* s, uint32_t& flip) {
+  return scalar_of_word<S>(load_scalar_word<S>(scalars, i), mont, skip_ones, sgn, s, flip);
+}
+
+template <class Fn>
+__device__ __forceinline__ void for_each_digit(const uint32_t* s, int c, int K, uint32_t flip, Fn f) {
+  uint32_t carry = 0;
+  const uint32_t half = 1u << (c - 1);
+  for (int w = 0; w < K; w++) {
+    uint32_t d = window_bits(s, w * c, c) + carry;
+    uint32_t neg = d > half;
+    uint32_t mag = neg ? (1u << c) - d : d;
+    carry = neg;
+    if (mag) f(w, mag - 1, neg ^ flip);
+  }
+}
+
+constexpr uint32_t SORT_BLOCKS = 256;
+constexpr uint32_t SORT_THREADS = 1024;
+
+struct SortRange { size_t lo, hi; };
+__host__ __device__ __forceinline__ SortRange sort_range(size_t n, uint32_t blocks, uint32_t x) {
+  const size_t chunk = (n + blocks - 1) / blocks, lo = x * chunk;
+  return SortRange{lo < n ? lo : n, lo + chunk < n ? lo + chunk : n};
+}
+
+template <int AHEAD>
+__device__ __forceinline__ uint32_t prefix_column(uint32_t* __restrict__ block_hist, uint32_t nb, uint32_t nblocks, uint32_t g) {
+  uint32_t run = 0, blk = 0;
+  for (; blk + AHEAD <= nblocks; blk += AHEAD) {
+    uint32_t v[AHEAD];
+#pragma unroll
+    for (int k = 0; k < AHEAD; k++) v[k] = block_hist[(size_t)(blk + k) * nb + g];
+#pragma unroll
+    for (int k = 0; k < AHEAD; k++) { block_hist[(size_t)(blk + k) * nb + g] = run; run += v[k]; }
+  }
+  for (; blk < nblocks; blk++) {
+    const size_t idx = (size_t)blk * nb + g;
+    const uint32_t v = block_hist[idx];
+    block_hist[idx] = run;
+    run += v;
+  }
+  return run;
+}
+
+__device__ __forceinline__ void scan_body(const uint32_t* __restrict__ counts, uint32_t nb,
+                                               uint32_t* __restrict__ bucket_off, uint32_t* __restrict__ sub_off,
+                                               uint32_t* __restrict__ totals, uint32_t sub,
+                                               uint32_t* __restrict__ heavy ,
+                                               uint32_t heavy_min, uint32_t heavy_cap) {
+  __shared__ uint32_t wv_e[2][16], wv_s[2][16];
+  const uint32_t t = threadIdx.x, lane = t & 63u, wv = t >> 6;
+  uint32_t carry_e = 0, carry_s = 0;
+  for (uint32_t base = 0, it = 0; base < nb; base += 1024, it++) {
+    const uint32_t b = base + t;
+    const uint32_t cnt = b < nb ? counts[b] : 0u, m = (cnt + sub - 1) / sub;
+    uint32_t ie = cnt, is = m;
+#pragma unroll
+    for (uint32_t d = 1; d < 64; d <<= 1) {
+      const uint32_t ve = __shfl_up(ie, d), vs = __shfl_up(is, d);
+      if (lane >= d) { ie += ve; is += vs; }
+    }
+    if (lane == 63) { wv_e[it & 1][wv] = ie; wv_s[it & 1][wv] = is; }
+    __syncthreads();
+    uint32_t oe = 0, os = 0, te = 0, ts = 0;
+    for (uint32_t q = 0; q < 16; q++) { const uint32_t xe = wv_e[it & 1][q], xs = wv_s[it & 1][q]; if (q < wv) { oe += xe; os += xs; } te += xe; ts += xs; }
+    if (b < nb) {
+      bucket_off[b] = carry_e + oe + ie - cnt; sub_off[b] = carry_s + os + is - m;
+      if (m > heavy_min) { const uint32_t slot = atomicAdd(&heavy[0], 1u); if (slot < heavy_cap) heavy[1 + slot] = b; }
+    }
+    carry_e += te; carry_s += ts;
+  }
+  if (t == 0) { bucket_off[nb] = carry_e; sub_off[nb] = carry_s; totals[0] = carry_s; totals[1] = carry_e; }
+}
+
+}
diff --git a/vimz_amd/csrc/msm_inst_bn254_g1.hip b/vimz_amd/csrc/msm_inst_bn254_g1.hip
--- a/vimz_amd/csrc/msm_inst_bn254_g1.hip
+++ b/vimz_amd/csrc/msm_inst_bn254_g1.hip
@@ -9,7 +9,9 @@
 template hipError_t ones_launch<BnG1>(hipStream_t, MsmWorkspace&, const uint32_t*, const uint32_t*, size_t, int, void*);
 template XYZZ<BnG1::Base> ones_finish<BnG1>(const void*);
 template hipError_t msm_launch_rows<BnG1>(hipStream_t, MsmWorkspace&, const uint32_t*, const uint32_t*, size_t, size_t, uint32_t, int, void*, size_t, MsmPlan*, int, const BaseTables*,
-                                          const OnesDesc*, uint32_t, uint32_t);
+                                          const OnesDesc*, uint32_t, uint32_t, const MsmPrehist*);
+template hipError_t msm_prehist_plan<BnG1>(MsmWorkspace&, size_t, const BaseTables*, int, MsmPrehist*);
+template hipError_t msm_launch_counted<BnG1>(hipStream_t, MsmWorkspace&, const uint32_t*, const uint32_t*, size_t, void*, MsmPlan*, hipEvent_t*, const BaseTables*, const MsmPrehist&);
 template size_t msm_rows_row_bytes<BnG1>(size_t, int, const BaseTables*);
 template hipError_t ones_launch_rows<BnG1>(hipStream_t, MsmWorkspace&, const OnesDesc*, uint32_t, int);
 }
diff --git a/vimz_amd/csrc/prover.hip b/vimz_amd/csrc/prover.hip
--- a/vimz_amd/csrc/prover.hip
+++ b/vimz_amd/csrc/prover.hip
@@ -7,6 +7,7 @@
 
 std::atomic<long>& vz_head_rows_override() { static std::atomic<long> v{-1}; return v; }
 std::atomic<long>& vz_rows_group_override() { static std::atomic<long> v{-1}; return v; }
+std::atomic<long>& vz_fused_sort_override() { static std::atomic<long> v{-1}; return v; }
 
 extern "C" {
 
@@ -196,6 +197,7 @@
 extern "C" {
 long vimz_set_head_rows(long rows) { return vz_head_rows_override().exchange(rows < 0 ? -1 : rows); }
 long vimz_set_rows_group(long rows) { return vz_rows_group_override().exchange(rows < 0 ? -1 : rows); }
+long vimz_set_fused_sort(long mode) { return vz_fused_sort_override().exchange(mode < 0 ? -1 : mode); }
 
 int vimz_prover_reset(vimz_prover* p, const uint64_t* z0) {
   if (!p || !z0) return VIMZ_ERR_INVALID;
diff --git a/vimz_amd/csrc/prover_internal.hpp b/vimz_amd/csrc/prover_internal.hpp
--- a/vimz_amd/csrc/prover_internal.hpp
+++ b/vimz_amd/csrc/prover_internal.hpp
@@ -432,6 +432,14 @@
   const long v = ov >= 0 ? ov : env >= 0 ? env : (long)ROWS_GROUP_DEFAULT;
   return (size_t)std::min<long>(v, (long)MSM_ROWS_MAX);
 }
+std::atomic<long>& vz_fused_sort_override();
+constexpr long FUSED_SORT_DEFAULT = 0;
+static int fused_sort_wanted() {
+  static const long env = [] { const char* e = getenv("VIMZ_TUNE"); const char* q = e ? strstr(e, "fused_sort=") : nullptr; return q ? atol(q + 11) : -1L; }();
+  const long ov = vz_fused_sort_override().load(std::memory_order_relaxed);
+  const long v = ov >= 0 ? ov : env >= 0 ? env : FUSED_SORT_DEFAULT;
+  return (int)std::min<long>(v, 2);
+}
 static inline hipError_t wait_row_flag(const vimz_prover::BatchBuf& bb, size_t idx, hipEvent_t ev) {
   const uint32_t want = bb.gen;
   const uint32_t* f = bb.row_flag + idx;
diff --git a/vimz_amd/csrc/r1cs_capi.hip b/vimz_amd/csrc/r1cs_capi.hip
--- a/vimz_amd/csrc/r1cs_capi.hip
+++ b/vimz_amd/csrc/r1cs_capi.hip
@@ -8,6 +8,7 @@
 
 #include "internal.hpp"
 #include "r1cs_ops.hpp"
+#include "fold_hist.hpp"
 
 using namespace vz;
 
@@ -360,5 +361,84 @@
   return VIMZ_OK;
 }
 
+int vimz_test_fold_cross_msm(vimz_ctx* ctx, const vimz_bases* bases, int use_tables, size_t n, vimz_vec* AZ, vimz_vec* BZ, vimz_vec* CZ, vimz_vec* E, const vimz_vec* Tin,
+                             const vimz_vec* az, const vimz_vec* bz, const vimz_vec* cz, const vimz_vec* azn, const vimz_vec* bzn, const vimz_vec* czn, const uint64_t r[4],
+                             const uint64_t u[4], int form, size_t nb, int fold_E, int mode, vimz_vec* out, vimz_vec* outm, uint64_t commit_xy[8]) {
+  if (!ctx || !bases || !r || !u || !commit_xy || !n) return vz_fail(ctx, VIMZ_ERR_INVALID, "vimz_test_fold_cross_msm: bad argument");
+  const vimz_vec* vs[13] = {AZ, BZ, CZ, E, Tin, az, bz, cz, azn, bzn, czn, out, outm};
+  for (const vimz_vec* v : vs) if (!v || v->field != VIMZ_FIELD_BN254_FR || v->n < n) return vz_fail(ctx, VIMZ_ERR_INVALID, "vimz_test_fold_cross_msm: field or length of a vector");
+  if (bases->curve != VIMZ_CURVE_BN254_G1 || n > bases->n || nb > n || n >= (1ull << 31) || mode < 0 || mode > 2 || out == outm || (use_tables && !bases->tables))
+    return vz_fail(ctx, VIMZ_ERR_INVALID, "vimz_test_fold_cross_msm: key, boolean prefix or mode");
+  typedef Fp<BnFr> F;
+  typedef BnG1::Base FS;
+  F rr, uu; int rc;
+  if ((rc = scalar_arg(ctx, r, form, &rr, "vimz_test_fold_cross_msm: r not below the modulus")) || (rc = scalar_arg(ctx, u, form, &uu, "vimz_test_fold_cross_msm: u not below the modulus"))) return rc;
+  std::lock_guard<std::mutex> g(ctx->mu);
+  R_TRY(hipSetDevice(ctx->device));
+  char* pin = nullptr;
+  R_TRY(hipHostMalloc((void**)&pin, 4 * (size_t)XYZZ_WORDS * MSM_MAX_WINDOWS));
+  memset(pin, 0xff, 4 * (size_t)XYZZ_WORDS * MSM_MAX_WINDOWS);
+  const BaseTables tb = bases->tb(0);
+  const BaseTables* tbp = use_tables ? &tb : nullptr;
+  MsmWorkspace& ws = ctx->msm_ws;
+  MsmPlan pl;
+  const F none = F::zero();
+  hipError_t e = hipSuccess;
+  if (mode == 0) {
+    hipLaunchKernelGGL(k_fold_cross<F>, dim3(stream_grid(n)), dim3(256), 0, ctx->stream, n, AZ->d, BZ->d, CZ->d, E->d, (const uint32_t*)Tin->d, fold_E ? 1 : 0, rr, 0, none, (const uint32_t*)nullptr, uu,
+                       (const uint32_t*)az->d, (const uint32_t*)bz->d, (const uint32_t*)cz->d, out->d, (const uint32_t*)azn->d, (const uint32_t*)bzn->d, (const uint32_t*)czn->d, F::one(), outm->d, (uint32_t)nb);
+    e = hipGetLastError();
+    if (e == hipSuccess) e = msm_launch<BnG1>(ctx->stream, ws, bases->d, outm->d, n, 1, 0, pin, &pl, nullptr, 0, tbp);
+  } else {
+    MsmPrehist h;
+    e = msm_prehist_plan<BnG1>(ws, n, tbp, mode == 2, &h);
+    if (e == hipSuccess)
+      e = launch_fold_cross_hist<F, BnG1::Scalar>(ctx->stream, h, n, AZ->d, BZ->d, CZ->d, E->d, (const uint32_t*)Tin->d, fold_E ? 1 : 0, rr, 0, none, (const uint32_t*)nullptr, uu,
+                                                  (const uint32_t*)az->d, (const uint32_t*)bz->d, (const uint32_t*)cz->d, out->d, (const uint32_t*)azn->d, (const uint32_t*)bzn->d,
+                                                  (const uint32_t*)czn->d, F::one(), outm->d, (uint32_t)nb);
+    if (e == hipSuccess) e = msm_launch_counted<BnG1>(ctx->stream, ws, bases->d, outm->d, n, pin, &pl, nullptr, tbp, h);
+  }
+  const hipError_t e2 = hipStreamSynchronize(ctx->stream);
+  if (e == hipSuccess && e2 == hipSuccess) {
+    const Affine<FS> a = msm_finish<BnG1>(pl, pin);
+    const FS x = FS::from_mont(a.x), y = FS::from_mont(a.y);
+    memcpy(commit_xy, x.v, 32); memcpy(commit_xy + 4, y.v, 32);
+  }
+  hipHostFree(pin);
+  if (e != hipSuccess) return vz_fail(ctx, VIMZ_ERR_HIP, "vimz_test_fold_cross_msm", e);
+  if (e2 != hipSuccess) return vz_fail(ctx, VIMZ_ERR_HIP, "vimz_test_fold_cross_msm: synchronize", e2);
+  return VIMZ_OK;
+}
+
+int vimz_test_msm_counted_refusal(vimz_ctx* ctx, const vimz_bases* bases, int use_tables, size_t n, size_t G, int* hip_error) {
+  if (!ctx || !bases || !hip_error || !n || !G || G > MSM_ROWS_MAX || bases->curve != VIMZ_CURVE_BN254_G1 || n > bases->n || (use_tables && !bases->tables))
+    return vz_fail(ctx, VIMZ_ERR_INVALID, "vimz_test_msm_counted_refusal: bad argument");
+  std::lock_guard<std::mutex> g(ctx->mu);
+  R_TRY(hipSetDevice(ctx->device));
+  int rc = vz_ensure_scratch(ctx, 32 * G * n); if (rc) return rc;
+  R_TRY(hipMemsetAsync(ctx->scratch, 0, 32 * G * n, ctx->stream));
+  const size_t pin_stride = 4 * (size_t)XYZZ_WORDS * MSM_MAX_WINDOWS;
+  char* pin = nullptr;
+  R_TRY(hipHostMalloc((void**)&pin, G * pin_stride));
+  const BaseTables tb = bases->tb(0);
+  const BaseTables* tbp = use_tables ? &tb : nullptr;
+  MsmWorkspace ws;
+  MsmPlan pl;
+  MsmPrehist h{};
+  hipError_t e = msm_prehist_plan<BnG1>(ws, n, tbp, 0, &h);
+  if (G == 1) {
+    if (e == hipSuccess) e = hipMemsetAsync(h.block_hist, 0, 4 * (size_t)h.sort_blocks * h.nb, ctx->stream); else { h = MsmPrehist{}; e = hipSuccess; }
+    if (e == hipSuccess) e = msm_launch_counted<BnG1>(ctx->stream, ws, bases->d, (const uint32_t*)ctx->scratch, n, pin, &pl, nullptr, tbp, h);
+  } else {
+    e = msm_launch_rows<BnG1>(ctx->stream, ws, bases->d, (const uint32_t*)ctx->scratch, n, n, (uint32_t)G, 1, pin, pin_stride, &pl, 0, tbp, nullptr, 0, (uint32_t)G, &h);
+  }
+  const hipError_t e2 = hipStreamSynchronize(ctx->stream);
+  ws.release();
+  hipHostFree(pin);
+  if (e2 != hipSuccess) return vz_fail(ctx, VIMZ_ERR_HIP, "vimz_test_msm_counted_refusal: synchronize", e2);
+  *hip_error = (int)e;
+  return VIMZ_OK;
+}
+
 }
 #endif
diff --git a/vimz_amd/csrc/r1cs_ops.hpp b/vimz_amd/csrc/r1cs_ops.hpp
--- a/vimz_amd/csrc/r1cs_ops.hpp
+++ b/vimz_amd/csrc/r1cs_ops.hpp
@@ -200,31 +200,39 @@
 }
 
 template <class F>
+__device__ __forceinline__ F fold_cross_row(size_t i, uint32_t* __restrict__ AZ, uint32_t* __restrict__ BZ, uint32_t* __restrict__ CZ, uint32_t* __restrict__ E,
+                                            const uint32_t* Tin, int fold_E, const F& r, int hasB, const F& r_prev, const uint32_t* __restrict__ negB, const F& u1_new,
+                                            const uint32_t* __restrict__ az, const uint32_t* __restrict__ bz, const uint32_t* __restrict__ cz,
+                                            uint32_t* out, const uint32_t* __restrict__ azn, const uint32_t* __restrict__ bzn, const uint32_t* __restrict__ czn, const F& u2,
+                                            uint32_t* __restrict__ outm, uint32_t nb) {
+  const F a = F::add(load_fe<F>(AZ, i), mul_fresh(r, load_fe<F>(az, i)));
+  const F b = F::add(load_fe<F>(BZ, i), mul_fresh(r, load_fe<F>(bz, i)));
+  const F c = F::add(load_fe<F>(CZ, i), mul_fresh(r, load_fe<F>(cz, i)));
+  store_fe(AZ, i, a); store_fe(BZ, i, b); store_fe(CZ, i, c);
+  if (fold_E) {
+    F t = load_fe<F>(Tin, i);
+    if (hasB) t = F::sub(t, mul_fresh(r_prev, load_fe<F>(negB, i)));
+    if (__ballot(!t.is_zero()) != 0ull) { const F e = F::add(load_fe<F>(E, i), F::mul(r, t)); if (!t.is_zero()) store_fe(E, i, e); }
+  }
+  if (!out) return F::zero();
+  const F an = load_fe<F>(azn, i);
+  F t = mul_fresh(a, load_fe<F>(bzn, i));
+  t = F::add(t, mul_fresh(b, an));
+  t = F::sub(t, mul_fresh(u1_new, load_fe<F>(czn, i)));
+  t = F::sub(t, mul_fresh(c, u2));
+  store_fe(out, i, t);
+  if (!outm) return t;
+  const F m = i < nb ? bool_row_masked(t, a, an) : t;
+  store_fe(outm, i, m);
+  return m;
+}
+template <class F>
 __global__ void __launch_bounds__(256) k_fold_cross(size_t n, uint32_t* __restrict__ AZ, uint32_t* __restrict__ BZ, uint32_t* __restrict__ CZ, uint32_t* __restrict__ E,
                                                     const uint32_t* Tin, int fold_E, F r, int hasB, F r_prev, const uint32_t* __restrict__ negB, F u1_new,
                                                     const uint32_t* __restrict__ az, const uint32_t* __restrict__ bz, const uint32_t* __restrict__ cz,
                                                     uint32_t* out, const uint32_t* __restrict__ azn, const uint32_t* __restrict__ bzn, const uint32_t* __restrict__ czn, F u2,
                                                     uint32_t* __restrict__ outm = nullptr, uint32_t nb = 0) {
-  VZ_GRID_STRIDE(i, n) {
-    const F a = F::add(load_fe<F>(AZ, i), mul_fresh(r, load_fe<F>(az, i)));
-    const F b = F::add(load_fe<F>(BZ, i), mul_fresh(r, load_fe<F>(bz, i)));
-    const F c = F::add(load_fe<F>(CZ, i), mul_fresh(r, load_fe<F>(cz, i)));
-    store_fe(AZ, i, a); store_fe(BZ, i, b); store_fe(CZ, i, c);
-    if (fold_E) {
-      F t = load_fe<F>(Tin, i);
-      if (hasB) t = F::sub(t, mul_fresh(r_prev, load_fe<F>(negB, i)));
-      if (__ballot(!t.is_zero()) != 0ull) { const F e = F::add(load_fe<F>(E, i), F::mul(r, t)); if (!t.is_zero()) store_fe(E, i, e); }
-    }
-    if (out) {
-      const F an = load_fe<F>(azn, i);
-      F t = mul_fresh(a, load_fe<F>(bzn, i));
-      t = F::add(t, mul_fresh(b, an));
-      t = F::sub(t, mul_fresh(u1_new, load_fe<F>(czn, i)));
-      t = F::sub(t, mul_fresh(c, u2));
-      store_fe(out, i, t);
-      if (outm) store_fe(outm, i, i < nb ? bool_row_masked(t, a, an) : t);
-    }
-  }
+  VZ_GRID_STRIDE(i, n) fold_cross_row<F>(i, AZ, BZ, CZ, E, Tin, fold_E, r, hasB, r_prev, negB, u1_new, az, bz, cz, out, azn, bzn, czn, u2, outm, nb);
 }
 
 template <class F>
diff --git a/vimz_amd/hip.py b/vimz_amd/hip.py
--- a/vimz_amd/hip.py
+++ b/vimz_amd/hip.py
@@ -828,6 +828,13 @@
     return int(lib.vimz_set_rows_group(int(rows)))
 
 
+def set_fused_sort(mode):
+    lib = L.lib()
+    lib.vimz_set_fused_sort.argtypes = [C.c_long]
+    lib.vimz_set_fused_sort.restype = C.c_long
+    return int(lib.vimz_set_fused_sort(int(mode)))
+
+
 class Decider:
     RESULT_BITS = {1: "fewer than two steps", 2: "KZG opening of cmW", 4: "KZG opening of cmE", 8: "Groth16", 16: "a word pair is not a curve point"}
 
```

Measured after the change: 1420. -1.2%, worse.
